# TropComplique/MultiPoseNet

Measured on AMD Instinct MI355X. Metric: images/sec keypoint fwd+bwd+Adam @512x512 bs32/GPU, higher is better.
Workload: dtype bf16; 1 GPU; MobileNet-v1+FPN+keypoint_subnet fwd+bwd+Adam, 512x512, per-GPU batch 32; global_batch=32, parallelism=dp1, hip_graph=True, rccl_ranks=1

## Files before the change

include/mpn.h:

```cpp
#ifndef MPN_H_
#define MPN_H_

#include <stddef.h>
#include <stdint.h>

#ifdef __cplusplus
extern "C" {
#endif

#define MPN_VERSION 600

enum { MPN_F32 = 0, MPN_BF16 = 1, MPN_F16 = 2  };

enum {
    MPN_OK = 0,
    MPN_ERR_BAD_SHAPE = -1,
    MPN_ERR_BAD_DTYPE = -2,
    MPN_ERR_BAD_ALIGN = -3,
    MPN_ERR_HIP = -4,
    MPN_ERR_BAD_ARG = -5,
    MPN_ERR_WORKSPACE = -6,
    MPN_ERR_BAD_DATA = -7
};

enum { MPN_ACT_NONE = 0, MPN_ACT_RELU = 1, MPN_ACT_RELU6 = 2 };

typedef void* mpn_stream_t;

int mpn_version(void);
int mpn_last_error(char* buf, size_t n);

size_t mpn_heatmap_decode_workspace_bytes(int B);
int mpn_heatmap_decode(const void* heatmaps, int dtype, int B, int h, int w, int C,
                       const double* box_hw, float threshold,
                       int32_t* out_xyv, float* out_score, int32_t* out_index,
                       void* workspace, size_t workspace_bytes, mpn_stream_t stream);

size_t mpn_conv_packed_bytes(int Cin, int Cout, int ksize, int transpose, int dtype);
int mpn_conv_pack_weights(const float* w_hwio, int Cin, int Cout, int ksize, int transpose,
                          int dtype, void* out, mpn_stream_t stream);
size_t mpn_conv_pack_desc_bytes(void);
int mpn_conv_pack_desc_fill(void* desc_host, const float* w_hwio, int Cin, int Cout, int ksize, int transpose,
                            int dtype, void* out, int block_begin);
int mpn_conv_pack_weights_batched(const void* descs_device, int ndesc, int total_blocks, int dtype,
                                  mpn_stream_t stream);
int mpn_conv_num_parts(int N, int H, int W, int ksize);
int mpn_conv_stats_rows(int N, int H, int W, int Cin, int Cout, int ksize, int dtype);
int mpn_conv_fwd(const void* x, const void* w_packed, void* y, int N, int H, int W, int Cin,
                 int Cout, int x_stride, int y_stride, int ksize, int dtype, const float* in_scale,
                 const float* in_shift, int in_act, float* stats_part, const void* up_res,
                 mpn_stream_t stream);
int mpn_conv_fwd_grouped(int njobs, const void* const* x, const void* const* w_packed, void* const* y, int N, const int* H,
                         const int* W, int Cin, int Cout, const int* x_stride, const int* y_stride, int ksize, int dtype,
                         const float* const* in_scale, const float* const* in_shift, int in_act,
                         float* const* stats_part, mpn_stream_t stream);
int mpn_conv_bwd_data_bn_supported(int K, int C, int ksize, int dtype);
int mpn_conv_bwd_data_bn(const void* dy, const void* w_packed_t, void* dx, int N, int H, int W, int K, int C, int dy_stride,
                         int dx_stride, int ksize, int dtype, const void* bn_x, int bn_x_stride, const float* bn_scale,
                         const float* bn_shift, int bn_act, float* part, mpn_stream_t stream);
int mpn_conv_bwd_data_bn_grouped(int njobs, const void* const* dy, const void* const* w_packed_t, void* const* dx, int N,
                                 const int* H, const int* W, int K, int C, const int* dy_stride, const int* dx_stride,
                                 int dtype, const void* const* bn_x, const int* bn_x_stride, const float* const* bn_scale,
                                 const float* const* bn_shift, int bn_act, float* const* part, mpn_stream_t stream);

int mpn_conv_wgrad_num_parts(int N, int H, int W, int Cin, int Cout, int ksize, int dtype);
int mpn_conv_bwd_weight(const void* x, const void* dy, float* part, int N, int H, int W, int Cin,
                        int Cout, int x_stride, int dy_stride, int ksize, int dtype, const float* in_scale,
                        const float* in_shift, int in_act, mpn_stream_t stream);

int mpn_conv1x1_bwd_fused_supported(int Cin, int Cout, int dtype);
int mpn_conv1x1_bwd_fused(const void* x, const void* dy, const float* w, void* dx, float* wpart, float* bn_part, int N, int H, int W,
                          int Cin, int Cout, int x_stride, int dy_stride, int dx_stride, int dtype, const float* in_scale,
                          const float* in_shift, int in_act, mpn_stream_t stream);
int mpn_conv1x1_bwd_fused_apply_supported(int Cin, int Cout, int dtype);
int mpn_conv1x1_bwd_fused_apply(const void* x, const void* g, const void* y_raw, const float* w, void* dx, float* wpart, float* bn_part,
                                int N, int H, int W, int Cin, int Cout, int x_stride, int g_stride, int y_stride, int dx_stride,
                                int dtype, const float* in_scale, const float* in_shift, int in_act, const float* ap_scale,
                                const float* ap_shift, const float* ap_mean, const float* ap_invstd, const float* ap_k1,
                                const float* ap_k2, int ap_act, mpn_stream_t stream);
int mpn_conv_wgrad_grouped_num_parts(int njobs, int N, const int* H, const int* W, int Cin, int Cout, int ksize, int dtype,
                                     int* nparts);
int mpn_conv_bwd_weight_grouped(int njobs, const void* const* x, const void* const* dy, float* const* part, int N,
                                const int* H, const int* W, int Cin, int Cout, const int* x_stride, const int* dy_stride,
                                int ksize, int dtype, const float* const* in_scale, const float* const* in_shift,
                                int in_act, mpn_stream_t stream);

int mpn_bn_stats_num_parts(long long M);
int mpn_bn_stats(const void* x, long long M, int C, int dtype, float* part, mpn_stream_t stream);
int mpn_bn_finalize(float* part, int nparts, int C, long long count, const float* gamma,
                    const float* beta, float* moving_mean, float* moving_var, float momentum,
                    float eps, float* scale, float* shift, float* save_mean, float* save_invstd,
                    mpn_stream_t stream);
int mpn_bn_bwd_reduce_grouped(int njobs, void* const* dA, const void* const* x, const long long* M, int C, int dtype,
                              const float* const* scale, const float* const* shift, const float* const* mean,
                              const float* const* invstd, int act, float* const* part, const int* dA_stride,
                              const int* x_stride, mpn_stream_t stream);
int mpn_bn_bwd_apply_grouped(int njobs, void* const* dA, const void* const* x, const long long* M, int C, int dtype,
                             const float* const* scale, const float* const* shift, const float* const* mean,
                             const float* const* invstd, const float* const* k1, const float* const* k2, int act,
                             const float* const* add_ch0, const int* dA_stride, const int* x_stride,
                             mpn_stream_t stream);
size_t mpn_bn_fin_desc_bytes(void);
size_t mpn_bn_bwd_fin_desc_bytes(void);
int mpn_bn_fin_desc_fill(void* desc_host, const float* part, int nparts, int C, long long count, const float* gamma,
                         const float* beta, float* moving_mean, float* moving_var, float* scale, float* shift,
                         float* save_mean, float* save_invstd, int block_begin);
int mpn_bn_bwd_fin_desc_fill(void* desc_host, const float* part, int nparts, int C, long long count, float* dgamma,
                             float* dbeta, float* k1, float* k2, int block_begin);
int mpn_bn_bwd_fin_desc_fill_raw(void* desc_host, const float* part, int nparts, int C, long long count, float* dgamma,
                                 float* dbeta, float* k1, float* k2, const float* mean, const float* invstd,
                                 int block_begin);
int mpn_bn_finalize_batched(const void* descs_device, int ndesc, int total_blocks, float momentum, float eps,
                            mpn_stream_t stream);
int mpn_bn_bwd_finalize_batched(const void* descs_device, int ndesc, int total_blocks, mpn_stream_t stream);
int mpn_bn_inference_affine(int C, const float* gamma, const float* beta, const float* moving_mean,
                            const float* moving_var, float eps, float* scale, float* shift,
                            mpn_stream_t stream);
int mpn_bn_act_apply(const void* x, void* y, long long M, int C, int dtype, const float* scale,
                     const float* shift, int act, mpn_stream_t stream);
int mpn_bn_bwd_reduce(const void* dA, const void* x, long long M, int C, int dtype,
                      const float* scale, const float* shift, const float* mean,
                      const float* invstd, int act, float* part, mpn_stream_t stream);
int mpn_bn_bwd_finalize(float* part, int nparts, int C, long long count, float* dgamma,
                        float* dbeta, float* k1, float* k2, mpn_stream_t stream);
int mpn_bn_bwd_finalize_raw(float* part, int nparts, int C, long long count, float* dgamma, float* dbeta, float* k1,
                            float* k2, const float* mean, const float* invstd, mpn_stream_t stream);
int mpn_bn_bwd_apply(void* dA, const void* x, long long M, int C, int dtype, const float* scale,
                     const float* shift, const float* mean, const float* invstd, const float* k1,
                     const float* k2, int act, const float* add_ch0, mpn_stream_t stream);

int mpn_dwconv_out_size(int size, int stride);
int mpn_dwconv_num_parts(int N, int H, int W, int C, int stride, int dtype);
int mpn_dwconv_fwd(const void* x, const float* w, void* y, int N, int H, int W, int C, int stride,
                   int dtype, const float* in_scale, const float* in_shift, int in_act, int flip,
                   float* stats_part, mpn_stream_t stream);
int mpn_dwconv_bwd_data(const void* dy, const float* w, void* dx, int N, int H, int W, int C,
                        int stride, int dtype, mpn_stream_t stream);
int mpn_dwconv_bwd_data_bn_num_parts(int N, int H, int W, int C, int stride, int dtype);
int mpn_dwconv_bwd_data_bn(const void* dy, const float* w, void* dx, int N, int H, int W, int C, int stride, int dtype,
                           const void* x_bn, const float* scale, const float* shift, const float* mean,
                           const float* invstd, int act, float* part, mpn_stream_t stream);
int mpn_dwconv_bwd_data_add_supported(int N, int H, int W, int C, int stride, int dtype);
int mpn_dwconv_bwd_data_add(const void* dy, const float* w, void* dx, int N, int H, int W, int C, int stride, int dtype,
                            const void* addend, const void* x_bn, const float* scale, const float* shift,
                            const float* mean, const float* invstd, int act, float* part, mpn_stream_t stream);
int mpn_dwconv_wgrad_num_parts(int N, int H, int W, int C, int stride, int dtype);
int mpn_dwconv_bwd_weight(const void* x, const void* dy, float* part, int N, int H, int W, int C,
                          int stride, int dtype, const float* in_scale, const float* in_shift,
                          int in_act, mpn_stream_t stream);

int mpn_dwconv_bwd_fused_supported(int N, int H, int W, int C, int stride, int dtype);
int mpn_dwconv_bwd_fused(const void* x, const void* dy, const float* w, void* dx, float* wpart, int N, int H, int W, int C,
                         int dtype, const float* in_scale, const float* in_shift, int in_act, const float* mean,
                         const float* invstd, float* bn_part, mpn_stream_t stream);
int mpn_dwconv_bwd_fused_s2(const void* x, const void* dy, const float* w, void* dx, float* wpart, int N, int H, int W, int C,
                            int dtype, const float* in_scale, const float* in_shift, int in_act, const float* mean,
                            const float* invstd, float* bn_part, const void* addend, mpn_stream_t stream);

int mpn_stem_conv_fwd(const void* images, int images_u8, const float* w, void* y, int N, int H,
                      int W, int C0, int dtype, mpn_stream_t stream);
int mpn_stem_conv_fwd_num_parts(int N, int H, int W, int C0, int dtype);
int mpn_stem_conv_fwd_stats(const void* images, int images_u8, const float* w, void* y, int N, int H, int W, int C0,
                            int dtype, float* stats_part, mpn_stream_t stream);
int mpn_stem_conv_wgrad_num_parts(int N, int H, int W);
int mpn_stem_conv_bwd_weight(const void* images, int images_u8, const void* dy, float* part, int N,
                             int H, int W, int C0, int dtype, mpn_stream_t stream);

int mpn_bilinear_up_fwd(const void* x, void* y, int N, int h, int w, int C, int upsample,
                        int y_channel_offset, int y_channels_total, int dtype,
                        const float* in_scale, const float* in_shift, int in_act,
                        mpn_stream_t stream);
int mpn_bilinear_up_bwd(const void* dy, void* dx, int N, int h, int w, int C, int upsample,
                        int y_channel_offset, int y_channels_total, int dtype, mpn_stream_t stream);
int mpn_sumpool2x2(const void* src, void* dst, int N, int h, int w, int C, int accumulate,
                   int dtype, mpn_stream_t stream);
int mpn_add_inplace(void* dst, const void* src, long long n, int dtype, mpn_stream_t stream);

int mpn_heatmap_head_fwd(const void* x, const float* w, const float* bias, long long M, int Cin,
                         int dtype, const float* in_scale, const float* in_shift, int in_act,
                         int mode, float* out, float* out_seg, mpn_stream_t stream);
int mpn_heatmap_head_bwd_num_parts(long long M);
int mpn_heatmap_head_bwd(const void* x, const float* dlogits, const float* w, long long M, int Cin,
                         int dtype, const float* in_scale, const float* in_shift, int in_act,
                         void* dA, float* part, mpn_stream_t stream);
int mpn_heatmap_head_bwd_bn_supported(int Cin, int dtype);
int mpn_heatmap_head_bwd_bn(const void* x, const float* dlogits, const float* w, long long M, int Cin, int dtype,
                            const float* in_scale, const float* in_shift, int in_act, void* dA, float* part,
                            float* bn_part, mpn_stream_t stream);

int mpn_keypoint_loss_num_parts(int B, int h, int w);
int mpn_keypoint_loss(const float* logits, const float* heatmaps, const float* loss_masks,
                      const float* segmentation_masks, const int* num_boxes, const void* p2,
                      const void* p3, const void* p4, const void* p5, int p_channels, int p_dtype,
                      float* dlogits, float* daux2, float* daux3, float* daux4, float* daux5,
                      float* part, float* losses_out, int B, int h, int w, mpn_stream_t stream);

int mpn_adam_prepare(long long* step, float* hyper, double initial_learning_rate,
                     double decay_steps, double alpha, double beta1, double beta2,
                     mpn_stream_t stream);
int mpn_adam_step(float* params, const float* grads, float* m, float* v, long long n,
                  const float* hyper, float beta1, float beta2, float eps, float clip,
                  float grad_scale, mpn_stream_t stream);
int mpn_adam_step_cast(float* params, const float* grads, float* m, float* v, long long n, const float* hyper, float beta1,
                       float beta2, float eps, float clip, float grad_scale, int ncast, const long long* cast_begin,
                       const long long* cast_count, void* const* cast_dst, int cast_dtype, mpn_stream_t stream);
int mpn_reduce_partials(const float* part, int nparts, long long n, float* out, int accumulate,
                        float scale, mpn_stream_t stream);
size_t mpn_reduce_desc_bytes(void);
int mpn_reduce_desc_fill(void* desc_host, const float* part, int nparts, long long n, float* out, float scale,
                         int block_begin);
int mpn_reduce_partials_batched(const void* descs_device, int ndesc, int total_blocks, mpn_stream_t stream);
int mpn_axpy(long long n, float a, const float* x, float* y, mpn_stream_t stream);
int mpn_axpy_batched(int count, const float* const* x, float* const* y, const long long* n, float a, mpn_stream_t stream);
int mpn_l2_loss_accumulate(long long n, const float* w, float scale, float* acc, mpn_stream_t stream);
size_t mpn_l2_loss_batched_workspace_bytes(int count, const long long* n);
int mpn_l2_loss_batched(int count, const float* const* w, const long long* n, float scale, float* acc, void* workspace,
                        size_t workspace_bytes, mpn_stream_t stream);

size_t mpn_heatmap_render_workspace_bytes(int total_persons);
int mpn_heatmap_render(const int32_t* keypoints, const float* boxes, const int32_t* first_person,
                       int B, int total_persons, int width, int height, int downsample, float* out,
                       void* workspace, size_t workspace_bytes, mpn_stream_t stream);

enum {
    MPN_AUGMENT_ROTATE = 1, MPN_AUGMENT_COLOR = 2, MPN_AUGMENT_GRAYSCALE = 4, MPN_AUGMENT_PIXEL_SCALE = 8,
    MPN_AUGMENT_FLIP = 16, MPN_AUGMENT_EVAL = 32
};
#define MPN_KEYPOINT_AUGMENT_DESC_BYTES 192
typedef struct mpn_keypoint_augment_desc {
    int64_t src_offset, mask_offset;
    int32_t src_h, src_w, mask_h, mask_w;
    int32_t crop_y, crop_x, crop_h, crop_w;
    int32_t valid_h, valid_w, valid_mh, valid_mw;
    float transform[8], mask_transform[8];
    float window[4];
    float scale_y, scale_x;
    float mask_scale_y, mask_scale_x;
    float color[3];
    uint32_t seed;
    int32_t flags;
    int32_t reserved[3];
} mpn_keypoint_augment_desc;
#ifdef __cplusplus
static_assert(sizeof(mpn_keypoint_augment_desc) == MPN_KEYPOINT_AUGMENT_DESC_BYTES, "descriptor size is fixed");
#endif
size_t mpn_keypoint_augment_desc_bytes(void);
int mpn_keypoint_augment(const uint8_t* sources, const uint8_t* masks, const void* descs, int B, int H, int W,
                         float* images, float* loss_masks, float* segmentation_masks, mpn_stream_t stream);

enum { MPN_AUGMENT_PAD = 64 };
#define MPN_DETECTOR_AUGMENT_DESC_BYTES 112
typedef struct mpn_detector_augment_desc {
    int64_t src_offset;
    int32_t src_h, src_w;
    int32_t crop_y, crop_x, crop_h, crop_w;
    int32_t valid_h, valid_w;
    int32_t pad_y, pad_x, pad_h, pad_w;
    float scale_y, scale_x;
    float pad_scale_y, pad_scale_x;
    float color[3];
    float minval, maxval;
    uint32_t seed;
    int32_t flags;
    int32_t reserved[3];
} mpn_detector_augment_desc;
#ifdef __cplusplus
static_assert(sizeof(mpn_detector_augment_desc) == MPN_DETECTOR_AUGMENT_DESC_BYTES, "descriptor size is fixed");
#endif
size_t mpn_detector_augment_desc_bytes(void);
int mpn_detector_augment(const uint8_t* sources, const void* descs, int B, int H, int W, float* images,
                         mpn_stream_t stream);

#define MPN_PRN_EXAMPLE_DESC_BYTES 16
typedef struct mpn_prn_example_desc {
    int32_t image;
    int32_t person;
    int32_t flip;
    int32_t reserved;
} mpn_prn_example_desc;
#ifdef __cplusplus
static_assert(sizeof(mpn_prn_example_desc) == MPN_PRN_EXAMPLE_DESC_BYTES, "descriptor size is fixed");
#endif
size_t mpn_prn_example_desc_bytes(void);
size_t mpn_prn_examples_workspace_bytes(int total_persons);
int mpn_prn_examples(const int32_t* keypoints, const float* boxes, int total_persons,
                     const int32_t* first_person, const int32_t* width, const int32_t* height,
                     int num_images, const void* examples, int N, int crop_h, int crop_w, int downsample,
                     float* crops, float* labels, void* workspace, size_t workspace_bytes, mpn_stream_t stream);

int mpn_gemm_nt_num_parts(int K);
int mpn_gemm_nt(const void* a, const void* b, float* part, int M, int N, int K, int dtype, mpn_stream_t stream);
int mpn_transpose_cast(const void* in, int in_dtype, void* out, int out_dtype, int R, int C, mpn_stream_t stream);
int mpn_cast(const void* in, int in_dtype, void* out, int out_dtype, long long n, mpn_stream_t stream);
int mpn_bias_relu_fwd(const void* pre, int pre_dtype, const float* bias, void* y, int out_dtype, int R, int C,
                      mpn_stream_t stream);
int mpn_bias_relu_bwd(const void* y, int y_dtype, const float* dy, void* dpre, int dpre_dtype, float* dbias, int R,
                      int C, mpn_stream_t stream);
int mpn_prn_loss(const float* x, const void* y2, int y2_dtype, const float* labels, int B, int P, int C,
                 float* logits, float* dlogits, float* loss_part, float grad_scale, mpn_stream_t stream);
int mpn_prn_residual(const float* x, const void* y2, int y2_dtype, long long n, float* logits, mpn_stream_t stream);

int mpn_heatmap_minmax(const float* heatmaps, int B, int h, int w, int C, void* minmax_keys, mpn_stream_t stream);
int mpn_prn_crop(const float* heatmaps, const void* minmax_keys, const float* boxes, const int* box_ind, int nb, int B,
                 int h, int w, int C, int crop_h, int crop_w, float threshold, float* crops, mpn_stream_t stream);
int mpn_prn_crop_slots(const float* heatmaps, const void* minmax_keys, const float* boxes, const int* num_boxes, int slot0,
                       int nb, int max_boxes, int B, int h, int w, int C, int crop_h, int crop_w, float threshold,
                       float* crops, mpn_stream_t stream);
int mpn_prn_decode(const float* logits, int nb, int crop_h, int crop_w, int C, float* scores, float* positions,
                   mpn_stream_t stream);

// ... 267 lines not shown
```

multiposenet_amd/_lib.py:

```python
import ctypes
import os

_HERE = os.path.dirname(os.path.abspath(__file__))
LIB_PATH = os.environ.get("MPN_LIB") or os.path.join(_HERE, "libmpn_hip.so")

MPN_VERSION = 600
MPN_F32, MPN_BF16, MPN_F16 = 0, 1, 2
ACT_NONE, ACT_RELU, ACT_RELU6 = 0, 1, 2

_c = ctypes
_P = _c.c_void_p
_I = _c.c_int
_F = _c.c_float
_D = _c.c_double
_Z = _c.c_size_t
_L = _c.c_longlong

SIGNATURES = {
    "mpn_version": (_I, []),
    "mpn_last_error": (_I, [_c.c_char_p, _Z]),
    "mpn_heatmap_decode_workspace_bytes": (_Z, [_I]),
    "mpn_heatmap_decode": (_I, [_P, _I, _I, _I, _I, _I, _P, _F, _P, _P, _P, _P, _Z, _P]),
    "mpn_heatmap_render_workspace_bytes": (_Z, [_I]),
    "mpn_heatmap_render": (_I, [_P, _P, _P, _I, _I, _I, _I, _I, _P, _P, _Z, _P]),
    "mpn_keypoint_augment_desc_bytes": (_Z, []),
    "mpn_keypoint_augment": (_I, [_P, _P, _P, _I, _I, _I, _P, _P, _P, _P]),
    "mpn_detector_augment_desc_bytes": (_Z, []),
    "mpn_detector_augment": (_I, [_P, _P, _I, _I, _I, _P, _P]),
    "mpn_prn_example_desc_bytes": (_Z, []),
    "mpn_prn_examples_workspace_bytes": (_Z, [_I]),
    "mpn_prn_examples": (_I, [_P, _P, _I, _P, _P, _P, _I, _P, _I, _I, _I, _I, _P, _P, _P, _Z, _P]),
    "mpn_conv_packed_bytes": (_Z, [_I, _I, _I, _I, _I]),
    "mpn_conv_pack_weights": (_I, [_P, _I, _I, _I, _I, _I, _P, _P]),
    "mpn_conv_pack_desc_bytes": (_Z, []),
    "mpn_conv_pack_desc_fill": (_I, [_P, _P, _I, _I, _I, _I, _I, _P, _I]),
    "mpn_conv_pack_weights_batched": (_I, [_P, _I, _I, _I, _P]),
    "mpn_conv_num_parts": (_I, [_I, _I, _I, _I]),
    "mpn_conv_stats_rows": (_I, [_I, _I, _I, _I, _I, _I, _I]),
    "mpn_conv_fwd": (_I, [_P, _P, _P, _I, _I, _I, _I, _I, _I, _I, _I, _I, _P, _P, _I, _P, _P, _P]),
    "mpn_conv_fwd_grouped": (_I, [_I, _P, _P, _P, _I, _P, _P, _I, _I, _P, _P, _I, _I, _P, _P, _I, _P, _P]),
    "mpn_conv_wgrad_num_parts": (_I, [_I, _I, _I, _I, _I, _I, _I]),
    "mpn_conv_bwd_weight": (_I, [_P, _P, _P, _I, _I, _I, _I, _I, _I, _I, _I, _I, _P, _P, _I, _P]),
    "mpn_conv1x1_bwd_fused_supported": (_I, [_I, _I, _I]),
    "mpn_conv1x1_bwd_fused": (_I, [_P, _P, _P, _P, _P, _P, _I, _I, _I, _I, _I, _I, _I, _I, _I, _P, _P, _I, _P]),
    "mpn_conv1x1_bwd_fused_apply_supported": (_I, [_I, _I, _I]),
    "mpn_conv1x1_bwd_fused_apply": (_I, [_P, _P, _P, _P, _P, _P, _P, _I, _I, _I, _I, _I, _I, _I, _I, _I, _I, _P, _P, _I, _P, _P, _P, _P, _P, _P, _I, _P]),
    "mpn_conv_wgrad_grouped_num_parts": (_I, [_I, _I, _P, _P, _I, _I, _I, _I, _P]),
    "mpn_conv_bwd_weight_grouped": (_I, [_I, _P, _P, _P, _I, _P, _P, _I, _I, _P, _P, _I, _I, _P, _P, _I, _P]),
    "mpn_bn_stats_num_parts": (_I, [_L]),
    "mpn_bn_stats": (_I, [_P, _L, _I, _I, _P, _P]),
    "mpn_bn_finalize": (_I, [_P, _I, _I, _L, _P, _P, _P, _P, _F, _F, _P, _P, _P, _P, _P]),
    "mpn_bn_inference_affine": (_I, [_I, _P, _P, _P, _P, _F, _P, _P, _P]),
    "mpn_bn_act_apply": (_I, [_P, _P, _L, _I, _I, _P, _P, _I, _P]),
    "mpn_bn_bwd_reduce": (_I, [_P, _P, _L, _I, _I, _P, _P, _P, _P, _I, _P, _P]),
    "mpn_bn_bwd_finalize": (_I, [_P, _I, _I, _L, _P, _P, _P, _P, _P]),
    "mpn_bn_bwd_apply": (_I, [_P, _P, _L, _I, _I, _P, _P, _P, _P, _P, _P, _I, _P, _P]),
    "mpn_dwconv_out_size": (_I, [_I, _I]),
    "mpn_dwconv_num_parts": (_I, [_I, _I, _I, _I, _I, _I]),
    "mpn_dwconv_fwd": (_I, [_P, _P, _P, _I, _I, _I, _I, _I, _I, _P, _P, _I, _I, _P, _P]),
    "mpn_dwconv_bwd_data": (_I, [_P, _P, _P, _I, _I, _I, _I, _I, _I, _P]),
    "mpn_dwconv_bwd_data_bn_num_parts": (_I, [_I, _I, _I, _I, _I, _I]),
    "mpn_dwconv_bwd_data_bn": (_I, [_P, _P, _P, _I, _I, _I, _I, _I, _I, _P, _P, _P, _P, _P, _I, _P, _P]),
    "mpn_dwconv_bwd_data_add_supported": (_I, [_I, _I, _I, _I, _I, _I]),
    "mpn_dwconv_bwd_data_add": (_I, [_P, _P, _P, _I, _I, _I, _I, _I, _I, _P, _P, _P, _P, _P, _P, _I, _P, _P]),
    "mpn_dwconv_wgrad_num_parts": (_I, [_I, _I, _I, _I, _I, _I]),
    "mpn_dwconv_bwd_weight": (_I, [_P, _P, _P, _I, _I, _I, _I, _I, _I, _P, _P, _I, _P]),
    "mpn_dwconv_bwd_fused_supported": (_I, [_I, _I, _I, _I, _I, _I]),
    "mpn_dwconv_bwd_fused": (_I, [_P, _P, _P, _P, _P, _I, _I, _I, _I, _I, _P, _P, _I, _P, _P, _P, _P]),
    "mpn_dwconv_bwd_fused_s2": (_I, [_P, _P, _P, _P, _P, _I, _I, _I, _I, _I, _P, _P, _I, _P, _P, _P, _P, _P]),
    "mpn_stem_conv_fwd": (_I, [_P, _I, _P, _P, _I, _I, _I, _I, _I, _P]),
    "mpn_stem_conv_fwd_num_parts": (_I, [_I, _I, _I, _I, _I]),
    "mpn_stem_conv_fwd_stats": (_I, [_P, _I, _P, _P, _I, _I, _I, _I, _I, _P, _P]),
    "mpn_stem_conv_wgrad_num_parts": (_I, [_I, _I, _I]),
    "mpn_stem_conv_bwd_weight": (_I, [_P, _I, _P, _P, _I, _I, _I, _I, _I, _P]),
    "mpn_bilinear_up_fwd": (_I, [_P, _P, _I, _I, _I, _I, _I, _I, _I, _I, _P, _P, _I, _P]),
    "mpn_bilinear_up_bwd": (_I, [_P, _P, _I, _I, _I, _I, _I, _I, _I, _I, _P]),
    "mpn_sumpool2x2": (_I, [_P, _P, _I, _I, _I, _I, _I, _I, _P]),
    "mpn_add_inplace": (_I, [_P, _P, _L, _I, _P]),
    "mpn_heatmap_head_fwd": (_I, [_P, _P, _P, _L, _I, _I, _P, _P, _I, _I, _P, _P, _P]),
    "mpn_heatmap_head_bwd_num_parts": (_I, [_L]),
    "mpn_heatmap_head_bwd": (_I, [_P, _P, _P, _L, _I, _I, _P, _P, _I, _P, _P, _P]),
    "mpn_heatmap_head_bwd_bn_supported": (_I, [_I, _I]),
    "mpn_heatmap_head_bwd_bn": (_I, [_P, _P, _P, _L, _I, _I, _P, _P, _I, _P, _P, _P, _P]),
    "mpn_keypoint_loss_num_parts": (_I, [_I, _I, _I]),
    "mpn_keypoint_loss": (_I, [_P] * 9 + [_I, _I] + [_P] * 7 + [_I, _I, _I, _P]),
    "mpn_adam_prepare": (_I, [_P, _P, _D, _D, _D, _D, _D, _P]),
    "mpn_adam_step": (_I, [_P, _P, _P, _P, _L, _P, _F, _F, _F, _F, _F, _P]),
    "mpn_adam_step_cast": (_I, [_P, _P, _P, _P, _L, _P, _F, _F, _F, _F, _F, _I, _P, _P, _P, _I, _P]),
    "mpn_reduce_partials": (_I, [_P, _I, _L, _P, _I, _F, _P]),
    "mpn_reduce_desc_bytes": (_Z, []),
    "mpn_reduce_desc_fill": (_I, [_P, _P, _I, _L, _P, _F, _I]),
    "mpn_reduce_partials_batched": (_I, [_P, _I, _I, _P]),
    "mpn_gemm_nt_num_parts": (_I, [_I]),
    "mpn_gemm_nt": (_I, [_P, _P, _P, _I, _I, _I, _I, _P]),
    "mpn_transpose_cast": (_I, [_P, _I, _P, _I, _I, _I, _P]),
    "mpn_cast": (_I, [_P, _I, _P, _I, _L, _P]),
    "mpn_bias_relu_fwd": (_I, [_P, _I, _P, _P, _I, _I, _I, _P]),
    "mpn_bias_relu_bwd": (_I, [_P, _I, _P, _P, _I, _P, _I, _I, _P]),
    "mpn_prn_loss": (_I, [_P, _P, _I, _P, _I, _I, _I, _P, _P, _P, _F, _P]),
    "mpn_bn_bwd_reduce_grouped": (_I, [_I, _P, _P, _P, _I, _I, _P, _P, _P, _P, _I, _P, _P, _P, _P]),
    "mpn_bn_bwd_apply_grouped": (_I, [_I, _P, _P, _P, _I, _I, _P, _P, _P, _P, _P, _P, _I, _P, _P, _P, _P]),
    "mpn_bn_fin_desc_bytes": (_Z, []),
    "mpn_bn_bwd_fin_desc_bytes": (_Z, []),
    "mpn_bn_fin_desc_fill": (_I, [_P, _P, _I, _I, _L, _P, _P, _P, _P, _P, _P, _P, _P, _I]),
    "mpn_bn_bwd_fin_desc_fill": (_I, [_P, _P, _I, _I, _L, _P, _P, _P, _P, _I]),
    "mpn_bn_finalize_batched": (_I, [_P, _I, _I, _F, _F, _P]),
    "mpn_bn_bwd_finalize_batched": (_I, [_P, _I, _I, _P]),
    "mpn_heatmap_minmax": (_I, [_P, _I, _I, _I, _I, _P, _P]),
    "mpn_prn_crop": (_I, [_P, _P, _P, _P, _I, _I, _I, _I, _I, _I, _I, _F, _P, _P]),
    "mpn_prn_decode": (_I, [_P, _I, _I, _I, _I, _P, _P, _P]),
    "mpn_conv_bwd_data_bn_supported": (_I, [_I, _I, _I, _I]),
    "mpn_conv_bwd_data_bn": (_I, [_P, _P, _P, _I, _I, _I, _I, _I, _I, _I, _I, _I, _P, _I, _P, _P, _I, _P, _P]),
    "mpn_bn_bwd_finalize_raw": (_I, [_P, _I, _I, _L, _P, _P, _P, _P, _P, _P, _P]),
    "mpn_conv_bwd_data_bn_grouped": (_I, [_I, _P, _P, _P, _I, _P, _P, _I, _I, _P, _P, _I, _P, _P, _P, _P, _I, _P, _P]),
    "mpn_bn_bwd_fin_desc_fill_raw": (_I, [_P, _P, _I, _I, _L, _P, _P, _P, _P, _P, _P, _I]),
    "mpn_prn_crop_slots": (_I, [_P, _P, _P, _P, _I, _I, _I, _I, _I, _I, _I, _I, _I, _F, _P, _P]),
    "mpn_prn_residual": (_I, [_P, _P, _I, _L, _P, _P]),
    "mpn_retina_loss_finalize": (_I, [_P, _P, _F, _F, _P, _P, _P, _P]),
    "mpn_axpy": (_I, [_L, _F, _P, _P, _P]),
    "mpn_axpy_batched": (_I, [_I, _P, _P, _P, _F, _P]),
    "mpn_patchify3x3s2": (_I, [_P, _P, _I, _I, _I, _I, _I, _P, _P, _I, _P]),
    "mpn_unpatchify3x3s2": (_I, [_P, _P, _I, _I, _I, _I, _I, _P]),
    "mpn_retina_match_workspace_bytes": (_Z, [_I, _I]),
    "mpn_retina_match": (_I, [_P, _P, _P, _I, _I, _I, _F, _F, _P, _P, _P, _P, _Z, _P]),
    "mpn_retina_loss_num_parts": (_I, [_I, _I]),
    "mpn_retina_loss": (_I, [_P, _P, _P, _P, _P, _P, _I, _P, _P, _P, _P, _P, _I, _F, _F, _F, _F, _P, _P]),
    "mpn_retina_nms_workspace_bytes": (_Z, [_I, _I]),
    "mpn_retina_nms_overflow_offset": (_Z, [_I, _I]),
    "mpn_retina_nms": (_I, [_P, _P, _P, _P, _I, _P, _P, _P, _I, _F, _F, _I, _P, _P, _P, _P, _Z, _P]),
    "mpn_l2_loss_accumulate": (_I, [_L, _P, _F, _P, _P]),
    "mpn_l2_loss_batched_workspace_bytes": (_Z, [_I, _P]),
    "mpn_l2_loss_batched": (_I, [_I, _P, _P, _F, _P, _P, _Z, _P]),
    "mpn_pose_gather_record_bytes": (_Z, [_I, _I]),
    "mpn_pose_gather_row_offset": (_Z, [_I, _I, _I]),
    "mpn_pose_gather": (_I, [_P, _P, _P, _P, _P, _P, _I, _I, _F, _I, _I, _P, _Z, _P]),
    "mpn_pose_gather_sized": (_I, [_P, _P, _P, _P, _P, _P, _I, _I, _F, _P, _P, _Z, _P]),
    "mpn_oks_gt_row_bytes": (_Z, []),
    "mpn_oks_match_out_bytes": (_Z, [_I, _I]),
    "mpn_oks_match": (_I, [_P, _I, _I, _P, _P, _I, _P, _I, _I, _I, _P, _P, _P]),
    "mpn_pose_track_state_bytes": (_Z, [_I, _I]),
    "mpn_pose_track_out_bytes": (_Z, [_I, _I]),
    "mpn_pose_track": (_I, [_P, _I, _I, _I, _I, _I, _F, _F, _I, _P, _P, _P, _P]),
    "mpn_coco_masks_image_desc_bytes": (_Z, []),
    "mpn_coco_masks_part_desc_bytes": (_Z, []),
    "mpn_coco_masks_plane_words": (_Z, [_I, _I]),
    "mpn_coco_masks_packed_bytes": (_Z, [_I, _I]),
    "mpn_coco_masks": (_I, [_P, _I, _I, _P, _I, _P, _L, _P, _L, _P, _L, _P, _Z, _P, _Z, _P, _Z, _P]),
    "mpn_image_resize_desc_bytes": (_Z, []),
    "mpn_image_resize_workspace_bytes": (_Z, [_I, _I, _I, _L]),
    "mpn_image_resize": (_I, [_P, _P, _P, _I, _I, _I, _P, _P, _Z, _P]),
    "mpn_draw_desc_bytes": (_Z, []),
    "mpn_draw_dot_stamp": (_I, [_I, _I, _I]),
    "mpn_draw_detections_workspace_bytes": (_Z, [_I, _I]),
    "mpn_draw_detections": (_I, [_P, _Z, _P, _P, _Z, _I, _I, _I, _P, _Z, _P, _Z, _P]),
    "mpn_plot_maps_desc_bytes": (_Z, []),
    "mpn_plot_maps_workspace_bytes": (_Z, [_I, _I, _I, _I, _I]),
    "mpn_plot_maps": (_I, [_P, _P, _P, _P, _P, _Z, _P, _I, _I, _I, _I, _I, _P, _P, _Z, _P]),
    "mpn_jpeg_desc_bytes": (_Z, []),
    "mpn_jpeg_info": (_I, [_P, _Z, _P]),
    "mpn_jpeg_entropy_decode": (_I, [_P, _Z, _P, _Z, _P]),
    "mpn_jpeg_decode_workspace_bytes": (_Z, [_I, _L]),
    "mpn_jpeg_decode": (_I, [_P, _Z, _P, _I, _P, _Z, _P, _Z, _P]),
    "mpn_jpeg_scans_info": (_I, [_P, _Z, _P]),
    "mpn_jpeg_scans_decode": (_I, [_P, _Z, _P, _Z, _P]),
    "mpn_jpeg_scan_desc_bytes": (_Z, []),
    "mpn_jpeg_scan_prepare": (_I, [_P, _Z, _P]),
    "mpn_jpeg_entropy_decode_device_workspace_bytes": (_Z, [_I, _L]),
    "mpn_jpeg_entropy_decode_device": (_I, [_P, _Z, _P, _I, _P, _Z, _P, _P, _P, _Z, _I, _P]),
    "mpn_jpeg_enc_desc_bytes": (_Z, []),
    "mpn_jpeg_forward": (_I, [_P, _Z, _P, _I, _P, _Z, _P]),
    "mpn_jpeg_entropy_encode_workspace_bytes": (_Z, [_L, _L]),
    "mpn_jpeg_entropy_encode": (_I, [_P, _Z, _P, _I, _P, _Z, _P, _P, _Z, _P]),
    "mpn_mirror_images": (_I, [_P, _I, _I, _I, _P, _P]),
    "mpn_tta_merge": (_I, [_P, _I, _I, _I, _I, _P, _P, _P]),
}

_lib = None


class MpnError(RuntimeError):
    pass


def lib():
    global _lib
    if _lib is None:
        if not os.path.exists(LIB_PATH):
            raise MpnError(
                f"{LIB_PATH} not found: build it with `python -m multiposenet_amd.build` "
                "(there is no CPU fallback)")
        import torch
        hip_rt = os.path.join(os.path.dirname(torch.__file__), "lib", "libamdhip64.so")
        if os.path.exists(hip_rt):
            ctypes.CDLL(hip_rt, mode=ctypes.RTLD_GLOBAL)
        l = ctypes.CDLL(LIB_PATH)
        l.mpn_version.restype = _I
        if l.mpn_version() != MPN_VERSION:
            raise MpnError(f"{LIB_PATH} is ABI revision {l.mpn_version()}, this binding needs {MPN_VERSION}: "
                           "rebuild with `python -m multiposenet_amd.build --force`")
        for name, (res, args) in SIGNATURES.items():
            fn = getattr(l, name)
            fn.restype = res
            fn.argtypes = args
        _lib = l
    return _lib


def last_error():
    buf = ctypes.create_string_buffer(512)
    lib().mpn_last_error(buf, 512)
    return buf.value.decode("utf-8", "replace")


_ERR_NAMES = {-1: "BAD_SHAPE", -2: "BAD_DTYPE", -3: "BAD_ALIGN", -4: "HIP", -5: "BAD_ARG", -6: "WORKSPACE", -7: "BAD_DATA"}


def check(rc):
    if rc != 0:
        msg = f"MPN_ERR_{_ERR_NAMES.get(rc, rc)}: {last_error()}"
        if rc in (-1, -2, -3, -5, -7):
            raise ValueError(msg)
        raise MpnError(msg)
# ... 92 lines not shown
```

multiposenet_amd/csrc/dwconv.hip:

```cpp
#include <type_traits>
#include "dwconv_walk.h"

namespace {

template <int STRIDE> struct DwTile;
template <> struct DwTile<1> { static constexpr int TH = 8, TW = 16, HH = 10, HW = 18; };
template <> struct DwTile<2> { static constexpr int TH = 4, TW = 8, HH = 9, HW = 17; };

struct DwBnReduce {
    const void* x;
    const float* scale;
    const float* shift;
    const float* mean;
    const float* invstd;
    int act;
};

struct DwParams {
    const void* x;
    const float* w;
    void* y;
    const void* dy;
    float* part;
    const float* in_scale;
    const float* in_shift;
    int in_act;
    int flip;
    int N, H, W, C, OH, OW;
    int pad_t, pad_l;
    int tiles_x, tiles_y;
    int nvg;
    int cblocks;
    DwBnReduce bnr;
    const void* addend;
    int stride;
    float* wpart;
    int swr;
};

__device__ __forceinline__ void load4(const float* p, float (&f)[4]) {
    const float4 q = *reinterpret_cast<const float4*>(p);
    f[0] = q.x; f[1] = q.y; f[2] = q.z; f[3] = q.w;
}
__device__ __forceinline__ void load4(const bf16_t* p, float (&f)[4]) {
    const uint2 q = *reinterpret_cast<const uint2*>(p);
    f[0] = __uint_as_float(q.x << 16); f[1] = __uint_as_float(q.x & 0xffff0000u);
    f[2] = __uint_as_float(q.y << 16); f[3] = __uint_as_float(q.y & 0xffff0000u);
}

template <int NV>
__device__ __forceinline__ void reduce_same_vg(float (&v)[NV], int nvg, float* smem ) {
#pragma unroll
    for (int k = 0; k < NV; ++k)
        for (int o = nvg; o < 64; o <<= 1) v[k] += __shfl_xor(v[k], o, 64);
    const int lane = threadIdx.x & 63, wave = threadIdx.x >> 6;
    __syncthreads();
    if (lane < nvg)
#pragma unroll
        for (int k = 0; k < NV; ++k) smem[(wave * 16 + lane) * NV + k] = v[k];
    __syncthreads();
    if ((int)threadIdx.x < nvg)
#pragma unroll
        for (int k = 0; k < NV; ++k)
            v[k] = smem[(0 * 16 + lane) * NV + k] + smem[(1 * 16 + lane) * NV + k] + smem[(2 * 16 + lane) * NV + k] +
                   smem[(3 * 16 + lane) * NV + k];
}

template <typename T> struct HaloAffine {
    float sc[Vec16<T>::N], sh[Vec16<T>::N];
    bool on;
};

template <typename T>
__device__ __forceinline__ HaloAffine<T> load_halo_affine(const DwParams& p, int c0, int cb_vecs) {
    constexpr int VE = Vec16<T>::N;
    HaloAffine<T> a;
    const int vg = threadIdx.x % p.nvg;
    a.on = p.in_scale != nullptr;
#pragma unroll
    for (int j = 0; j < VE; ++j) {
        const bool ok = a.on && vg < cb_vecs;
        a.sc[j] = ok ? p.in_scale[c0 + vg * VE + j] : 1.f;
        a.sh[j] = ok ? p.in_shift[c0 + vg * VE + j] : 0.f;
    }
    return a;
}

template <typename T, int STRIDE> struct HaloRegs {
    using TL = DwTile<STRIDE>;
    static constexpr int MAXV = (TL::HH * TL::HW * 8 + kThreads - 1) / kThreads;
    Vec16<T> v[MAXV];
    unsigned okmask;

    __device__ __forceinline__ void load(const DwParams& p, int img, int oy0, int ox0, int c0, int cb_vecs) {
        constexpr int VE = Vec16<T>::N;
        const T* __restrict__ x = reinterpret_cast<const T*>(p.x);
        const int iy0 = oy0 * STRIDE - p.pad_t, ix0 = ox0 * STRIDE - p.pad_l;
        int tid_ = threadIdx.x;
        asm volatile("" : "+v"(tid_));
        const int vg = tid_ % p.nvg;
        const int hp0 = tid_ / p.nvg, hstep = kThreads / p.nvg;
        okmask = 0u;
#pragma unroll
        for (int k = 0; k < MAXV; ++k) {
            const int hp = hp0 + k * hstep;
            const int hy = hp / TL::HW, hx = hp - hy * TL::HW;
            const int iy = iy0 + hy, ix = ix0 + hx;
            const bool ok = hp < TL::HH * TL::HW && vg < cb_vecs && iy >= 0 && iy < p.H && ix >= 0 && ix < p.W;
            v[k].load(x + (ok ? (((long long)img * p.H + iy) * p.W + ix) * p.C + c0 + vg * VE : 0));
            okmask |= (ok ? 1u : 0u) << k;
        }
    }

    __device__ __forceinline__ void commit(const DwParams& p, const HaloAffine<T>& aff, float* tile) {
        constexpr int VE = Vec16<T>::N;
        int tid_ = threadIdx.x;
        asm volatile("" : "+v"(tid_));
        const int vg = tid_ % p.nvg;
        const int hp0 = tid_ / p.nvg, hstep = kThreads / p.nvg;
        const float lo = (p.in_act != MPN_ACT_NONE) ? 0.f : -INFINITY;
        const float hi = (p.in_act == MPN_ACT_RELU6) ? 6.f : INFINITY;
#pragma unroll
        for (int k = 0; k < MAXV; ++k) {
            const int hp = hp0 + k * hstep;
            if (hp < TL::HH * TL::HW) {
                float f[VE];
                v[k].unpack(f);
                const bool ok = (okmask >> k) & 1u;
                if (aff.on) {
#pragma unroll
                    for (int j = 0; j < VE; ++j) f[j] = __builtin_amdgcn_fmed3f(f[j] * aff.sc[j] + aff.sh[j], lo, hi);
                }
                if (!ok) {
#pragma unroll
                    for (int j = 0; j < VE; ++j) f[j] = 0.f;
                }
                float* dst = tile + (hp * p.nvg + vg) * VE;
#pragma unroll
                for (int j = 0; j < VE; j += 4)
                    *reinterpret_cast<float4*>(dst + j) = make_float4(f[j], f[j + 1], f[j + 2], f[j + 3]);
            }
        }
    }
};

__device__ __forceinline__ void dw_tile_origin(const DwParams& p, int t, int th, int tw, int& img, int& oy0, int& ox0) {
    const int tx = t % p.tiles_x;
    const int t2 = t / p.tiles_x;
    const int ty = t2 % p.tiles_y;
    img = t2 / p.tiles_y;
    oy0 = ty * th;
    ox0 = tx * tw;
}


__host__ __device__ inline int sw_rows(int OH) { return OH >= 64 ? 32 : 16; }

template <typename T>
__global__ __launch_bounds__(kThreads) void dwconv_fwd_s2_kernel(const DwParams p, int ncg, int cols, int xblocks, int yblocks) {
    __shared__ float red[kThreads * 8];
    const SwLane l = sw_lane<1, false>(p.C, p.OW, ncg, cols, xblocks, yblocks, p.cblocks);
    f32x2_t w01[9], w23[9];
    load_weights(p.w, p.C, l.cc, p.flip != 0, w01, w23);
    InAffine aff;
    aff.load<true>(p.in_scale, p.in_shift, p.in_act, l.cc);
    const int swr = p.swr > 0 ? p.swr : sw_rows(p.OH);
    const int oy_begin = l.yb * swr, oy_end = min(oy_begin + swr, p.OH);
    const T* ximg = reinterpret_cast<const T*>(p.x) + (long long)l.img * p.H * p.W * p.C + l.cc;
    WinCols<T, 3> win;
    win.init(l.ox * 2 - p.pad_l, l.ok, p.H, p.W, p.C);
    auto row_act = [&](const Raw4<T> (&r)[3], int iy, f32x2_t (&a)[3][2]) { win.template act<true, true, -1>(r, iy, aff, a); };
    f32x2_t s01 = {0.f, 0.f}, s23 = {0.f, 0.f}, q01 = {0.f, 0.f}, q23 = {0.f, 0.f};
    f32x2_t r0[3][2], r1[3][2], r2[3][2];
    T* yp = reinterpret_cast<T*>(p.y) + (((long long)l.img * p.OH + oy_begin) * p.OW + l.ox) * p.C + l.cc;
    const long long ystep = (long long)p.OW * p.C;
    auto emit = [&](const f32x2_t (&a)[3][2], const f32x2_t (&bb)[3][2], const f32x2_t (&cr)[3][2]) {
        f32x2_t a01 = {0.f, 0.f}, a23 = {0.f, 0.f};
#pragma unroll
        for (int k = 0; k < 3; ++k) {
            a01 += a[k][0] * w01[k];      a23 += a[k][1] * w23[k];
            a01 += bb[k][0] * w01[3 + k]; a23 += bb[k][1] * w23[3 + k];
            a01 += cr[k][0] * w01[6 + k]; a23 += cr[k][1] * w23[6 + k];
        }
        if (l.ok) {
            add_stats(a01, a23, s01, s23, q01, q23);
            store4x2(yp, a01, a23);
        }
        yp += ystep;
    };
    Raw4<T> ra[3], rb[3];
// ... 91 lines not shown
        bnr_load(yb, oy_begin + 1);
        bnr_load(yc, oy_begin + 2);
        row_act(ra, iy, r0);
        win.load(ra, ximg, iy + 3);
        row_act(rb, iy + 1, r1);
        win.load(rb, ximg, iy + 4);
        iy += 2;
        for (int oy = oy_begin; oy < oy_end; oy += 3, iy += 3) {
            row_act(rc, iy, r2);
            win.load(rc, ximg, iy + 3);
            emit(r0, r1, r2, ya);
            bnr_load(ya, oy + 3);
            if (oy + 1 < oy_end) {
                row_act(ra, iy + 1, r0);
                win.load(ra, ximg, iy + 4);
                emit(r1, r2, r0, yb);
                bnr_load(yb, oy + 4);
            }
            if (oy + 2 < oy_end) {
                row_act(rb, iy + 2, r1);
                win.load(rb, ximg, iy + 5);
                emit(r2, r0, r1, yc);
                bnr_load(yc, oy + 5);
            }
        }
    };
    if (interior) walk(std::false_type{}); else walk(std::true_type{});
    if (p.part != nullptr) write_sums_row(red, l, ncg, cols, p.C, p.part, s01, s23, q01, q23);
}

template <typename T>
__global__ __launch_bounds__(kThreads) void dwconv_wgrad_s2_kernel(const DwParams p, int ncg, int cols, int xblocks, int yblocks,
                                                                  int rows) {
    __shared__ __attribute__((aligned(16))) float red[9 * kThreads * 4];
    const SwLane l = sw_lane<1, true>(p.C, p.OW, ncg, cols, xblocks, yblocks, p.cblocks);
    InAffine aff;
    aff.load<true>(p.in_scale, p.in_shift, p.in_act, l.cc);
    const int oy_begin = l.yb * rows, oy_end = min(oy_begin + rows, p.OH);
    const T* ximg = reinterpret_cast<const T*>(p.x) + (long long)l.img * p.H * p.W * p.C + l.cc;
    const T* dyimg = reinterpret_cast<const T*>(p.dy) + ((long long)l.img * p.OH * p.OW + l.ox) * p.C + l.cc;
    WinCols<T, 3> win;
    win.init(l.ox * 2 - p.pad_l, l.ok, p.H, p.W, p.C);
    auto row_act = [&](const Raw4<T> (&r)[3], int iy, f32x2_t (&a)[3][2]) { win.template act<true, true, -1>(r, iy, aff, a); };
    auto dy_load = [&](Raw4<T>& r, int oy) { raw_load(r, dyimg + (long long)min(oy, p.OH - 1) * p.OW * p.C); };
    f32x2_t a01[9] = {}, a23[9] = {};
    auto accum = [&](const f32x2_t (&ra_)[3][2], const f32x2_t (&rb_)[3][2], const f32x2_t (&rc_)[3][2], const Raw4<T>& d) {
        f32x2_t g01, g23;
        raw_unpack2(d, g01, g23);
#pragma unroll
        for (int k = 0; k < 3; ++k) {
            a01[k] += ra_[k][0] * g01;     a23[k] += ra_[k][1] * g23;
            a01[3 + k] += rb_[k][0] * g01; a23[3 + k] += rb_[k][1] * g23;
            a01[6 + k] += rc_[k][0] * g01; a23[6 + k] += rc_[k][1] * g23;
        }
    };
    f32x2_t r0[3][2], r1[3][2], r2[3][2];
    Raw4<T> ra[3], rb[3], da, db;
    int iy = oy_begin * 2 - p.pad_t;
    win.load(ra, ximg, iy);
    dy_load(da, oy_begin);
    dy_load(db, oy_begin + 1);
    row_act(ra, iy, r0);
    win.load(ra, ximg, iy + 1);
    win.load(rb, ximg, iy + 2);
    for (int oy = oy_begin; oy < oy_end; oy += 2, iy += 4) {
        row_act(ra, iy + 1, r1);
        row_act(rb, iy + 2, r2);
        win.load(ra, ximg, iy + 3);
        win.load(rb, ximg, iy + 4);
        accum(r0, r1, r2, da);
        dy_load(da, oy + 2);
        if (oy + 1 < oy_end) {
            row_act(ra, iy + 3, r1);
            row_act(rb, iy + 4, r0);
            win.load(ra, ximg, iy + 5);
            win.load(rb, ximg, iy + 6);
            accum(r2, r1, r0, db);
            dy_load(db, oy + 3);
        }
    }
    write_taps_row(red, l, ncg, cols, p.C, p.part, a01, a23);
}

template <typename T>
__global__ __launch_bounds__(kThreads) void dwconv_wgrad_sw2_kernel(const DwParams p, int ncg, int cols, int xblocks, int yblocks,
                                                                   int rows) {
    __shared__ __attribute__((aligned(16))) float red[9 * kThreads * 4];
    const SwLane l = sw_lane<2, true>(p.C, p.OW, ncg, cols, xblocks, yblocks, p.cblocks);
    const bool ok1 = l.ok && l.ox + 1 < p.OW;
    InAffine aff;
    aff.load<true>(p.in_scale, p.in_shift, p.in_act, l.cc);
    const int oy_begin = l.yb * rows, oy_end = min(oy_begin + rows, p.OH);
    const T* ximg = reinterpret_cast<const T*>(p.x) + (long long)l.img * p.H * p.W * p.C + l.cc;
    const T* dyimg = reinterpret_cast<const T*>(p.dy) + ((long long)l.img * p.OH * p.OW + l.ox) * p.C + l.cc;
    const int dyoff1 = ok1 ? p.C : 0;
    WinCols<T, 4> win;
    win.init(l.ox - p.pad_l, l.ok, p.H, p.W, p.C);
    auto row_act = [&](const Raw4<T> (&r)[4], int iy, f32x2_t (&a)[4][2]) { win.template act<true, true, 1>(r, iy, aff, a); };
    auto dy_load = [&](Raw4<T> (&r)[2], int oy) {
        const T* q = dyimg + (long long)min(oy, p.OH - 1) * p.OW * p.C;
        raw_load(r[0], q);
        raw_load(r[1], q + dyoff1);
    };
    f32x2_t a01[9] = {}, a23[9] = {};
    auto accum = [&](const f32x2_t (&ra_)[4][2], const f32x2_t (&rb_)[4][2], const f32x2_t (&rc_)[4][2], const Raw4<T> (&d)[2]) {
        float h[4];
        f32x2_t g01, g23;
        raw_unpack2(d[0], g01, g23);
        raw_unpack(d[1], h);
        const float m1 = ok1 ? 1.f : 0.f;
        const f32x2_t h01 = {h[0] * m1, h[1] * m1}, h23 = {h[2] * m1, h[3] * m1};
#pragma unroll
        for (int k = 0; k < 3; ++k) {
            a01[k] += ra_[k][0] * g01 + ra_[k + 1][0] * h01;     a23[k] += ra_[k][1] * g23 + ra_[k + 1][1] * h23;
            a01[3 + k] += rb_[k][0] * g01 + rb_[k + 1][0] * h01; a23[3 + k] += rb_[k][1] * g23 + rb_[k + 1][1] * h23;
            a01[6 + k] += rc_[k][0] * g01 + rc_[k + 1][0] * h01; a23[6 + k] += rc_[k][1] * g23 + rc_[k + 1][1] * h23;
        }
    };
    f32x2_t r0[4][2], r1[4][2], r2[4][2];
    Raw4<T> ra[4], rb[4], rc[4], da[2], db[2], dc[2];
    int iy = oy_begin - p.pad_t;
    win.load(ra, ximg, iy);
    win.load(rb, ximg, iy + 1);
    win.load(rc, ximg, iy + 2);
    dy_load(da, oy_begin);
    dy_load(db, oy_begin + 1);
    dy_load(dc, oy_begin + 2);
    row_act(ra, iy, r0);
    win.load(ra, ximg, iy + 3);
    row_act(rb, iy + 1, r1);
    win.load(rb, ximg, iy + 4);
    iy += 2;
    for (int oy = oy_begin; oy < oy_end; oy += 3, iy += 3) {
        row_act(rc, iy, r2);
        win.load(rc, ximg, iy + 3);
        accum(r0, r1, r2, da);
        dy_load(da, oy + 3);
        if (oy + 1 < oy_end) {
            row_act(ra, iy + 1, r0);
            win.load(ra, ximg, iy + 4);
            accum(r1, r2, r0, db);
            dy_load(db, oy + 4);
        }
        if (oy + 2 < oy_end) {
            row_act(rb, iy + 2, r1);
            win.load(rb, ximg, iy + 5);
            accum(r2, r0, r1, dc);
            dy_load(dc, oy + 5);
        }
    }
    write_taps_row(red, l, ncg, cols, p.C, p.part, a01, a23);
}

template <typename T, bool BNR>
__global__ __launch_bounds__(kThreads) void dwconv_bwd_sw2_kernel(const DwParams p, int ncg, int cols, int xblocks, int yblocks, int rows) {
    __shared__ __attribute__((aligned(16))) float red[9 * kThreads * 4];
    const SwLane l = sw_lane<2, true>(p.C, p.W, ncg, cols, xblocks, yblocks, p.cblocks);
    const bool ok1 = l.ok && l.ox + 1 < p.W;
    f32x2_t w01[9], w23[9];
#pragma unroll
    for (int t = 0; t < 9; ++t) {
        const float4 q = *reinterpret_cast<const float4*>(p.w + (8 - t) * p.C + l.cc);
        w01[t] = (f32x2_t){q.x, q.y};
        w23[t] = (f32x2_t){q.z, q.w};
    }
    InAffine aff;
    aff.load<false>(p.in_scale, p.in_shift, p.in_act, l.cc);
    f32x2_t s01 = {0.f, 0.f}, s23 = {0.f, 0.f}, q01 = {0.f, 0.f}, q23 = {0.f, 0.f};
    BnReduce<T> bn;
    if constexpr (BNR) bn.load(p.in_scale, p.in_shift, p.bnr.mean, p.bnr.invstd, p.in_act, l.cc);
    const int oy_begin = l.yb * rows, oy_end = min(oy_begin + rows, p.H);
    const long long img_off = (long long)l.img * p.H * p.W * p.C + l.cc;
    const T* ximg = reinterpret_cast<const T*>(p.x) + img_off;
    const T* dimg = reinterpret_cast<const T*>(p.dy) + img_off;
    WinCols<T, 4> win;
    win.init(l.ox - 1, l.ok, p.H, p.W, p.C);
    bool xok[4];
#pragma unroll
    for (int k = 0; k < 4; ++k) xok[k] = l.ok && l.ox - 1 + k >= 0 && l.ox - 1 + k < p.W;
    auto dy_row = [&](const Raw4<T> (&r)[4], int iy, f32x2_t (&a)[4][2]) {
        const bool rowok = iy >= 0 && iy < p.H;
#pragma unroll
        for (int k = 0; k < 4; ++k) {
            float f[4];
            raw_unpack(r[k], f);
            zero_unless(rowok && xok[k], f);
            store_pairs(a[k], f);
        }
    };
    auto in_row = [&](const Raw4<T> (&r)[4], f32x2_t (&a)[4][2]) {
#pragma unroll
        for (int k = 0; k < 4; ++k) {
            float f[4];
            raw_unpack(r[k], f);
            aff.apply(f);
            if (k != 1) zero_unless(xok[k], f);
            store_pairs(a[k], f);
        }
    };
    f32x2_t a01[9] = {}, a23[9] = {};
    T* yp = reinterpret_cast<T*>(p.y) + img_off + ((long long)oy_begin * p.W + l.ox) * p.C;
    auto step = [&](const f32x2_t (&d0)[4][2], const f32x2_t (&d1)[4][2], const f32x2_t (&d2)[4][2], const f32x2_t (&xin)[4][2],
                    const Raw4<T> (&xr)[4]) {
        f32x2_t e01 = {0.f, 0.f}, e23 = {0.f, 0.f}, g01 = {0.f, 0.f}, g23 = {0.f, 0.f};
#pragma unroll
        for (int k = 0; k < 3; ++k) {
            e01 += d0[k][0] * w01[k];          e23 += d0[k][1] * w23[k];
            e01 += d1[k][0] * w01[3 + k];      e23 += d1[k][1] * w23[3 + k];
            e01 += d2[k][0] * w01[6 + k];      e23 += d2[k][1] * w23[6 + k];
            g01 += d0[k + 1][0] * w01[k];      g23 += d0[k + 1][1] * w23[k];
            g01 += d1[k + 1][0] * w01[3 + k];  g23 += d1[k + 1][1] * w23[3 + k];
            g01 += d2[k + 1][0] * w01[6 + k];  g23 += d2[k + 1][1] * w23[6 + k];
        }
        if (l.ok) {
            if constexpr (BNR) bn.add(e01, e23, xr[1], s01, s23, q01, q23);
            store4x2(yp, e01, e23);
        }
        if (ok1) {
            if constexpr (BNR) bn.add(g01, g23, xr[2], s01, s23, q01, q23);
            store4x2(yp + p.C, g01, g23);
        }
        yp += win.rstep;
#pragma unroll
        for (int k = 0; k < 3; ++k) {
            a01[k] += xin[k][0] * d2[1][0] + xin[k + 1][0] * d2[2][0];     a23[k] += xin[k][1] * d2[1][1] + xin[k + 1][1] * d2[2][1];
            a01[3 + k] += xin[k][0] * d1[1][0] + xin[k + 1][0] * d1[2][0]; a23[3 + k] += xin[k][1] * d1[1][1] + xin[k + 1][1] * d1[2][1];
            a01[6 + k] += xin[k][0] * d0[1][0] + xin[k + 1][0] * d0[2][0]; a23[6 + k] += xin[k][1] * d0[1][1] + xin[k + 1][1] * d0[2][1];
        }
    };
    f32x2_t r0[4][2], r1[4][2], r2[4][2], xin[4][2];
    Raw4<T> da[4], db[4], dc[4], xa[4], xb[4], xc[4];
    win.load(da, dimg, oy_begin - 1);
    win.load(db, dimg, oy_begin);
    win.load(dc, dimg, oy_begin + 1);
    win.load(xa, ximg, oy_begin);
    win.load(xb, ximg, oy_begin + 1);
    win.load(xc, ximg, oy_begin + 2);
    dy_row(da, oy_begin - 1, r0);
    win.load(da, dimg, oy_begin + 2);
    dy_row(db, oy_begin, r1);
    win.load(db, dimg, oy_begin + 3);
    for (int r = oy_begin; r < oy_end; r += 3) {
        dy_row(dc, r + 1, r2);
        win.load(dc, dimg, r + 4);
        in_row(xa, xin);
        step(r0, r1, r2, xin, xa);
        win.load(xa, ximg, r + 3);
        if (r + 1 < oy_end) {
            dy_row(da, r + 2, r0);
            win.load(da, dimg, r + 5);
            in_row(xb, xin);
            step(r1, r2, r0, xin, xb);
            win.load(xb, ximg, r + 4);
        }
        if (r + 2 < oy_end) {
            dy_row(db, r + 3, r1);
            win.load(db, dimg, r + 6);
            in_row(xc, xin);
            step(r2, r0, r1, xin, xc);
            win.load(xc, ximg, r + 5);
        }
    }
    write_taps_row(red, l, ncg, cols, p.C, p.wpart, a01, a23);
    if constexpr (BNR) {
        __syncthreads();
        write_sums_row(red, l, ncg, cols, p.C, p.part, s01, s23, q01, q23);
    }
}

__host__ __device__ inline int dg_rows(int OH) { return OH >= 64 ? 32 : (OH >= 32 ? 16 : 8); }
template <typename T, bool BNR, bool ADD>
__global__ __launch_bounds__(kThreads) void dwconv_dgrad_s2_sw_kernel(const T* __restrict__ dy, const float* __restrict__ w,
                                                                      T* __restrict__ dx, int H, int W, int C, int OH, int OW,
                                                                      int ncg, int cols, int xblocks, int yblocks, int cblocks,
                                                                      const DwParams p) {
    __shared__ float red[BNR ? kThreads * 8 : 1];
    const SwLane l = sw_lane<1, false>(C, OW, ncg, cols, xblocks, yblocks, cblocks);
    f32x2_t w01[9], w23[9];
#pragma unroll
    for (int t = 0; t < 9; ++t) {
        const float4 q = *reinterpret_cast<const float4*>(w + t * C + l.cc);
        w01[t] = (f32x2_t){q.x, q.y};
        w23[t] = (f32x2_t){q.z, q.w};
    }
    const int dgr = dg_rows(OH);
    const int a_begin = l.yb * dgr, a_end = min(a_begin + dgr, OH);
    const bool left_ok = l.ox > 0;
    const T* dyimg = dy + ((long long)l.img * OH * OW) * C + l.cc;
    const int off_c = l.ox * C, off_l = (left_ok ? l.ox - 1 : 0) * C;
    auto dy_load = [&](Raw4<T> (&r)[2], int a) {
        const T* rowp = dyimg + (long long)min(max(a, 0), OH - 1) * OW * C;
        raw_load(r[0], rowp + off_l);
        raw_load(r[1], rowp + off_c);
    };
    auto dy_cvt = [&](const Raw4<T> (&r)[2], int a, f32x2_t (&v)[2][2]) {
        if (a < 0) {
            v[0][0] = v[0][1] = v[1][0] = v[1][1] = (f32x2_t){0.f, 0.f};
            return;
        }
        float f[4];
        raw_unpack(r[0], f);
#pragma unroll
        for (int j = 0; j < 4; ++j) f[j] = left_ok ? f[j] : 0.f;
        v[0][0] = (f32x2_t){f[0], f[1]}; v[0][1] = (f32x2_t){f[2], f[3]};
        raw_unpack(r[1], f);
        v[1][0] = (f32x2_t){f[0], f[1]}; v[1][1] = (f32x2_t){f[2], f[3]};
    };
    const long long xrow = (long long)W * C;
    const long long quad0 = (((long long)l.img * H + 2 * a_begin) * W + 2 * l.ox) * C + l.cc;
    T* xp = dx + quad0;
    f32x2_t s01 = {0.f, 0.f}, s23 = {0.f, 0.f}, q01 = {0.f, 0.f}, q23 = {0.f, 0.f};
    BnReduce<T> bn;
    const T* bxp = nullptr;
    if constexpr (BNR) {
        bn.load(p.bnr.scale, p.bnr.shift, p.bnr.mean, p.bnr.invstd, p.bnr.act, l.cc);
        bxp = reinterpret_cast<const T*>(p.bnr.x) + quad0;
    }
    const T* adp = nullptr;
    if constexpr (ADD) adp = reinterpret_cast<const T*>(p.addend) + quad0;
    Raw4<T> yq[4], aq[4];
    auto next_quads = [&](int a) {
        const long long o = (long long)(2 * (min(a, OH - 1) - a_begin)) * xrow;
        if constexpr (BNR) quad_load(yq, bxp + o, xrow, C);
        if constexpr (ADD) quad_load(aq, adp + o, xrow, C);
    };
    int a_cur = a_begin;
    auto emit = [&](const f32x2_t (&pv)[2][2], const f32x2_t (&cv)[2][2]) {
        f32x2_t e01 = cv[1][0] * w01[0] + pv[1][0] * w01[6] + cv[0][0] * w01[2] + pv[0][0] * w01[8];
        f32x2_t e23 = cv[1][1] * w23[0] + pv[1][1] * w23[6] + cv[0][1] * w23[2] + pv[0][1] * w23[8];
        f32x2_t f01 = cv[1][0] * w01[1] + pv[1][0] * w01[7];
        f32x2_t f23 = cv[1][1] * w23[1] + pv[1][1] * w23[7];
        f32x2_t g01 = cv[1][0] * w01[3] + cv[0][0] * w01[5];
        f32x2_t g23 = cv[1][1] * w23[3] + cv[0][1] * w23[5];
        f32x2_t h01 = cv[1][0] * w01[4];
        f32x2_t h23 = cv[1][1] * w23[4];
        if constexpr (ADD) {
            add_raw4(aq[0], e01, e23);
            add_raw4(aq[1], f01, f23);
            add_raw4(aq[2], g01, g23);
            add_raw4(aq[3], h01, h23);
        }
        if (l.ok) {
            store4x2(xp, e01, e23);
            store4x2(xp + C, f01, f23);
            store4x2(xp + xrow, g01, g23);
            store4x2(xp + xrow + C, h01, h23);
            if constexpr (BNR) {
                bn.add(e01, e23, yq[0], s01, s23, q01, q23);
                bn.add(f01, f23, yq[1], s01, s23, q01, q23);
                bn.add(g01, g23, yq[2], s01, s23, q01, q23);
                bn.add(h01, h23, yq[3], s01, s23, q01, q23);
            }
        }
        xp += 2 * xrow;
        next_quads(++a_cur);
    };
    next_quads(a_begin);
    Raw4<T> ra[2], rb[2], rc[2];
    f32x2_t v0[2][2], v1[2][2];
    dy_load(ra, a_begin - 1);
    dy_load(rb, a_begin);
    dy_load(rc, a_begin + 1);
    dy_cvt(ra, a_begin - 1, v0);
    dy_load(ra, a_begin + 2);
    for (int a = a_begin; a < a_end; a += 6) {
        dy_cvt(rb, a, v1);     dy_load(rb, a + 3); emit(v0, v1);
        if (a + 1 < a_end) { dy_cvt(rc, a + 1, v0); dy_load(rc, a + 4); emit(v1, v0); }
        if (a + 2 < a_end) { dy_cvt(ra, a + 2, v1); dy_load(ra, a + 5); emit(v0, v1); }
        if (a + 3 < a_end) { dy_cvt(rb, a + 3, v0); dy_load(rb, a + 6); emit(v1, v0); }
        if (a + 4 < a_end) { dy_cvt(rc, a + 4, v1); dy_load(rc, a + 7); emit(v0, v1); }
        if (a + 5 < a_end) { dy_cvt(ra, a + 5, v0); dy_load(ra, a + 8); emit(v1, v0); }
    }
    if constexpr (BNR) write_sums_row(red, l, ncg, cols, C, p.part, s01, s23, q01, q23);
}

template <typename T, bool BNR, bool ADD>
__global__ __launch_bounds__(kThreads) void dwconv_bwd_s2_kernel(const DwParams p, int ncg, int cols, int xblocks, int yblocks, int rows) {
    __shared__ __attribute__((aligned(16))) float red[9 * kThreads * 4];
    const int H = p.H, W = p.W, C = p.C, OH = p.OH, OW = p.OW;
    const SwLane l = sw_lane<1, true>(C, OW, ncg, cols, xblocks, yblocks, p.cblocks);
    f32x2_t w01[9], w23[9];
#pragma unroll
    for (int t = 0; t < 9; ++t) {
        const float4 q = *reinterpret_cast<const float4*>(p.w + t * C + l.cc);
        w01[t] = (f32x2_t){q.x, q.y};
        w23[t] = (f32x2_t){q.z, q.w};
    }
    InAffine aff;
    aff.load<false>(p.in_scale, p.in_shift, p.in_act, l.cc);
    f32x2_t s01 = {0.f, 0.f}, s23 = {0.f, 0.f}, q01 = {0.f, 0.f}, q23 = {0.f, 0.f};
    BnReduce<T> bn;
    if constexpr (BNR) bn.load(p.in_scale, p.in_shift, p.bnr.mean, p.bnr.invstd, p.in_act, l.cc);
    const int a_begin = l.yb * rows, a_end = min(a_begin + rows, OH);
    const bool right_ok = l.ok && 2 * l.ox + 2 < W;
    const bool left_ok = l.ox > 0;
    const T* dyimg = reinterpret_cast<const T*>(p.dy) + ((long long)l.img * OH * OW) * C + l.cc;
    const int off_c = l.ox * C, off_l = (left_ok ? l.ox - 1 : 0) * C;
    auto dy_load = [&](Raw4<T> (&r)[2], int a) {
        const T* rowp = dyimg + (long long)min(max(a, 0), OH - 1) * OW * C;
        raw_load(r[0], rowp + off_l);
        raw_load(r[1], rowp + off_c);
    };
    auto dy_cvt = [&](const Raw4<T> (&r)[2], int a, f32x2_t (&v)[2][2]) {
        if (a < 0) {
            v[0][0] = v[0][1] = v[1][0] = v[1][1] = (f32x2_t){0.f, 0.f};
            return;
        }
        float f[4];
        raw_unpack(r[0], f);
#pragma unroll
        for (int j = 0; j < 4; ++j) f[j] = left_ok ? f[j] : 0.f;
        v[0][0] = (f32x2_t){f[0], f[1]}; v[0][1] = (f32x2_t){f[2], f[3]};
        raw_unpack(r[1], f);
        v[1][0] = (f32x2_t){f[0], f[1]}; v[1][1] = (f32x2_t){f[2], f[3]};
    };
    const T* ximg = reinterpret_cast<const T*>(p.x) + (long long)l.img * H * W * C + l.cc;
    const int xo0 = 2 * l.ox * C, xo1 = xo0 + C, xo2 = right_ok ? xo0 + 2 * C : xo0;
    const long long xrow = (long long)W * C;
    auto x_load = [&](Raw4<T> (&r)[3], int iy) {
        const T* rowp = ximg + (long long)min(iy, H - 1) * xrow;
        raw_load(r[0], rowp + xo0);
        raw_load(r[1], rowp + xo1);
        raw_load(r[2], rowp + xo2);
    };
    auto x_act = [&](const Raw4<T> (&r)[3], int iy, f32x2_t (&a)[3][2]) {
        const bool rowok = iy < H;
#pragma unroll
        for (int k = 0; k < 3; ++k) {
            float f[4];
            raw_unpack(r[k], f);
            aff.apply(f);
            zero_unless(rowok && (k < 2 || right_ok), f);
            store_pairs(a[k], f);
        }
    };
    const long long quad0 = (((long long)l.img * H + 2 * a_begin) * W + 2 * l.ox) * C + l.cc;
    T* xp = reinterpret_cast<T*>(p.y) + quad0;
    const T* adp = nullptr;
    if constexpr (ADD) adp = reinterpret_cast<const T*>(p.addend) + quad0;
    Raw4<T> aq[4];
    auto add_load = [&](int a) {
        if constexpr (ADD) quad_load(aq, adp + (long long)(2 * (min(a, OH - 1) - a_begin)) * xrow, xrow, C);
    };
    f32x2_t a01[9] = {}, a23[9] = {};
    int a_cur = a_begin;
    auto emit = [&](const f32x2_t (&pv)[2][2], const f32x2_t (&cv)[2][2], const Raw4<T> (&e0)[2], const Raw4<T> (&e1)[2]) {
        f32x2_t e01 = cv[1][0] * w01[0] + pv[1][0] * w01[6] + cv[0][0] * w01[2] + pv[0][0] * w01[8];
        f32x2_t e23 = cv[1][1] * w23[0] + pv[1][1] * w23[6] + cv[0][1] * w23[2] + pv[0][1] * w23[8];
        f32x2_t f01 = cv[1][0] * w01[1] + pv[1][0] * w01[7];
        f32x2_t f23 = cv[1][1] * w23[1] + pv[1][1] * w23[7];
        f32x2_t g01 = cv[1][0] * w01[3] + cv[0][0] * w01[5];
        f32x2_t g23 = cv[1][1] * w23[3] + cv[0][1] * w23[5];
        f32x2_t h01 = cv[1][0] * w01[4];
        f32x2_t h23 = cv[1][1] * w23[4];
        if constexpr (ADD) {
            add_raw4(aq[0], e01, e23);
            add_raw4(aq[1], f01, f23);
            add_raw4(aq[2], g01, g23);
            add_raw4(aq[3], h01, h23);
        }
        if (l.ok) {
            store4x2(xp, e01, e23);
            store4x2(xp + C, f01, f23);
            store4x2(xp + xrow, g01, g23);
            store4x2(xp + xrow + C, h01, h23);
            if constexpr (BNR) {
                bn.add(e01, e23, e0[0], s01, s23, q01, q23);
                bn.add(f01, f23, e0[1], s01, s23, q01, q23);
                bn.add(g01, g23, e1[0], s01, s23, q01, q23);
                bn.add(h01, h23, e1[1], s01, s23, q01, q23);
            }
        }
        xp += 2 * xrow;
        add_load(++a_cur);
    };
    auto wacc = [&](const f32x2_t (&r0)[3][2], const f32x2_t (&r1)[3][2], const f32x2_t (&r2)[3][2], const f32x2_t (&cv)[2][2]) {
#pragma unroll
        for (int k = 0; k < 3; ++k) {
            a01[k] += r0[k][0] * cv[1][0];     a23[k] += r0[k][1] * cv[1][1];
            a01[3 + k] += r1[k][0] * cv[1][0]; a23[3 + k] += r1[k][1] * cv[1][1];
            a01[6 + k] += r2[k][0] * cv[1][0]; a23[6 + k] += r2[k][1] * cv[1][1];
        }
    };
    add_load(a_begin);
    Raw4<T> ra[2], rb[2], rc[2];
    Raw4<T> xa[3], xb[3];
    Raw4<T> ke[2], ko[2], k1[2];
    f32x2_t v0[2][2], v1[2][2];
    f32x2_t E0[3][2], E1[3][2], E2[3][2];
    dy_load(ra, a_begin - 1);
    dy_load(rb, a_begin);
    dy_load(rc, a_begin + 1);
    x_load(xa, 2 * a_begin);
    dy_cvt(ra, a_begin - 1, v0);
    dy_load(ra, a_begin + 2);
    x_act(xa, 2 * a_begin, E0);
    ke[0] = xa[0]; ke[1] = xa[1];
    x_load(xa, 2 * a_begin + 1);
    x_load(xb, 2 * a_begin + 2);
    auto step = [&](int a, Raw4<T> (&rd)[2], const f32x2_t (&pv)[2][2], f32x2_t (&cv)[2][2], const f32x2_t (&Ein)[3][2], const Raw4<T> (&kin)[2],
                    f32x2_t (&Eout)[3][2], Raw4<T> (&kout)[2]) __attribute__((always_inline)) {
        dy_cvt(rd, a, cv);
        dy_load(rd, a + 3);
        x_act(xa, 2 * a + 1, E1);
        k1[0] = xa[0]; k1[1] = xa[1];
        x_act(xb, 2 * a + 2, Eout);
        kout[0] = xb[0]; kout[1] = xb[1];
        x_load(xa, 2 * a + 3);
        x_load(xb, 2 * a + 4);
        emit(pv, cv, kin, k1);
        wacc(Ein, E1, Eout, cv);
    };
    for (int a = a_begin; a < a_end; a += 6) {
        step(a, rb, v0, v1, E0, ke, E2, ko);
        if (a + 1 < a_end) step(a + 1, rc, v1, v0, E2, ko, E0, ke);
        if (a + 2 < a_end) step(a + 2, ra, v0, v1, E0, ke, E2, ko);
        if (a + 3 < a_end) step(a + 3, rb, v1, v0, E2, ko, E0, ke);
        if (a + 4 < a_end) step(a + 4, rc, v0, v1, E0, ke, E2, ko);
        if (a + 5 < a_end) step(a + 5, ra, v1, v0, E2, ko, E0, ke);
    }
    write_taps_row(red, l, ncg, cols, C, p.wpart, a01, a23);
    if constexpr (BNR) {
        __syncthreads();
        write_sums_row(red, l, ncg, cols, C, p.part, s01, s23, q01, q23);
    }
}

template <typename T>
__global__ __launch_bounds__(kThreads) void dwconv_dgrad_s2_kernel(const T* __restrict__ dy, const float* __restrict__ w,
                                                                   T* __restrict__ dx, int N, int H, int W, int C, int OH,
                                                                   int OW, int pad_t, int pad_l, long long total_vec) {
    constexpr int VE = Vec16<T>::N;
    const int cvec = C / VE;
    for (long long i = (long long)blockIdx.x * kThreads + threadIdx.x; i < total_vec;
         i += (long long)gridDim.x * kThreads) {
        const int vg = (int)(i % cvec);
        long long r = i / cvec;
        const int ix = (int)(r % W); r /= W;
        const int iy = (int)(r % H);
        const int n = (int)(r / H);
        float acc[VE];
#pragma unroll
        for (int j = 0; j < VE; ++j) acc[j] = 0.f;
#pragma unroll
        for (int ky = 0; ky < 3; ++ky) {
            const int ty = iy + pad_t - ky;
            if (ty < 0 || (ty & 1) || (ty >> 1) >= OH) continue;
#pragma unroll
            for (int kx = 0; kx < 3; ++kx) {
                const int tx = ix + pad_l - kx;
                if (tx < 0 || (tx & 1) || (tx >> 1) >= OW) continue;
                Vec16<T> v;
                v.load(dy + (((long long)n * OH + (ty >> 1)) * OW + (tx >> 1)) * C + vg * VE);
                float f[VE];
                v.unpack(f);
#pragma unroll
                for (int j = 0; j < VE; ++j) acc[j] += f[j] * w[(ky * 3 + kx) * C + vg * VE + j];
            }
        }
        Vec16<T> ov;
        ov.pack(acc);
        ov.store(dx + i * VE);
    }
}

template <typename T, int STRIDE>
__global__ __launch_bounds__(kThreads, 2) void dwconv_wgrad_kernel(const DwParams p, int nsplit) {
    using TL = DwTile<STRIDE>;
    constexpr int VE = Vec16<T>::N;
    extern __shared__ __attribute__((aligned(16))) float smem_f[];
    float* tile = smem_f;
    float* red = smem_f + TL::HH * TL::HW * p.nvg * VE;

    const int cb = blockIdx.x % p.cblocks;
    const int split = blockIdx.x / p.cblocks;
    const int c0 = cb * p.nvg * VE;
    const int cb_vecs = min(p.nvg, (p.C - c0) / VE);
    const int cstride = p.nvg * VE;
    const int ncg = cstride / 4;
    const int cg = threadIdx.x % ncg;
    const int pt = threadIdx.x / ncg;
    const int npt = kThreads / ncg;
    const bool cg_ok = cg * 4 < cb_vecs * VE;
    const T* __restrict__ dy = reinterpret_cast<const T*>(p.dy);

    f32x2_t acc2[18];
#pragma unroll
    for (int j = 0; j < 18; ++j) acc2[j] = (f32x2_t){0.f, 0.f};

    const HaloAffine<T> aff = load_halo_affine<T>(p, c0, cb_vecs);
    const int ntiles = p.N * p.tiles_y * p.tiles_x;
    HaloRegs<T, STRIDE> hr;
    int img, oy0, ox0;
    constexpr int NOP = TL::TH * TL::TW / (kThreads / 16);
    if (split < ntiles) {
        dw_tile_origin(p, split, TL::TH, TL::TW, img, oy0, ox0);
        hr.load(p, img, oy0, ox0, c0, cb_vecs);
        hr.commit(p, aff, tile);
    }
    for (int t = split; t < ntiles; t += nsplit) {
        dw_tile_origin(p, t, TL::TH, TL::TW, img, oy0, ox0);
        float g_all[NOP][4];
        unsigned gmask = 0u;
#pragma unroll
        for (int k = 0; k < NOP; ++k) {
            const int op = pt + k * npt;
            const int oyl = op / TL::TW, oxl = op - oyl * TL::TW;
            const int oy = oy0 + oyl, ox = ox0 + oxl;
            const bool ok = op < TL::TH * TL::TW && cg_ok && oy < p.OH && ox < p.OW;
            load4(dy + (ok ? (((long long)img * p.OH + oy) * p.OW + ox) * p.C + c0 + cg * 4 : 0), g_all[k]);
            gmask |= (ok ? 1u : 0u) << k;
        }
        const bool more = t + nsplit < ntiles;
        if (more) {
            int img2, oy2, ox2;
            dw_tile_origin(p, t + nsplit, TL::TH, TL::TW, img2, oy2, ox2);
            hr.load(p, img2, oy2, ox2, c0, cb_vecs);
        }
        __syncthreads();
#pragma unroll
        for (int k = 0; k < NOP; ++k) {
            const int op = pt + k * npt;
            const int oyl = op / TL::TW, oxl = op - oyl * TL::TW;
            if (!((gmask >> k) & 1u)) continue;
            const float (&g)[4] = g_all[k];
            float4 q[9];
            const float* base = tile + ((oyl * STRIDE) * TL::HW + oxl * STRIDE) * cstride + cg * 4;
#pragma unroll
            for (int t = 0; t < 9; ++t) q[t] = *reinterpret_cast<const float4*>(base + ((t / 3) * TL::HW + (t % 3)) * cstride);
            __builtin_amdgcn_sched_barrier(0);
#pragma unroll
            for (int t = 0; t < 9; ++t) {
                acc2[t * 2 + 0] += (f32x2_t){q[t].x, q[t].y} * (f32x2_t){g[0], g[1]};
                acc2[t * 2 + 1] += (f32x2_t){q[t].z, q[t].w} * (f32x2_t){g[2], g[3]};
            }
            __builtin_amdgcn_sched_barrier(0);
        }
        __syncthreads();
        if (more) hr.commit(p, aff, tile);
    }
    float acc[36];
#pragma unroll
    for (int j = 0; j < 18; ++j) { acc[2 * j] = acc2[j].x; acc[2 * j + 1] = acc2[j].y; }
    reduce_same_vg<36>(acc, ncg, red);
    if ((int)threadIdx.x < ncg && cg_ok) {
// ... 173 lines not shown
        return dw_launch_fwd(p, dw_sw_geom(p), dtype, "dwconv_bwd_data", st);
    }
    const DwDgS2Geom g = dw_dg_s2_geom(p);
    if (g.ok) {
        unsigned grid;
        if (int rc = dw_grid((long long)N * g.cblocks * g.yblocks * g.xblocks, "dwconv_bwd_data", &grid)) return rc;
        MPN_DISPATCH_DTYPE(dtype, dw_with_bnr_add(bnr != nullptr, addend != nullptr, [&](auto B, auto A) {
            dwconv_dgrad_s2_sw_kernel<T, decltype(B)::value, decltype(A)::value><<<grid, kThreads, 0, st>>>(
                (const T*)dy, w, (T*)dx, H, W, C, p.OH, p.OW, g.ncg, g.cols, g.xblocks, g.yblocks, g.cblocks, p);
        }));
        MPN_LAUNCH_CHECK();
        return MPN_OK;
    }
    MPN_REQUIRE(bnr == nullptr, MPN_ERR_BAD_SHAPE, "dwconv_bwd_data_bn: shape not supported (mpn_dwconv_bwd_data_bn_num_parts == 0)");
    const int ve = dtype == MPN_F32 ? 4 : 8;
    const long long total_vec = (long long)N * H * W * (C / ve);
    long long blocks = (total_vec + kThreads - 1) / kThreads;
    if (blocks > 8192) blocks = 8192;
    MPN_DISPATCH_DTYPE(dtype, (dwconv_dgrad_s2_kernel<T><<<(int)blocks, kThreads, 0, st>>>(
                                  (const T*)dy, w, (T*)dx, N, H, W, C, p.OH, p.OW, p.pad_t, p.pad_l, total_vec)));
    MPN_LAUNCH_CHECK();
    return MPN_OK;
}

extern "C" int mpn_dwconv_bwd_data(const void* dy, const float* w, void* dx, int N, int H, int W, int C, int stride,
                                   int dtype, mpn_stream_t stream) {
    return dw_bwd_data_impl(dy, w, dx, N, H, W, C, stride, dtype, nullptr, nullptr, stream);
}

extern "C" int mpn_dwconv_bwd_data_bn_num_parts(int N, int H, int W, int C, int stride, int dtype) {
    DwParams p = {};
    if (fill_params(p, N, H, W, C, stride, dtype)) return 0;
    if (C % 4 != 0) return 0;
    if (stride == 1) {
        p.bnr.x = &p;
        const DwSwGeom g = dw_sw_geom(p);
        if (kThreads % g.ncg != 0) return 0;
        return p.N * g.yblocks * g.xblocks;
    }
    const DwDgS2Geom g = dw_dg_s2_geom(p);
    return g.ok ? N * g.yblocks * g.xblocks : 0;
}

extern "C" int mpn_dwconv_bwd_data_bn(const void* dy, const float* w, void* dx, int N, int H, int W, int C, int stride,
                                      int dtype, const void* x_bn, const float* scale, const float* shift, const float* mean,
                                      const float* invstd, int act, float* part, mpn_stream_t stream) {
    MPN_REQUIRE(x_bn && scale && shift && mean && invstd && part, MPN_ERR_BAD_ARG, "dwconv_bwd_data_bn: null pointer");
    MPN_REQUIRE(mpn_dwconv_bwd_data_bn_num_parts(N, H, W, C, stride, dtype) > 0, MPN_ERR_BAD_SHAPE,
                "dwconv_bwd_data_bn: shape not supported (mpn_dwconv_bwd_data_bn_num_parts == 0)");
    const DwBnReduce b = {x_bn, scale, shift, mean, invstd, act};
    return dw_bwd_data_impl(dy, w, dx, N, H, W, C, stride, dtype, &b, part, stream);
}

extern "C" int mpn_dwconv_bwd_data_add_supported(int N, int H, int W, int C, int stride, int dtype) {
    DwParams p = {};
    if (fill_params(p, N, H, W, C, stride, dtype)) return 0;
    return (stride == 2 && C % 4 == 0 && dw_dg_s2_geom(p).ok) ? 1 : 0;
}

extern "C" int mpn_dwconv_bwd_data_add(const void* dy, const float* w, void* dx, int N, int H, int W, int C, int stride,
                                       int dtype, const void* addend, const void* x_bn, const float* scale,
                                       const float* shift, const float* mean, const float* invstd, int act, float* part,
                                       mpn_stream_t stream) {
    MPN_REQUIRE(addend, MPN_ERR_BAD_ARG, "dwconv_bwd_data_add: null addend");
    MPN_REQUIRE(mpn_dwconv_bwd_data_add_supported(N, H, W, C, stride, dtype), MPN_ERR_BAD_SHAPE,
                "dwconv_bwd_data_add: shape not supported (mpn_dwconv_bwd_data_add_supported == 0)");
    if (x_bn == nullptr) return dw_bwd_data_impl(dy, w, dx, N, H, W, C, stride, dtype, nullptr, nullptr, stream, addend);
    MPN_REQUIRE(scale && shift && mean && invstd && part, MPN_ERR_BAD_ARG, "dwconv_bwd_data_add: null batch-norm pointer");
    const DwBnReduce b = {x_bn, scale, shift, mean, invstd, act};
    return dw_bwd_data_impl(dy, w, dx, N, H, W, C, stride, dtype, &b, part, stream, addend);
}

struct DwWgSwGeom { int ncg, cols, xblocks, yblocks, cblocks, rows, units; };
static DwWgSwGeom dw_wg_sw_geom(const DwParams& p) {
    DwWgSwGeom g;
    const int cg_total = p.C / 4;
    g.ncg = cg_total < 32 ? cg_total : 32;
    g.cols = kThreads / g.ncg;
    g.cblocks = (cg_total + g.ncg - 1) / g.ncg;
    g.rows = p.stride == 1 ? (p.OH >= 128 ? 64 : (p.OH >= 64 ? 32 : 16)) : (p.OH >= 64 ? 32 : (p.OH >= 32 ? 16 : 8));
    g.xblocks = (p.OW + g.cols * dw_cols_per_lane(p.stride) - 1) / (g.cols * dw_cols_per_lane(p.stride));
    g.yblocks = (p.OH + g.rows - 1) / g.rows;
    g.units = p.N * g.yblocks * g.xblocks;
    return g;
}
static bool dw_wg_use_sw(const DwParams& p) {
    const int cg_total = p.C / 4;
    const int ncg = cg_total < 32 ? cg_total : 32;
    return (ncg & (ncg - 1)) == 0 && kThreads % ncg == 0;
}

extern "C" int mpn_dwconv_wgrad_num_parts(int N, int H, int W, int C, int stride, int dtype) {
    DwParams p = {};
    if (fill_params(p, N, H, W, C, stride, dtype)) return 0;
    if (dw_wg_use_sw(p)) return dw_wg_sw_geom(p).units;
    const int ntiles = N * p.tiles_y * p.tiles_x;
    int nsplit = 2048 / p.cblocks;
    if (nsplit < 1) nsplit = 1;
    if (nsplit > ntiles) nsplit = ntiles;
    return nsplit;
}

extern "C" int mpn_dwconv_bwd_weight(const void* x, const void* dy, float* part, int N, int H, int W, int C,
                                     int stride, int dtype, const float* in_scale, const float* in_shift, int in_act,
                                     mpn_stream_t stream) {
    DwParams p = {};
    if (int rc = fill_params(p, N, H, W, C, stride, dtype)) return rc;
    MPN_REQUIRE(x && dy && part, MPN_ERR_BAD_ARG, "dwconv_bwd_weight: null pointer");
    p.x = x; p.dy = dy; p.part = part;
    p.in_scale = in_scale; p.in_shift = in_shift; p.in_act = in_act;
    const int ve = dtype == MPN_F32 ? 4 : 8;
    const int nsplit = mpn_dwconv_wgrad_num_parts(N, H, W, C, stride, dtype);
    hipStream_t st = (hipStream_t)stream;
    if (dw_wg_use_sw(p)) {
        const DwWgSwGeom g = dw_wg_sw_geom(p);
        p.cblocks = g.cblocks;
        unsigned grid;
        if (int rc = dw_grid((long long)g.units * g.cblocks, "dwconv_bwd_weight", &grid)) return rc;
        MPN_DISPATCH_DTYPE(dtype, {
            if (stride == 1) dwconv_wgrad_sw2_kernel<T><<<grid, kThreads, 0, st>>>(p, g.ncg, g.cols, g.xblocks, g.yblocks, g.rows);
            else dwconv_wgrad_s2_kernel<T><<<grid, kThreads, 0, st>>>(p, g.ncg, g.cols, g.xblocks, g.yblocks, g.rows);
        });
        MPN_LAUNCH_CHECK();
        return MPN_OK;
    }
    const int grid = nsplit * p.cblocks;
    if (stride == 1) {
        const size_t sm = dw_smem<1>(ve, 36, p.nvg);
        MPN_DISPATCH_DTYPE(dtype, {
            if (int rc = set_smem(dwconv_wgrad_kernel<T, 1>, sm)) return rc;
            dwconv_wgrad_kernel<T, 1><<<grid, kThreads, sm, st>>>(p, nsplit);
        });
    } else {
        const size_t sm = dw_smem<2>(ve, 36, p.nvg);
        MPN_DISPATCH_DTYPE(dtype, {
            if (int rc = set_smem(dwconv_wgrad_kernel<T, 2>, sm)) return rc;
            dwconv_wgrad_kernel<T, 2><<<grid, kThreads, sm, st>>>(p, nsplit);
        });
    }
    MPN_LAUNCH_CHECK();
    return MPN_OK;
}

extern "C" int mpn_dwconv_bwd_fused_supported(int N, int H, int W, int C, int stride, int dtype) {
    DwParams p = {};
    if ((stride != 1 && stride != 2) || fill_params(p, N, H, W, C, stride, dtype)) return 0;
    if (C % 4 != 0 || !dw_wg_use_sw(p)) return 0;
    if (stride == 1) return 1;
    const DwDgS2Geom d = dw_dg_s2_geom(p);
    const DwWgSwGeom g = dw_wg_sw_geom(p);
    return (d.ok && d.ncg == g.ncg && d.cols == g.cols && d.xblocks == g.xblocks && d.yblocks == g.yblocks && dg_rows(p.OH) == g.rows) ? 1 : 0;
}

extern "C" int mpn_dwconv_bwd_fused(const void* x, const void* dy, const float* w, void* dx, float* wpart, int N, int H, int W, int C,
                                    int dtype, const float* in_scale, const float* in_shift, int in_act, const float* mean,
                                    const float* invstd, float* bn_part, mpn_stream_t stream) {
    MPN_REQUIRE(mpn_dwconv_bwd_fused_supported(N, H, W, C, 1, dtype), MPN_ERR_BAD_SHAPE,
                "dwconv_bwd_fused: shape not supported (mpn_dwconv_bwd_fused_supported == 0)");
    MPN_REQUIRE(x && dy && w && dx && wpart && in_scale && in_shift, MPN_ERR_BAD_ARG, "dwconv_bwd_fused: null pointer");
    MPN_REQUIRE(bn_part == nullptr || (mean && invstd), MPN_ERR_BAD_ARG, "dwconv_bwd_fused: the reduction needs mean and invstd");
    MPN_REQUIRE(dx != dy && dx != x, MPN_ERR_BAD_ARG, "dwconv_bwd_fused: dx must not alias an input");
    DwParams p = {};
    if (int rc = fill_params(p, N, H, W, C, 1, dtype)) return rc;
    p.x = x; p.dy = dy; p.w = w; p.y = dx; p.wpart = wpart; p.part = bn_part;
    p.in_scale = in_scale; p.in_shift = in_shift; p.in_act = in_act; p.bnr.mean = mean; p.bnr.invstd = invstd;
    const DwWgSwGeom g = dw_wg_sw_geom(p);
    p.cblocks = g.cblocks;
    unsigned grid;
    if (int rc = dw_grid((long long)g.units * g.cblocks, "dwconv_bwd_fused", &grid)) return rc;
    hipStream_t st = (hipStream_t)stream;
    MPN_DISPATCH_DTYPE(dtype, {
        if (bn_part) dwconv_bwd_sw2_kernel<T, true><<<grid, kThreads, 0, st>>>(p, g.ncg, g.cols, g.xblocks, g.yblocks, g.rows);
        else dwconv_bwd_sw2_kernel<T, false><<<grid, kThreads, 0, st>>>(p, g.ncg, g.cols, g.xblocks, g.yblocks, g.rows);
    });
    MPN_LAUNCH_CHECK();
    return MPN_OK;
}

extern "C" int mpn_dwconv_bwd_fused_s2(const void* x, const void* dy, const float* w, void* dx, float* wpart, int N, int H, int W, int C,
                                       int dtype, const float* in_scale, const float* in_shift, int in_act, const float* mean,
                                       const float* invstd, float* bn_part, const void* addend, mpn_stream_t stream) {
    MPN_REQUIRE(mpn_dwconv_bwd_fused_supported(N, H, W, C, 2, dtype), MPN_ERR_BAD_SHAPE,
                "dwconv_bwd_fused_s2: shape not supported (mpn_dwconv_bwd_fused_supported == 0)");
    MPN_REQUIRE(x && dy && w && dx && wpart && in_scale && in_shift, MPN_ERR_BAD_ARG, "dwconv_bwd_fused_s2: null pointer");
    MPN_REQUIRE(bn_part == nullptr || (mean && invstd), MPN_ERR_BAD_ARG, "dwconv_bwd_fused_s2: the reduction needs mean and invstd");
    MPN_REQUIRE(dx != dy && dx != x && dx != addend, MPN_ERR_BAD_ARG, "dwconv_bwd_fused_s2: dx must not alias an input");
    DwParams p = {};
    if (int rc = fill_params(p, N, H, W, C, 2, dtype)) return rc;
    p.x = x; p.dy = dy; p.w = w; p.y = dx; p.wpart = wpart; p.part = bn_part; p.addend = addend;
    p.in_scale = in_scale; p.in_shift = in_shift; p.in_act = in_act; p.bnr.mean = mean; p.bnr.invstd = invstd;
    const DwWgSwGeom g = dw_wg_sw_geom(p);
    p.cblocks = g.cblocks;
    unsigned grid;
    if (int rc = dw_grid((long long)g.units * g.cblocks, "dwconv_bwd_fused_s2", &grid)) return rc;
    hipStream_t st = (hipStream_t)stream;
    MPN_DISPATCH_DTYPE(dtype, dw_with_bnr_add(bn_part != nullptr, addend != nullptr, [&](auto B, auto A) {
        dwconv_bwd_s2_kernel<T, decltype(B)::value, decltype(A)::value><<<grid, kThreads, 0, st>>>(p, g.ncg, g.cols, g.xblocks, g.yblocks, g.rows);
    }));
    MPN_LAUNCH_CHECK();
    return MPN_OK;
}
```

multiposenet_amd/csrc/dwconv_walk.h:

```cpp
#pragma once
#include "common.h"

namespace {

constexpr int kThreads = 256;
typedef float f32x2_t __attribute__((ext_vector_type(2)));
typedef __bf16 bf16x2_t __attribute__((ext_vector_type(2)));

template <typename T> struct Raw4;
template <> struct Raw4<float> { float4 v; };
template <> struct Raw4<bf16_t> { uint2 v; };
__device__ __forceinline__ void raw_load(Raw4<float>& r, const float* p) { r.v = *reinterpret_cast<const float4*>(p); }
__device__ __forceinline__ void raw_load(Raw4<bf16_t>& r, const bf16_t* p) { r.v = *reinterpret_cast<const uint2*>(p); }
__device__ __forceinline__ void raw_unpack(const Raw4<float>& r, float (&f)[4]) { f[0] = r.v.x; f[1] = r.v.y; f[2] = r.v.z; f[3] = r.v.w; }
__device__ __forceinline__ void raw_unpack(const Raw4<bf16_t>& r, float (&f)[4]) {
    f[0] = __uint_as_float(r.v.x << 16); f[1] = __uint_as_float(r.v.x & 0xffff0000u);
    f[2] = __uint_as_float(r.v.y << 16); f[3] = __uint_as_float(r.v.y & 0xffff0000u);
}
template <typename T> __device__ __forceinline__ void raw_unpack2(const Raw4<T>& r, f32x2_t& v01, f32x2_t& v23) {
    float f[4];
    raw_unpack(r, f);
    v01 = (f32x2_t){f[0], f[1]};
    v23 = (f32x2_t){f[2], f[3]};
}
// ... 4 lines not shown
    const bf16x2_t lo = __builtin_convertvector(a, bf16x2_t), hi = __builtin_convertvector(b, bf16x2_t);
    uint2 q;
    q.x = __builtin_bit_cast(unsigned, lo);
    q.y = __builtin_bit_cast(unsigned, hi);
    *reinterpret_cast<uint2*>(p) = q;
}
template <typename T> __device__ __forceinline__ f32x2_t round_storage(f32x2_t a);
template <> __device__ __forceinline__ f32x2_t round_storage<float>(f32x2_t a) { return a; }
template <> __device__ __forceinline__ f32x2_t round_storage<bf16_t>(f32x2_t a) {
    return __builtin_convertvector(__builtin_convertvector(a, bf16x2_t), f32x2_t);
}

__device__ __forceinline__ int xcd_work_id() {
    const int wid = blockIdx.x, nwg = gridDim.x, q = nwg >> 3, r = nwg & 7, xcd = wid & 7;
    return (xcd < r ? xcd * (q + 1) : r * (q + 1) + (xcd - r) * q) + (wid >> 3);
}

struct SwLane {
    int img, yb, cgb, unit;
    int ox;
    int cc;
    bool ok;
};
template <int XT, bool CB_INNER>
__device__ __forceinline__ SwLane sw_lane(int C, int OW, int ncg, int cols, int xblocks, int yblocks, int cblocks) {
    SwLane l;
    int b = xcd_work_id(), xb;
    if (CB_INNER) {
        l.cgb = b % cblocks; b /= cblocks;
        l.unit = b;
        xb = b % xblocks; b /= xblocks;
        l.yb = b % yblocks;
        l.img = b / yblocks;
    } else {
        xb = b % xblocks; b /= xblocks;
        l.yb = b % yblocks; b /= yblocks;
        l.cgb = b % cblocks;
        l.img = b / cblocks;
        l.unit = (l.img * yblocks + l.yb) * xblocks + xb;
    }
    const int cgl = threadIdx.x % ncg, col = threadIdx.x / ncg;
    const int c = (l.cgb * ncg + cgl) * 4, ox = (xb * cols + col) * XT;
    l.ok = c < C && ox < OW && col < cols;
    l.cc = l.ok ? c : 0;
    l.ox = l.ok ? ox : 0;
    return l;
}

struct InAffine {
    f32x2_t sc01, sc23, sh01, sh23;
    float lo, hi;
    template <bool NULLABLE>
    __device__ __forceinline__ void load(const float* scale, const float* shift, int act, int cc) {
        const bool on = !NULLABLE || scale != nullptr;
        float4 s4 = make_float4(1.f, 1.f, 1.f, 1.f), h4 = make_float4(0.f, 0.f, 0.f, 0.f);
        if (on) { s4 = *reinterpret_cast<const float4*>(scale + cc); h4 = *reinterpret_cast<const float4*>(shift + cc); }
        sc01 = (f32x2_t){s4.x, s4.y}; sc23 = (f32x2_t){s4.z, s4.w};
        sh01 = (f32x2_t){h4.x, h4.y}; sh23 = (f32x2_t){h4.z, h4.w};
        lo = (on && act != MPN_ACT_NONE) ? 0.f : -INFINITY;
        hi = (on && act == MPN_ACT_RELU6) ? 6.f : INFINITY;
    }
    __device__ __forceinline__ void apply(float (&f)[4]) const {
        const f32x2_t v01 = (f32x2_t){f[0], f[1]} * sc01 + sh01, v23 = (f32x2_t){f[2], f[3]} * sc23 + sh23;
        f[0] = __builtin_amdgcn_fmed3f(v01.x, lo, hi); f[1] = __builtin_amdgcn_fmed3f(v01.y, lo, hi);
        f[2] = __builtin_amdgcn_fmed3f(v23.x, lo, hi); f[3] = __builtin_amdgcn_fmed3f(v23.y, lo, hi);
    }
};

__device__ __forceinline__ void load_weights(const float* w, int C, int cc, bool flip, f32x2_t (&w01)[9], f32x2_t (&w23)[9]) {
#pragma unroll
    for (int t = 0; t < 9; ++t) {
        const float4 q = *reinterpret_cast<const float4*>(w + (flip ? 8 - t : t) * C + cc);
        w01[t] = (f32x2_t){q.x, q.y};
        w23[t] = (f32x2_t){q.z, q.w};
    }
}

__device__ __forceinline__ void zero_unless(bool ok, float (&f)[4]) {
#pragma unroll
    for (int j = 0; j < 4; ++j) f[j] = ok ? f[j] : 0.f;
}
__device__ __forceinline__ void store_pairs(f32x2_t (&a)[2], const float (&f)[4]) {
    a[0] = (f32x2_t){f[0], f[1]};
    a[1] = (f32x2_t){f[2], f[3]};
}

template <typename T, int NC> struct WinCols {
    bool ok[NC];
    int off[NC];
    int H;
    long long rstep;
    __device__ __forceinline__ void init(int ix0, bool lane_ok, int H_, int W, int C) {
        H = H_;
        rstep = (long long)W * C;
#pragma unroll
        for (int k = 0; k < NC; ++k) {
            const int ix = ix0 + k;
            ok[k] = lane_ok && ix >= 0 && ix < W;
            off[k] = (ok[k] ? ix : 0) * C;
        }
    }
    __device__ __forceinline__ void load(Raw4<T> (&r)[NC], const T* img, int iy) const {
        const T* rowp = img + (long long)min(max(iy, 0), H - 1) * rstep;
#pragma unroll
        for (int k = 0; k < NC; ++k) raw_load(r[k], rowp + off[k]);
    }
    template <bool AFF, bool EDGE, int INSIDE>
    __device__ __forceinline__ void act(const Raw4<T> (&r)[NC], int iy, const InAffine& aff, f32x2_t (&a)[NC][2]) const {
        if (iy < 0 || iy >= H) {
#pragma unroll
            for (int k = 0; k < NC; ++k) { a[k][0] = (f32x2_t){0.f, 0.f}; a[k][1] = (f32x2_t){0.f, 0.f}; }
            return;
        }
#pragma unroll
        for (int k = 0; k < NC; ++k) {
            float f[4];
            raw_unpack(r[k], f);
            if constexpr (AFF) aff.apply(f);
            if (EDGE && k != INSIDE) zero_unless(ok[k], f);
            store_pairs(a[k], f);
        }
    }
};

__device__ __forceinline__ void add_stats(f32x2_t y01, f32x2_t y23, f32x2_t& s01, f32x2_t& s23, f32x2_t& q01, f32x2_t& q23) {
    s01 += y01; s23 += y23;
    q01 += y01 * y01; q23 += y23 * y23;
}
template <typename T> struct BnReduce {
    f32x2_t sc01, sc23, sh01, sh23, is01, is23, nm01, nm23;
    float lo, hi;
    __device__ __forceinline__ void load(const float* scale, const float* shift, const float* mean, const float* invstd, int act, int cc) {
        const float4 s4 = *reinterpret_cast<const float4*>(scale + cc), h4 = *reinterpret_cast<const float4*>(shift + cc);
        const float4 m4 = *reinterpret_cast<const float4*>(mean + cc), i4 = *reinterpret_cast<const float4*>(invstd + cc);
        sc01 = (f32x2_t){s4.x, s4.y}; sc23 = (f32x2_t){s4.z, s4.w};
        sh01 = (f32x2_t){h4.x, h4.y}; sh23 = (f32x2_t){h4.z, h4.w};
        is01 = (f32x2_t){i4.x, i4.y}; is23 = (f32x2_t){i4.z, i4.w};
        nm01 = (f32x2_t){-m4.x * i4.x, -m4.y * i4.y}; nm23 = (f32x2_t){-m4.z * i4.z, -m4.w * i4.w};
        lo = (act != MPN_ACT_NONE) ? 0.f : -INFINITY;
        hi = (act == MPN_ACT_RELU6) ? 6.f : INFINITY;
    }
    __device__ __forceinline__ void add(f32x2_t d01, f32x2_t d23, const Raw4<T>& xr, f32x2_t& s01, f32x2_t& s23, f32x2_t& q01, f32x2_t& q23) const {
        f32x2_t x01, x23;
        raw_unpack2(xr, x01, x23);
        const f32x2_t p01 = x01 * sc01 + sh01, p23 = x23 * sc23 + sh23;
        d01 = round_storage<T>(d01); d23 = round_storage<T>(d23);
        f32x2_t g01, g23;
        g01.x = (p01.x > lo && p01.x < hi) ? d01.x : 0.f; g01.y = (p01.y > lo && p01.y < hi) ? d01.y : 0.f;
        g23.x = (p23.x > lo && p23.x < hi) ? d23.x : 0.f; g23.y = (p23.y > lo && p23.y < hi) ? d23.y : 0.f;
        s01 += g01; s23 += g23;
        q01 += g01 * (x01 * is01 + nm01); q23 += g23 * (x23 * is23 + nm23);
    }
};
__device__ __forceinline__ void write_sums_row(float* red, const SwLane& l, int ncg, int cols, int C, float* part, f32x2_t s01, f32x2_t s23,
                                               f32x2_t q01, f32x2_t q23) {
    float st[8] = {s01.x, s01.y, s23.x, s23.y, q01.x, q01.y, q23.x, q23.y};
#pragma unroll
    for (int j = 0; j < 8; ++j) red[threadIdx.x * 8 + j] = l.ok ? st[j] : 0.f;
    __syncthreads();
    if ((int)threadIdx.x < ncg && (l.cgb * ncg + (int)threadIdx.x) * 4 < C) {
        float acc8[8] = {0.f, 0.f, 0.f, 0.f, 0.f, 0.f, 0.f, 0.f};
        for (int cidx = 0; cidx < cols; ++cidx)
#pragma unroll
            for (int j = 0; j < 8; ++j) acc8[j] += red[(cidx * ncg + threadIdx.x) * 8 + j];
        float* dst = part + (long long)l.unit * 2 * C + (l.cgb * ncg + threadIdx.x) * 4;
#pragma unroll
        for (int j = 0; j < 4; ++j) { dst[j] = acc8[j]; dst[C + j] = acc8[4 + j]; }
    }
}
__device__ __forceinline__ void write_taps_row(float* red, const SwLane& l, int ncg, int cols, int C, float* part, const f32x2_t (&a01)[9],
                                               const f32x2_t (&a23)[9]) {
#pragma unroll
    for (int t = 0; t < 9; ++t) {
        float4 v = make_float4(a01[t].x, a01[t].y, a23[t].x, a23[t].y);
        if (!l.ok) v = make_float4(0.f, 0.f, 0.f, 0.f);
        *reinterpret_cast<float4*>(&red[(t * kThreads + threadIdx.x) * 4]) = v;
    }
    __syncthreads();
    const int nch = ncg * 4;
    float* dst = part + (long long)l.unit * 9 * C + l.cgb * nch;
    for (int o = threadIdx.x; o < 9 * nch; o += kThreads) {
        const int t = o / nch, cj = o - t * nch;
        if (l.cgb * nch + cj < C) {
            float sum = 0.f;
            for (int cidx = 0; cidx < cols; ++cidx) sum += red[(t * kThreads + cidx * ncg) * 4 + cj];
            dst[t * C + cj] = sum;
        }
    }
}

template <typename T> __device__ __forceinline__ void quad_load(Raw4<T> (&r)[4], const T* q, long long xrow, int C) {
    raw_load(r[0], q); raw_load(r[1], q + C); raw_load(r[2], q + xrow); raw_load(r[3], q + xrow + C);
}
template <typename T> __device__ __forceinline__ void add_raw4(const Raw4<T>& r, f32x2_t& o01, f32x2_t& o23) {
    float f[4];
    raw_unpack(r, f);
    o01 += (f32x2_t){f[0], f[1]};
    o23 += (f32x2_t){f[2], f[3]};
}

}
```

multiposenet_amd/net.py:

```python
import math
import os
from collections import OrderedDict

import numpy as np
import torch

from . import _lib, ops
from ._lib import ACT_NONE, ACT_RELU, ACT_RELU6
from .model_state import ModelState, _Arena, is_trainable, resolve_device

NUM_KEYPOINTS = 17
DOWNSAMPLE = 4
DIVISOR = 128
DEPTH = 128
STRIDES_AND_FILTERS = [(1, 64), (2, 128), (1, 128), (2, 256), (1, 256), (2, 512), (1, 512), (1, 512),
                       (1, 512), (1, 512), (1, 512), (2, 1024), (1, 1024)]
FEATURE_BLOCKS = {3: "c2", 5: "c3", 11: "c4", 13: "c5"}


def depth(x, depth_multiplier):
    return max(int(x * depth_multiplier), 8)


def variable_shapes(depth_multiplier=1.0):
    s = OrderedDict()

    def bn(prefix, c):
        for n in ("gamma", "beta", "moving_mean", "moving_variance"):
            s[f"{prefix}/{n}"] = (c,)

    c = depth(32, depth_multiplier)
    s["MobilenetV1/Conv2d_0/weights"] = (3, 3, 3, c)
    bn("MobilenetV1/Conv2d_0/BatchNorm", c)
    for i, (_, f) in enumerate(STRIDES_AND_FILTERS, 1):
        s[f"MobilenetV1/Conv2d_{i}_depthwise/depthwise_weights"] = (3, 3, c, 1)
        bn(f"MobilenetV1/Conv2d_{i}_depthwise/BatchNorm", c)
        f = depth(f, depth_multiplier)
        s[f"MobilenetV1/Conv2d_{i}_pointwise/weights"] = (1, 1, c, f)
        bn(f"MobilenetV1/Conv2d_{i}_pointwise/BatchNorm", f)
        c = f
    feat = {2: depth(128, depth_multiplier), 3: depth(256, depth_multiplier),
            4: depth(512, depth_multiplier), 5: depth(1024, depth_multiplier)}
    s["keypoint_fpn/lateral5/kernel"] = (1, 1, feat[5], DEPTH)
    s["keypoint_fpn/p5/kernel"] = (3, 3, DEPTH, DEPTH)
    for i in (4, 3, 2):
        s[f"keypoint_fpn/lateral{i}/kernel"] = (1, 1, feat[i], DEPTH)
        s[f"keypoint_fpn/p{i}/kernel"] = (3, 3, DEPTH, DEPTH)
    for l in (2, 3, 4, 5):
        bn(f"p{l}_batch_norm", DEPTH)
    for l in (2, 3, 4, 5):
        s[f"phi_subnet_{l}/conv1/kernel"] = (3, 3, DEPTH, DEPTH)
        bn(f"phi_subnet_{l}/bn1", DEPTH)
        s[f"phi_subnet_{l}/conv2/kernel"] = (3, 3, DEPTH, DEPTH)
        bn(f"phi_subnet_{l}/bn2", DEPTH)
    s["final_conv3x3/kernel"] = (3, 3, 4 * DEPTH, 64)
    bn("final_bn", 64)
    s["heatmaps/kernel"] = (1, 1, 64, NUM_KEYPOINTS + 1)
    s["heatmaps/bias"] = (NUM_KEYPOINTS + 1,)
    return s


def internal_shapes(depth_multiplier=1.0):
    ref = variable_shapes(depth_multiplier)
    c0 = depth(32, depth_multiplier)
    c0p = (c0 + 15) // 16 * 16
    if c0p == c0:
        return ref, {}
    shapes, pads = OrderedDict(), {}
    for name, shape in ref.items():
        axis = None
        if name.startswith("MobilenetV1/Conv2d_0/") or name.startswith("MobilenetV1/Conv2d_1_depthwise/BatchNorm/"):
            axis = len(shape) - 1
        elif name in ("MobilenetV1/Conv2d_1_depthwise/depthwise_weights", "MobilenetV1/Conv2d_1_pointwise/weights"):
            axis = 2
        if axis is not None:
            assert shape[axis] == c0
            pads[name] = (axis, c0)
            shape = tuple(c0p if i == axis else d for i, d in enumerate(shape))
        shapes[name] = shape
    return shapes, pads


def initial_values(seed=0, depth_multiplier=1.0):
    rs = np.random.RandomState(seed)
    out = OrderedDict()
    for name, shape in variable_shapes(depth_multiplier).items():
        if name.endswith("/gamma") or name.endswith("moving_variance"):
            v = np.ones(shape)
        elif name.endswith("/beta") or name.endswith("moving_mean"):
            v = np.zeros(shape)
        elif name == "heatmaps/bias":
            v = np.array([-math.log(99.0)] * NUM_KEYPOINTS + [0.0])
        elif name == "heatmaps/kernel":
            v = rs.randn(*shape) * 1e-4
        else:
            fan_in = shape[0] * shape[1] * (shape[2] if not name.endswith("depthwise_weights") else 1)
            v = rs.randn(*shape) * math.sqrt(1.0 / fan_in) * 1.2
        out[name] = v.astype(np.float32)
    return out


DP_DEEP_FROM_BLOCK = 7


def backbone_deep_begin_of(arena, first_block=DP_DEEP_FROM_BLOCK):
    return arena.offsets[f"MobilenetV1/Conv2d_{first_block}_depthwise/depthwise_weights"][0]


def backbone_grad_end_of(arena):
    end = 0
    for k, (o, n, _) in arena.offsets.items():
        if k.startswith("MobilenetV1/"):
            end = max(end, o + (n + 3) // 4 * 4)
    return end


@ops._lib.device_guarded("_init", "load_state_dict", "repack_weights", "prepare_inference", "forward", "predict",
                         "backbone_forward", "subnet_forward", "compute_losses", "backward", "add_weight_decay_gradients",
                         "add_weight_decay_loss", "optimizer_step")
class KeypointNet(ModelState):
    def __init__(self, values=None, depth_multiplier=1.0, dtype=torch.bfloat16, device="cuda:0", seed=0):
        if dtype not in (torch.float32, torch.bfloat16):
            raise ValueError("dtype must be torch.float32 or torch.bfloat16")
        self.dtype, self.device, self.dm = dtype, resolve_device(device), depth_multiplier
        self._init(values, depth_multiplier, dtype, seed)

    def _init(self, values, depth_multiplier, dtype, seed):
        shapes, pads = internal_shapes(depth_multiplier)
        for n, s in shapes.items():
            if n.endswith("gamma") and (s[0] % 16 != 0):
                raise ValueError(f"depth_multiplier={depth_multiplier}: {n} has {s[0]} channels; every layer behind the stem "
                                 f"must be a multiple of 16 channels wide (depth multipliers that are multiples of 0.25)")
        self._init_state(shapes, pads=pads)
        self.load_state_dict(values if values is not None else initial_values(seed, depth_multiplier))
        self._build_layers()
        self._bufs = {}

    def _build_layers(self):
        self.stem_w = self.vars["MobilenetV1/Conv2d_0/weights"]
        self.stem_dw = self.grads["MobilenetV1/Conv2d_0/weights"]
        self.stem_bn = self._bn("MobilenetV1/Conv2d_0/BatchNorm", ACT_RELU6)
        self.blocks = []
        for i, (stride, _) in enumerate(STRIDES_AND_FILTERS, 1):
            d, p = f"MobilenetV1/Conv2d_{i}_depthwise", f"MobilenetV1/Conv2d_{i}_pointwise"
            self.blocks.append(dict(
                i=i, stride=stride,
                dw_w=self.vars[d + "/depthwise_weights"], dw_dw=self.grads[d + "/depthwise_weights"],
                dw_bn=self._bn(d + "/BatchNorm", ACT_RELU6),
                pw=self._conv(p + "/weights"), pw_bn=self._bn(p + "/BatchNorm", ACT_RELU6)))
        self.lateral = {l: self._conv(f"keypoint_fpn/lateral{l}/kernel") for l in (5, 4, 3, 2)}
        self.pconv = {l: self._conv(f"keypoint_fpn/p{l}/kernel") for l in (5, 4, 3, 2)}
        self.p_bn = {l: self._bn(f"p{l}_batch_norm", ACT_RELU) for l in (2, 3, 4, 5)}
        self.phi = {}
        for l in (2, 3, 4, 5):
            s = f"phi_subnet_{l}"
            self.phi[l] = dict(conv1=self._conv(s + "/conv1/kernel"), bn1=self._bn(s + "/bn1", ACT_RELU),
                               conv2=self._conv(s + "/conv2/kernel"), bn2=self._bn(s + "/bn2", ACT_RELU))
        self.final_conv = self._conv("final_conv3x3/kernel")
        self.final_bn = self._bn("final_bn", ACT_RELU)
        self.concat_scale = torch.ones(4 * DEPTH, dtype=torch.float32, device=self.device)
        self.concat_shift = torch.zeros(4 * DEPTH, dtype=torch.float32, device=self.device)
        self.phi[2]["bn2"].scale = self.concat_scale[:DEPTH]
        self.phi[2]["bn2"].shift = self.concat_shift[:DEPTH]
        self.concat_affine = ops.Affine(self.concat_scale, self.concat_shift, ACT_RELU)
        self.heat_w, self.heat_b = self.vars["heatmaps/kernel"], self.vars["heatmaps/bias"]
        ok, nk, _ = self._train_arena.offsets["heatmaps/kernel"]
        ob, nb, _ = self._train_arena.offsets["heatmaps/bias"]
        assert ob == ok + nk, "heatmaps/kernel and heatmaps/bias must be adjacent in the arena"
        self._head_grad = self.grad[ok:ob + nb]
        self.fuse_dw_bn = True
        self.fuse_conv_bn = True
        self._l2 = None
        self._wd = None
        self.cache_inference_affine = False
        self._infer_clean = False
        self.fuse_stem_stats = True
        self._build_pack_table()
        self.all_bn = [self.stem_bn] + [b[k] for b in self.blocks for k in ("dw_bn", "pw_bn")] + \
            [self.p_bn[l] for l in (2, 3, 4, 5)] + [self.phi[l][k] for l in (2, 3, 4, 5) for k in ("bn1", "bn2")] + [self.final_bn]

    def _build_pack_table(self):
        import ctypes
        lib = ops._lib.lib()
        nb = lib.mpn_conv_pack_desc_bytes()
        jobs = [(c, t) for c in self.convs for t in (0, 1)]
        host = (ctypes.c_ubyte * (nb * len(jobs)))()
        begin = 0
        dc = ops._lib.dtype_code(self.dtype)
        for j, (c, t) in enumerate(jobs):
            out = c.packed.bwd if t else c.packed.fwd
            blocks = lib.mpn_conv_pack_desc_fill(ctypes.byref(host, j * nb), ops.ptr(c.w), c.cin, c.cout, c.ksize, t, dc,
                                                 ops.ptr(out), begin)
            assert blocks > 0
            begin += blocks
        self._pack_table = torch.frombuffer(bytearray(host), dtype=torch.uint8).to(self.device)
        self._pack_jobs, self._pack_blocks = len(jobs), begin

    def repack_weights(self):
        if ops.LAUNCH_JOBS_ALONE:
            for c in self.convs:
                c.packed.repack()
            return
        ops.call("mpn_conv_pack_weights_batched", ops.ptr(self._pack_table), self._pack_jobs, self._pack_blocks,
                 ops._lib.dtype_code(self.dtype), ops.stream_ptr())

    def _buffers(self, N, H, W, head=True):
        key = (N, H, W) if head else (N, H, W, "backbone")
        b = self._bufs.get(key)
        if b is not None:
            return b
        if H % DIVISOR or W % DIVISOR:
            raise ValueError(f"image height and width must be multiples of {DIVISOR} (got {H}x{W})")
        dt, dev = self.dtype, self.device

        def act(h, w, c):
            return torch.empty((N, h, w, c), dtype=dt, device=dev)

        b = {"shape": (N, H, W)}
        h, w = H // 2, W // 2
        c = self.stem_w.shape[3]
        b["stem"] = act(h, w, c)
        b["dw"], b["pw"], b["hw"] = [], [], [(h, w)]
        for blk in self.blocks:
            if blk["stride"] == 2:
                h, w = h // 2, w // 2
            b["dw"].append(act(h, w, c))
            c = blk["pw"].cout
            b["pw"].append(act(h, w, c))
            b["hw"].append((h, w))
        if not head:
            nbn0 = ops._lib.lib().mpn_bn_stats_num_parts
            b["stat_part"] = torch.empty(nbn0(N * (H // 2) * (W // 2)) * 2 * b["stem"].shape[3], dtype=torch.float32, device=dev)
            self._bufs[key] = b
            return b
        lv = {l: (H >> l, W >> l) for l in (2, 3, 4, 5)}
        b["lv"] = lv
        b["x"] = {l: act(*lv[l], DEPTH) for l in lv}
        b["p"] = {l: act(*lv[l], DEPTH) for l in lv}
        b["y1"] = {l: act(*lv[l], DEPTH) for l in lv}
        b["concat"] = act(*lv[2], 4 * DEPTH)
        b["y2"] = {l: act(*lv[l], DEPTH) for l in lv if l != 2}
        b["y2"][2] = b["concat"][..., :DEPTH]
        b["final"] = act(*lv[2], 64)
        b["logits"] = torch.empty((N, lv[2][0], lv[2][1], NUM_KEYPOINTS + 1), dtype=torch.float32, device=dev)
        nbn = ops._lib.lib().mpn_bn_stats_num_parts

        def rows(t):
            return t.numel() // t.shape[3]

        stat_floats = nbn(rows(b["stem"])) * 2 * b["stem"].shape[3]
        for i, blk in enumerate(self.blocks):
            hh, ww = b["hw"][i]
            cdw, cpw = b["dw"][i].shape[3], blk["pw"].cout
            stat_floats = max(stat_floats, ops.dwconv_num_parts(N, hh, ww, cdw, blk["stride"], dt) * 2 * cdw,
                              nbn(rows(b["dw"][i])) * 2 * cdw,
                              ops.conv_num_parts(N, *b["hw"][i + 1], 1) * 2 * cpw, nbn(rows(b["pw"][i])) * 2 * cpw,
                              ops.dwconv_bwd_data_bn_num_parts(N, hh, ww, cdw, blk["stride"], dt) * 2 * cdw,
                              ops.dwconv_wgrad_num_parts(N, hh, ww, cdw, blk["stride"], dt) * 2 * cdw,
                              ops.conv_wgrad_num_parts(N, *b["hw"][i + 1], cdw, cpw, 1, dt) * 2 * cdw)
        for l in lv:
            stat_floats = max(stat_floats, ops.conv_num_parts(N, *lv[l], 3) * 2 * DEPTH, nbn(N * lv[l][0] * lv[l][1]) * 2 * DEPTH)
        b["stat_part"] = torch.empty(stat_floats, dtype=torch.float32, device=dev)
        b["stat_lv"] = {l: torch.empty(max(ops.conv_num_parts(N, *lv[l], 3), nbn(N * lv[l][0] * lv[l][1])) * 2 * DEPTH,
                                       dtype=torch.float32, device=dev) for l in lv}
        b["fin"] = None
        b["loss_part"] = torch.empty(ops._lib.lib().mpn_keypoint_loss_num_parts(N, *lv[2]) * 8, dtype=torch.float32, device=dev)
        b["losses"] = torch.zeros(8, dtype=torch.float32, device=dev)
        self._bufs[key] = b
        return b

    def _grad_buffers(self, b):
        if "g" in b:
            return b["g"]
        N, H, W = b["shape"]
        dt, dev = self.dtype, self.device
        g = {}
        g["dlogits"] = torch.empty_like(b["logits"])
        g["daux"] = {l: torch.empty((N, *b["lv"][l]), dtype=torch.float32, device=dev) for l in b["lv"]}
        g["final"] = torch.empty_like(b["final"])
        g["concat"] = torch.empty_like(b["concat"])
        for k in ("y1", "p", "x"):
            g[k] = {l: torch.empty_like(b[k][l]) for l in b["lv"]}
        g["y2"] = {l: torch.empty_like(b["y2"][l]) for l in b["lv"] if l != 2}
        g["y2"][2] = g["concat"][..., :DEPTH]
        g["c"] = {}
        for i, name in FEATURE_BLOCKS.items():
            g["c"][name] = torch.empty_like(b["pw"][i - 1])
        g["pw"] = [torch.empty_like(t) for t in b["pw"]]
        g["dw"] = [torch.empty_like(t) for t in b["dw"]]
        g["stem"] = torch.empty_like(b["stem"])
        lib, dc = ops._lib.lib(), ops._lib.dtype_code(dt)
        sites = []
        grouped_np = {}
        for group in self._wgrad_groups():
            hws = [self._conv_hw(b, c) for c in group]
            for c, np_ in zip(group, ops.conv_wgrad_grouped_num_parts(N, hws, group[0].cin, group[0].cout, group[0].ksize, dt)):
                grouped_np[id(c.dw)] = np_
        for c in self.convs:
            hw = self._conv_hw(b, c)
            np_ = grouped_np.get(id(c.dw))
            if np_ is None:
                np_ = ops.conv_wgrad_num_parts(N, hw[0], hw[1], c.cin, c.cout, c.ksize, dt)
            sites.append((id(c.dw), np_, c.w.numel(), c.dw))
        for i, blk in enumerate(self.blocks):
            hh, ww = b["hw"][i]
            cc = b["dw"][i].shape[3]
            sites.append((id(blk["dw_dw"]), lib.mpn_dwconv_wgrad_num_parts(N, hh, ww, cc, blk["stride"], dc), 9 * cc, blk["dw_dw"]))
        sites.append((id(self.stem_dw), lib.mpn_stem_conv_wgrad_num_parts(N, H, W), self.stem_w.numel(), self.stem_dw))
        sites.append((id(self._head_grad), lib.mpn_heatmap_head_bwd_num_parts(N * b["lv"][2][0] * b["lv"][2][1]),
                      self._head_grad.numel(), self._head_grad))
        total = sum(((np_ * n + 3) // 4) * 4 for _, np_, n, _ in sites)
        slab = torch.empty(total, dtype=torch.float32, device=dev)
        deep_keys = {id(blk[k]) if k == "dw_dw" else id(blk[k].dw) for blk in self.blocks if blk["i"] >= DP_DEEP_FROM_BLOCK
                     for k in ("pw", "dw_dw")}
        shallow_keys = {id(blk[k]) if k == "dw_dw" else id(blk[k].dw) for blk in self.blocks if blk["i"] < DP_DEEP_FROM_BLOCK
                        for k in ("pw", "dw_dw")} | {id(self.stem_dw)}
        g["slab"], jobs, off = {}, ([], [], []), 0
        for key, np_, n, out in sites:
            view = slab[off:off + np_ * n]
            g["slab"][key] = view
            jobs[1 if key in deep_keys else (2 if key in shallow_keys else 0)].append((view, np_, n, out.view(-1)))
            off += ((np_ * n + 3) // 4) * 4
        g["reducer"] = tuple(ops.SlabReducer(j, dev) for j in jobs)
# ... 87 lines not shown
                             [self.p_bn[l].affine for l in LV], [b["y1"][l] for l in LV], spl)
        if sep:
            fin["bn1"].run()
        ops.conv_fwd_grouped([b["y1"][l] for l in LV], [self.phi[l]["conv2"].packed.fwd for l in LV], DEPTH, 3,
                             [self.phi[l]["bn1"].affine for l in LV], [b["y2"][l] for l in LV], spl)
        if sep:
            fin["bn2"].run()
        for l in (3, 4, 5):
            ops.bilinear_up_fwd(b["y2"][l], 2 ** (l - 2), b["concat"], (l - 2) * DEPTH, self.phi[l]["bn2"].affine)
        return self._subnet_final(b, N, sp, sep, inference_outputs)

    def _subnet_final(self, b, N, sp, sep, inference_outputs):
        h, w = b["lv"][2]
        ops.conv_fwd(b["concat"], self.final_conv.packed.fwd, 64, 3, self.concat_affine, out=b["final"], stats_part=sp)
        if sep:
            ops.bn_finalize(self.final_bn, sp, ops.conv_stats_rows(N, h, w, b["concat"].shape[3], 64, 3, self.dtype), N * h * w)
        if inference_outputs:
            return ops.heatmap_head_fwd(b["final"], self.heat_w, self.heat_b, self.final_bn.affine, inference=True)
        return ops.heatmap_head_fwd(b["final"], self.heat_w, self.heat_b, self.final_bn.affine, out=b["logits"])

    def _finalize_tables(self, b):
        N = b["shape"][0]
        nbn = ops._lib.lib().mpn_bn_stats_num_parts
        fwd = {k: [] for k in ("p", "bn1", "bn2")}
        bwd = {k: [] for k in ("p", "bn1", "bn2")}
        for l in (2, 3, 4, 5):
            h, w = b["lv"][l]
            cnt = N * h * w
            for k, bn in (("p", self.p_bn[l]), ("bn1", self.phi[l]["bn1"]), ("bn2", self.phi[l]["bn2"])):
                rows3 = ops.conv_stats_rows(N, h, w, DEPTH, DEPTH, 3, self.dtype)
                fwd[k].append((bn, b["stat_lv"][l], rows3, cnt))
                if k != "bn2" and self._fused_conv_bn():
                    bwd[k].append((bn, b["stat_lv"][l], rows3, cnt, True))
                else:
                    bwd[k].append((bn, b["stat_lv"][l], nbn(cnt), cnt))
        out = {k: ops.BnFinalizeBatch(v, self.device) for k, v in fwd.items()}
        out.update({"d" + k: ops.BnBwdFinalizeBatch(v, self.device) for k, v in bwd.items()})
        return out

    def _fused_conv_bn(self):
        return self.fuse_conv_bn and ops.conv_bwd_data_bn_supported(DEPTH, DEPTH, 3, self.dtype)

    def forward(self, images, is_training):
        N, H, W, _ = images.shape
        b = self._buffers(N, H, W)
        feats = self.backbone_forward(images, is_training, b)
        logits = self.subnet_forward(feats, is_training, b)
        self._last = (b, feats, images)
        return logits, {f"p{l}": b["p"][l] for l in (2, 3, 4, 5)}

    def predict(self, images):
        N, H, W, _ = images.shape
        b = self._buffers(N, H, W)
        feats = self.backbone_forward(images, False, b)
        return self.subnet_forward(feats, False, b, inference_outputs=True)

    def compute_losses(self, labels, with_grad=True):
        b = self._last[0]
        g = self._grad_buffers(b) if with_grad else None
        ps = [b["p"][l] for l in (2, 3, 4, 5)]
        return ops.keypoint_loss(b["logits"], labels, ps, g["dlogits"] if g else None,
                                 [g["daux"][l] for l in (2, 3, 4, 5)] if g else None, b["loss_part"], b["losses"])

    @property
    def backbone_deep_begin(self):
        return backbone_deep_begin_of(self._train_arena)

    @property
    def backbone_grad_end(self):
        return backbone_grad_end_of(self._train_arena)

    def backward(self, part=None):
        b, feats, images = self._last
        g = self._grad_buffers(b)
        sp, slab = b["stat_part"], g["slab"]
        if part in (None, 0):
            self._backward_head(b, g, feats, sp, slab)
            g["reducer"][0].run()
        for ph in (1, 2):
            if part in (None, ph):
                self._backward_backbone(b, g, images, sp, slab, ph)
                g["reducer"][ph].run()

    def _backward_head(self, b, g, feats, sp, slab):
        if self._fused_conv_bn() and ops.heatmap_head_bwd_bn_supported(b["final"].shape[3], self.dtype):
            rows = ops.heatmap_head_bwd(b["final"], g["dlogits"], self.heat_w, self.final_bn.affine, g["final"], self._head_grad,
                                        slab[id(self._head_grad)], reduce=False, bn_part=sp)
            ops.bn_backward(self.final_bn, g["final"], b["final"], sp, reduced_parts=rows, raw=True)
        else:
            ops.heatmap_head_bwd(b["final"], g["dlogits"], self.heat_w, self.final_bn.affine, g["final"], self._head_grad,
                                 slab[id(self._head_grad)], reduce=False)
            ops.bn_backward(self.final_bn, g["final"], b["final"], sp)
        ops.conv_bwd_weight(b["concat"], g["final"], 3, self.concat_affine, self.final_conv.dw, slab[id(self.final_conv.dw)], reduce=False)
        ops.conv_fwd(g["final"], self.final_conv.packed.bwd, 4 * DEPTH, 3, None, out=g["concat"])
        if b["fin"] is None:
            b["fin"] = self._finalize_tables(b)
        fin, spl = b["fin"], b["stat_lv"]
        LV = (2, 3, 4, 5)
        sps = [spl[l] for l in LV]
        bn2s, bn1s, pbns = [self.phi[l]["bn2"] for l in LV], [self.phi[l]["bn1"] for l in LV], [self.p_bn[l] for l in LV]
        gy2, gy1, gp = [g["y2"][l] for l in LV], [g["y1"][l] for l in LV], [g["p"][l] for l in LV]
        by2, by1, bp = [b["y2"][l] for l in LV], [b["y1"][l] for l in LV], [b["p"][l] for l in LV]
        for l in (3, 4, 5):
            ops.bilinear_up_bwd(g["concat"], 2 ** (l - 2), (l - 2) * DEPTH, DEPTH, out=g["y2"][l])
        ops.bn_bwd_reduce_grouped(bn2s, gy2, by2, sps)
        fin["dbn2"].run()
        none4 = [None] * 4
        fused = self._fused_conv_bn()
        ops.bn_bwd_apply_grouped(bn2s, gy2, by2)
        ops.conv_bwd_weight_grouped(by1, gy2, 3, [self.phi[l]["bn1"].affine for l in LV], [slab[id(self.phi[l]["conv2"].dw)] for l in LV])
        if fused:
            ops.conv_bwd_data_bn_grouped(gy2, [self.phi[l]["conv2"].packed.bwd for l in LV], DEPTH, bn1s, by1, gy1, sps)
        else:
            ops.conv_fwd_grouped([g["y2"][l] for l in LV], [self.phi[l]["conv2"].packed.bwd for l in LV], DEPTH, 3, none4,
                                 [g["y1"][l] for l in LV], none4)
            ops.bn_bwd_reduce_grouped(bn1s, gy1, by1, sps)
        fin["dbn1"].run()
        ops.bn_bwd_apply_grouped(bn1s, gy1, by1)
        ops.conv_bwd_weight_grouped(bp, gy1, 3, [self.p_bn[l].affine for l in LV], [slab[id(self.phi[l]["conv1"].dw)] for l in LV])
        if fused:
            ops.conv_bwd_data_bn_grouped(gy1, [self.phi[l]["conv1"].packed.bwd for l in LV], DEPTH, pbns, bp, gp, sps)
        else:
            ops.conv_fwd_grouped([g["y1"][l] for l in LV], [self.phi[l]["conv1"].packed.bwd for l in LV], DEPTH, 3, none4,
                                 [g["p"][l] for l in LV], none4)
            ops.bn_bwd_reduce_grouped(pbns, gp, bp, sps)
        fin["dp"].run()
        ops.bn_bwd_apply_grouped(pbns, gp, bp, [g["daux"][l] for l in LV])
        ops.conv_bwd_weight_grouped([b["x"][l] for l in LV], gp, 3, none4, [slab[id(self.pconv[l].dw)] for l in LV])
        ops.conv_fwd_grouped(gp, [self.pconv[l].packed.bwd for l in LV], DEPTH, 3, none4, [g["x"][l] for l in LV], none4)
        g["c5_reduced"] = 0
        for l in (2, 3, 4, 5):
            if l > 2:
                ops.sumpool2x2(g["x"][l - 1], g["x"][l], accumulate=True)
            raw, aff = feats[f"c{l}"]
            ops.conv_bwd_weight(raw, g["x"][l], 1, aff, self.lateral[l].dw, slab[id(self.lateral[l].dw)], reduce=False)
            if l == 5 and self.fuse_conv_bn and ops.conv_bwd_data_bn_supported(DEPTH, raw.shape[3], 1, self.dtype):
                g["c5_reduced"] = ops.conv_bwd_data_bn(g["x"][l], self.lateral[l].packed.bwd, raw.shape[3], 1, self.blocks[-1]["pw_bn"], raw,
                                                       g["c"][f"c{l}"], sp)
            else:
                ops.conv_fwd(g["x"][l], self.lateral[l].packed.bwd, raw.shape[3], 1, None, out=g["c"][f"c{l}"])

    def _backward_backbone(self, b, g, images, sp, slab, phase):
        first, last = DP_DEEP_FROM_BLOCK - 1, len(self.blocks) - 1
        if phase == 1:
            dA, reduced, lateral_added = g["c"]["c5"], g.get("c5_reduced", 0), False
            rng = range(last, first - 1, -1)
        else:
            dA, reduced, lateral_added = g["bb_chain"]
            rng = range(first - 1, -1, -1)
        for i in rng:
            feature = FEATURE_BLOCKS.get(self.blocks[i]["i"])
            if feature in ("c2", "c3", "c4") and not lateral_added:
                ops.add_inplace(dA, g["c"][feature])
            dY = self._backward_pointwise(b, g, sp, slab, i, dA, reduced, raw=i == last)
            dA, reduced, lateral_added = self._backward_depthwise(b, g, sp, slab, i, dY)
        if phase == 1:
            g["bb_chain"] = (dA, reduced, lateral_added)
            return
        ops.bn_backward(self.stem_bn, g["stem"], b["stem"], sp, reduced_parts=reduced)
        ops.stem_conv_bwd_weight(images, g["stem"], self.stem_dw, slab[id(self.stem_dw)], reduce=False)

    def _backward_pointwise(self, b, g, sp, slab, i, dA, reduced, raw):
        blk = self.blocks[i]
        pw, x, dY = blk["pw"], b["dw"][i], g["dw"][i]
        fused = self.fuse_conv_bn and ops.conv1x1_bwd_fused_supported(pw.cin, pw.cout, self.dtype) and pw.cin <= 64
        apply = fused and ops.conv1x1_bwd_fused_apply_supported(pw.cin, pw.cout, self.dtype)
        ops.bn_backward(blk["pw_bn"], dA, b["pw"][i], sp, reduced_parts=reduced, raw=raw, apply=not apply)
        rows = 0
        with _lib.tagged("pointwise"):
            if fused:
                rows = ops.conv1x1_bwd_fused(x, dA, pw.w, blk["dw_bn"], dY, slab[id(pw.dw)], sp,
                                             apply_bn=blk["pw_bn"] if apply else None, y_raw=b["pw"][i] if apply else None)
            else:
                ops.conv_bwd_weight(x, dA, 1, blk["dw_bn"].affine, pw.dw, slab[id(pw.dw)], reduce=False)
                if self.fuse_conv_bn and ops.conv_bwd_data_bn_supported(pw.cout, pw.cin, 1, self.dtype):
                    rows = ops.conv_bwd_data_bn(dA, pw.packed.bwd, pw.cin, 1, blk["dw_bn"], x, dY, sp)
                else:
                    ops.conv_fwd(dA, pw.packed.bwd, pw.cin, 1, None, out=dY)
        ops.bn_backward(blk["dw_bn"], dY, x, sp, reduced_parts=rows, raw=True)
        return dY

    def _backward_depthwise(self, b, g, sp, slab, i, dY):
        blk = self.blocks[i]
        x, bn, dA = (b["pw"][i - 1], self.blocks[i - 1]["pw_bn"], g["pw"][i - 1]) if i > 0 else (b["stem"], self.stem_bn, g["stem"])
        N, hw, C, s = dA.shape[0], b["hw"][i], dA.shape[3], blk["stride"]
        lateral = g["c"][FEATURE_BLOCKS[self.blocks[i - 1]["i"]]] if i > 0 and self.blocks[i - 1]["i"] in FEATURE_BLOCKS else None
        if self.fuse_dw_bn and (s == 2 or lateral is None) and ops.dwconv_bwd_fused_supported(N, *hw, C, s, self.dtype):
            _, reduced = ops.dwconv_bwd_fused(x, dY, blk["dw_w"], bn, None, out=dA, wpart=slab[id(blk["dw_dw"])], bn_part=sp,
                                              reduce=False, stride=s, addend=lateral)
            return dA, reduced, lateral is not None
        ops.dwconv_bwd_weight(x, dY, s, bn.affine, blk["dw_dw"], slab[id(blk["dw_dw"])], reduce=False)
        late = lateral is not None and not ops.dwconv_bwd_data_add_supported(N, *hw, C, s, self.dtype)
        addend = None if late else lateral
        if self.fuse_dw_bn and not late and ops.dwconv_bwd_data_bn_num_parts(N, *hw, C, s, self.dtype) > 0:
            _, reduced = ops.dwconv_bwd_data(dY, blk["dw_w"], hw, s, out=dA, bn=bn, x_bn=x, part=sp, addend=addend)
            return dA, reduced, addend is not None
        ops.dwconv_bwd_data(dY, blk["dw_w"], hw, s, out=dA, addend=addend)
        return dA, 0, addend is not None

    def add_weight_decay_gradients(self, weight_decay):
        if self._wd is None:
            ks = [k for k in self.vars if ("weights" in k or "kernel" in k) and "depthwise_weights" not in k]
            self._wd = ops.AxpyBatch([self.vars[k] for k in ks], [self.grads[k] for k in ks])
        self._wd.run(weight_decay)

    def add_weight_decay_loss(self, weight_decay):
        total = self._last[0]["losses"][6:7]
        if self._l2 is None:
            self._l2 = ops.L2LossBatch([w for k, w in self.vars.items()
                                        if ("weights" in k or "kernel" in k) and "depthwise_weights" not in k])
        self._l2.run(weight_decay, total)

    def optimizer_step(self, initial_learning_rate, num_steps, grad_scale=1.0):
        ops.adam_prepare(self.global_step, self.hyper, initial_learning_rate, num_steps)
        ops.adam_step(self.theta, self.grad, self.adam_m, self.adam_v, self.hyper, grad_scale=grad_scale)
        self.mark_variables_changed()
        self.repack_weights()
```

multiposenet_amd/ops.py:

```python
import ctypes
from collections import namedtuple

import torch

from . import _lib
from ._lib import ACT_NONE, ACT_RELU, ACT_RELU6, call, ptr, stream_ptr

BN_MOMENTUM = 0.95
BN_EPSILON = 1e-3

LAUNCH_JOBS_ALONE = False

Affine = namedtuple("Affine", ["scale", "shift", "act"])


def _f32(n, dev):
    return torch.empty(n, dtype=torch.float32, device=dev)


def _check_nhwc(x, name="x"):
    if x.dim() != 4 or not x.is_contiguous():
        raise ValueError(f"{name} must be a contiguous NHWC tensor, got shape {tuple(x.shape)}")
    if x.dtype not in (torch.float32, torch.bfloat16):
        raise ValueError(f"{name}: unsupported dtype {x.dtype}")
# ... 338 lines not shown
    n = len(bns)
    PA, LA, IA = ctypes.c_void_p * n, ctypes.c_longlong * n, ctypes.c_int * n
    C = xs[0].shape[-1]
    Ms = [x.numel() // x.shape[-1] for x in xs]
    sd, sx = [_row_stride(t, C) for t in dAs], [_row_stride(t, C) for t in xs]
    strides = (None, None) if all(s == C for s in sd + sx) else (IA(*sd), IA(*sx))
    return n, PA, PA(*[ptr(t) for t in dAs]), PA(*[ptr(t) for t in xs]), LA(*Ms), C, _lib.dtype_code(xs[0].dtype), strides


def bn_bwd_reduce_grouped(bns, dAs, xs, parts):
    if LAUNCH_JOBS_ALONE and len(bns) > 1:
        for j in range(len(bns)):
            bn_bwd_reduce_grouped([bns[j]], [dAs[j]], [xs[j]], [parts[j]])
        return
    n, PA, pd, px, Ms, C, dc, (sd, sx) = _bn_group_args(bns, dAs, xs)
    call("mpn_bn_bwd_reduce_grouped", n, pd, px, Ms, C, dc, PA(*[ptr(b.scale) for b in bns]), PA(*[ptr(b.shift) for b in bns]),
         PA(*[ptr(b.mean) for b in bns]), PA(*[ptr(b.invstd) for b in bns]), int(bns[0].act), PA(*[ptr(p) for p in parts]),
         sd, sx, stream_ptr())


def bn_bwd_apply_grouped(bns, dAs, xs, add_ch0s=None):
    if LAUNCH_JOBS_ALONE and len(bns) > 1:
        for j in range(len(bns)):
            bn_bwd_apply_grouped([bns[j]], [dAs[j]], [xs[j]], None if add_ch0s is None else [add_ch0s[j]])
        return
    n, PA, pd, px, Ms, C, dc, (sd, sx) = _bn_group_args(bns, dAs, xs)
    add = add_ch0s if add_ch0s is not None else [None] * n
    call("mpn_bn_bwd_apply_grouped", n, pd, px, Ms, C, dc, PA(*[ptr(b.scale) for b in bns]), PA(*[ptr(b.shift) for b in bns]),
         PA(*[ptr(b.mean) for b in bns]), PA(*[ptr(b.invstd) for b in bns]), PA(*[ptr(b.k1) for b in bns]),
         PA(*[ptr(b.k2) for b in bns]), int(bns[0].act), PA(*[ptr(t) for t in add]), sd, sx, stream_ptr())


def bn_inference_affine(bn):
    call("mpn_bn_inference_affine", bn.C, ptr(bn.gamma), ptr(bn.beta), ptr(bn.moving_mean), ptr(bn.moving_var),
         BN_EPSILON, ptr(bn.scale), ptr(bn.shift), stream_ptr())


def bn_act_apply(x, affine, out=None):
    M, C = x.numel() // x.shape[-1], x.shape[-1]
    if out is None:
        out = torch.empty_like(x)
    call("mpn_bn_act_apply", ptr(x), ptr(out), M, C, _lib.dtype_code(x.dtype), ptr(affine.scale), ptr(affine.shift),
         int(affine.act), stream_ptr())
    return out


def bn_backward(bn, dA, x, part, add_ch0=None, reduced_parts=0, raw=False, apply=True):
    M, C = x.numel() // x.shape[-1], x.shape[-1]
    dc = _lib.dtype_code(x.dtype)
    nparts = _lib.lib().mpn_bn_stats_num_parts(M)
    if reduced_parts and raw:
        call("mpn_bn_bwd_finalize_raw", ptr(part), int(reduced_parts), C, M, ptr(bn.dgamma), ptr(bn.dbeta), ptr(bn.k1), ptr(bn.k2),
             ptr(bn.mean), ptr(bn.invstd), stream_ptr())
    elif reduced_parts:
        call("mpn_bn_bwd_finalize", ptr(part), int(reduced_parts), C, M, ptr(bn.dgamma), ptr(bn.dbeta), ptr(bn.k1), ptr(bn.k2), stream_ptr())
    else:
        call("mpn_bn_bwd_reduce", ptr(dA), ptr(x), M, C, dc, ptr(bn.scale), ptr(bn.shift), ptr(bn.mean), ptr(bn.invstd),
             int(bn.act), ptr(part), stream_ptr())
        call("mpn_bn_bwd_finalize", ptr(part), nparts, C, M, ptr(bn.dgamma), ptr(bn.dbeta), ptr(bn.k1), ptr(bn.k2), stream_ptr())
    if apply:
        call("mpn_bn_bwd_apply", ptr(dA), ptr(x), M, C, dc, ptr(bn.scale), ptr(bn.shift), ptr(bn.mean), ptr(bn.invstd),
             ptr(bn.k1), ptr(bn.k2), int(bn.act), ptr(add_ch0), stream_ptr())
    return dA


def dwconv_out_hw(H, W, stride):
    l = _lib.lib()
    return l.mpn_dwconv_out_size(H, stride), l.mpn_dwconv_out_size(W, stride)


def dwconv_num_parts(N, H, W, C, stride, dtype):
    return _lib.lib().mpn_dwconv_num_parts(N, H, W, C, stride, _lib.dtype_code(dtype))


def dwconv_fwd(x, w, stride, affine=None, out=None, stats_part=None):
    _check_nhwc(x)
    N, H, W, C = x.shape
    OH, OW = dwconv_out_hw(H, W, stride)
    if out is None:
        out = torch.empty((N, OH, OW, C), dtype=x.dtype, device=x.device)
    sc, sh, act = _aff(affine)
    call("mpn_dwconv_fwd", ptr(x), ptr(w), ptr(out), N, H, W, C, stride, _lib.dtype_code(x.dtype), sc, sh, act, 0,
         ptr(stats_part), stream_ptr())
    return out


def dwconv_bwd_data_bn_num_parts(N, H, W, C, stride, dtype):
    return _lib.lib().mpn_dwconv_bwd_data_bn_num_parts(N, H, W, C, stride, _lib.dtype_code(dtype))


def dwconv_bwd_data_add_supported(N, H, W, C, stride, dtype):
    return _lib.lib().mpn_dwconv_bwd_data_add_supported(N, H, W, C, stride, _lib.dtype_code(dtype)) == 1


def dwconv_bwd_data(dy, w, in_hw, stride, out=None, bn=None, x_bn=None, part=None, addend=None):
    N, OH, OW, C = dy.shape
    H, W = in_hw
    if out is None:
        out = torch.empty((N, H, W, C), dtype=dy.dtype, device=dy.device)
    dc = _lib.dtype_code(dy.dtype)
    if addend is not None:
        if addend.shape != out.shape or addend.dtype != out.dtype or not addend.is_contiguous():
            raise ValueError("dwconv_bwd_data: addend must have the result's shape and dtype")
        rows = 0
        if bn is not None:
            rows = dwconv_bwd_data_bn_num_parts(N, H, W, C, stride, dy.dtype)
            if rows <= 0:
                raise ValueError("dwconv_bwd_data: fused batch-norm reduction not available for this shape")
            if part is None:
                part = _f32(rows * 2 * C, dy.device)
            if part.numel() < rows * 2 * C:
                raise ValueError("dwconv_bwd_data: partial slab too small")
        call("mpn_dwconv_bwd_data_add", ptr(dy), ptr(w), ptr(out), N, H, W, C, stride, dc, ptr(addend),
             ptr(x_bn) if bn is not None else None, *((ptr(bn.scale), ptr(bn.shift), ptr(bn.mean), ptr(bn.invstd), int(bn.act),
                                                      ptr(part)) if bn is not None else (None, None, None, None, 0, None)),
             stream_ptr())
        return (out, rows) if bn is not None else out
    if bn is not None:
        rows = dwconv_bwd_data_bn_num_parts(N, H, W, C, stride, dy.dtype)
        if rows <= 0:
            raise ValueError("dwconv_bwd_data: fused batch-norm reduction not available for this shape")
        if part is None:
            part = _f32(rows * 2 * C, dy.device)
        if part.numel() < rows * 2 * C:
            raise ValueError("dwconv_bwd_data: partial slab too small")
        call("mpn_dwconv_bwd_data_bn", ptr(dy), ptr(w), ptr(out), N, H, W, C, stride, dc, ptr(x_bn), ptr(bn.scale), ptr(bn.shift),
             ptr(bn.mean), ptr(bn.invstd), int(bn.act), ptr(part), stream_ptr())
        return out, rows
    call("mpn_dwconv_bwd_data", ptr(dy), ptr(w), ptr(out), N, H, W, C, stride, dc, stream_ptr())
    return out


def dwconv_wgrad_num_parts(N, H, W, C, stride, dtype):
    return _lib.lib().mpn_dwconv_wgrad_num_parts(N, H, W, C, stride, _lib.dtype_code(dtype))


def dwconv_bwd_weight(x, dy, stride, affine, dw_out, part=None, reduce=True):
    N, H, W, C = x.shape
    dc = _lib.dtype_code(x.dtype)
    nparts = _lib.lib().mpn_dwconv_wgrad_num_parts(N, H, W, C, stride, dc)
    if part is None:
        part = _f32(nparts * 9 * C, x.device)
    sc, sh, act = _aff(affine)
    call("mpn_dwconv_bwd_weight", ptr(x), ptr(dy), ptr(part), N, H, W, C, stride, dc, sc, sh, act, stream_ptr())
    if reduce:
        call("mpn_reduce_partials", ptr(part), nparts, 9 * C, ptr(dw_out), 0, 1.0, stream_ptr())
    return dw_out


def dwconv_bwd_fused_supported(N, H, W, C, stride, dtype):
    return _lib.lib().mpn_dwconv_bwd_fused_supported(N, H, W, C, stride, _lib.dtype_code(dtype)) == 1


def dwconv_bwd_fused(x, dy, w, bn, dw_out, out=None, wpart=None, bn_part=None, reduce=True, reduce_bn=True, stride=1, addend=None):
    N, H, W, C = x.shape
    dc = _lib.dtype_code(x.dtype)
    if not dwconv_bwd_fused_supported(N, H, W, C, stride, x.dtype):
        raise ValueError("dwconv_bwd_fused: shape not supported")
    if addend is not None and (stride != 2 or addend.shape != x.shape or addend.dtype != x.dtype or not addend.is_contiguous()):
        raise ValueError("dwconv_bwd_fused: addend needs stride 2 and the result's shape and dtype")
    if out is None:
        out = torch.empty_like(x)
    rows = _lib.lib().mpn_dwconv_wgrad_num_parts(N, H, W, C, stride, dc)
    if wpart is None:
        wpart = _f32(rows * 9 * C, x.device)
    if reduce_bn and bn_part is None:
        bn_part = _f32(rows * 2 * C, x.device)
    if wpart.numel() < rows * 9 * C or (reduce_bn and bn_part.numel() < rows * 2 * C):
        raise ValueError("dwconv_bwd_fused: partial slab too small")
    if stride == 2:
        call("mpn_dwconv_bwd_fused_s2", ptr(x), ptr(dy), ptr(w), ptr(out), ptr(wpart), N, H, W, C, dc, ptr(bn.scale), ptr(bn.shift),
             int(bn.act), ptr(bn.mean), ptr(bn.invstd), ptr(bn_part) if reduce_bn else None, ptr(addend), stream_ptr())
    else:
        call("mpn_dwconv_bwd_fused", ptr(x), ptr(dy), ptr(w), ptr(out), ptr(wpart), N, H, W, C, dc, ptr(bn.scale), ptr(bn.shift),
             int(bn.act), ptr(bn.mean), ptr(bn.invstd), ptr(bn_part) if reduce_bn else None, stream_ptr())
    if reduce:
        call("mpn_reduce_partials", ptr(wpart), rows, 9 * C, ptr(dw_out), 0, 1.0, stream_ptr())
    return out, (rows if reduce_bn else 0)


def stem_conv_fwd_num_parts(N, H, W, c0, dtype):
    return _lib.lib().mpn_stem_conv_fwd_num_parts(N, H, W, c0, _lib.dtype_code(dtype))


def stem_conv_fwd(images, w, c0, dtype, out=None, stats_part=None):
    if images.dim() != 4 or images.shape[3] != 3 or not images.is_contiguous():
        raise ValueError("images must be contiguous [N,H,W,3]")
    u8 = images.dtype == torch.uint8
    if not u8 and images.dtype != torch.float32:
        raise ValueError("images must be float32 in [0,1] or uint8")
    N, H, W, _ = images.shape
    if out is None:
        out = torch.empty((N, (H + 1) // 2, (W + 1) // 2, c0), dtype=dtype, device=images.device)
    if stats_part is not None:
        rows = stem_conv_fwd_num_parts(N, H, W, c0, dtype)
        if rows <= 0 or stats_part.numel() < rows * 2 * c0:
            raise ValueError("stem_conv_fwd: fused statistics not available for this shape, or slab too small")
        call("mpn_stem_conv_fwd_stats", ptr(images), int(u8), ptr(w), ptr(out), N, H, W, c0, _lib.dtype_code(dtype),
             ptr(stats_part), stream_ptr())
        return out
    call("mpn_stem_conv_fwd", ptr(images), int(u8), ptr(w), ptr(out), N, H, W, c0, _lib.dtype_code(dtype), stream_ptr())
    return out


def stem_conv_bwd_weight(images, dy, dw_out, part=None, reduce=True):
    N, H, W, _ = images.shape
    c0 = dy.shape[3]
    nparts = _lib.lib().mpn_stem_conv_wgrad_num_parts(N, H, W)
    if part is None:
        part = _f32(nparts * 27 * c0, dy.device)
    call("mpn_stem_conv_bwd_weight", ptr(images), int(images.dtype == torch.uint8), ptr(dy), ptr(part), N, H, W, c0,
         _lib.dtype_code(dy.dtype), stream_ptr())
    if reduce:
        call("mpn_reduce_partials", ptr(part), nparts, 27 * c0, ptr(dw_out), 0, 1.0, stream_ptr())
    return dw_out


def bilinear_up_fwd(x, upsample, out, channel_offset, affine=None):
    N, h, w, C = x.shape
    sc, sh, act = _aff(affine)
    call("mpn_bilinear_up_fwd", ptr(x), ptr(out), N, h, w, C, upsample, channel_offset, out.shape[3],
         _lib.dtype_code(x.dtype), sc, sh, act, stream_ptr())
    return out


def bilinear_up_bwd(dy, upsample, channel_offset, C, out=None):
    N, OH, OW, ctot = dy.shape
    h, w = OH // upsample, OW // upsample
    if out is None:
        out = torch.empty((N, h, w, C), dtype=dy.dtype, device=dy.device)
    call("mpn_bilinear_up_bwd", ptr(dy), ptr(out), N, h, w, C, upsample, channel_offset, ctot, _lib.dtype_code(dy.dtype),
         stream_ptr())
    return out


def sumpool2x2(src, dst=None, accumulate=False):
    N, H2, W2, C = src.shape
    if dst is None:
        dst = torch.empty((N, H2 // 2, W2 // 2, C), dtype=src.dtype, device=src.device)
    call("mpn_sumpool2x2", ptr(src), ptr(dst), N, H2 // 2, W2 // 2, C, int(accumulate), _lib.dtype_code(src.dtype), stream_ptr())
    return dst


def add_inplace(dst, src):
    if dst.shape != src.shape or dst.dtype != src.dtype:
        raise ValueError("add_inplace: shape/dtype mismatch")
    call("mpn_add_inplace", ptr(dst), ptr(src), dst.numel(), _lib.dtype_code(dst.dtype), stream_ptr())
    return dst


def heatmap_head_fwd(x, w, bias, affine, inference=False, out=None, out_seg=None):
    N, H, W, cin = x.shape
    M = N * H * W
    sc, sh, act = _aff(affine)
    if inference:
        if out is None:
            out = torch.empty((N, H, W, 17), dtype=torch.float32, device=x.device)
        if out_seg is None:
            out_seg = torch.empty((N, H, W), dtype=torch.float32, device=x.device)
    elif out is None:
        out = torch.empty((N, H, W, 18), dtype=torch.float32, device=x.device)
    call("mpn_heatmap_head_fwd", ptr(x), ptr(w), ptr(bias), M, cin, _lib.dtype_code(x.dtype), sc, sh, act,
         int(inference), ptr(out), ptr(out_seg), stream_ptr())
    return (out, out_seg) if inference else out


def heatmap_head_bwd_bn_supported(cin, dtype):
    return bool(_lib.lib().mpn_heatmap_head_bwd_bn_supported(int(cin), _lib.dtype_code(dtype)))


def heatmap_head_bwd(x, dlogits, w, affine, dA, dw_db_out, part=None, reduce=True, bn_part=None):
    N, H, W, cin = x.shape
    M = N * H * W
    nparts = _lib.lib().mpn_heatmap_head_bwd_num_parts(M)
    nout = cin * 18 + 18
    if part is None:
        part = _f32(nparts * nout, x.device)
    sc, sh, act = _aff(affine)
    if bn_part is not None:
        if bn_part.numel() < nparts * 2 * cin:
            raise ValueError("heatmap_head_bwd: bn_part too small")
        call("mpn_heatmap_head_bwd_bn", ptr(x), ptr(dlogits), ptr(w), M, cin, _lib.dtype_code(x.dtype), sc, sh, act, ptr(dA),
             ptr(part), ptr(bn_part), stream_ptr())
    else:
        call("mpn_heatmap_head_bwd", ptr(x), ptr(dlogits), ptr(w), M, cin, _lib.dtype_code(x.dtype), sc, sh, act, ptr(dA),
             ptr(part), stream_ptr())
    if reduce:
        call("mpn_reduce_partials", ptr(part), nparts, nout, ptr(dw_db_out), 0, 1.0, stream_ptr())
    return nparts if bn_part is not None else dA


LOSS_NAMES = ["focal_loss", "regression_loss", "segmentation_loss_at_level_2", "segmentation_loss_at_level_3",
              "segmentation_loss_at_level_4", "segmentation_loss_at_level_5", "total_loss", "per_pixel_reg_loss"]


def keypoint_loss(logits, labels, ps, dlogits=None, daux=None, part=None, losses_out=None):
    B, h, w, _ = logits.shape
    dev = logits.device
    nparts = _lib.lib().mpn_keypoint_loss_num_parts(B, h, w)
    if part is None:
        part = _f32(nparts * 8, dev)
    if losses_out is None:
        losses_out = _f32(8, dev)
    da = daux if daux is not None else [None] * 4
    call("mpn_keypoint_loss", ptr(logits), ptr(labels["heatmaps"]), ptr(labels["loss_masks"]),
         ptr(labels["segmentation_masks"]), ptr(labels["num_boxes"]), ptr(ps[0]), ptr(ps[1]), ptr(ps[2]), ptr(ps[3]),
         ps[0].shape[3], _lib.dtype_code(ps[0].dtype), ptr(dlogits), ptr(da[0]), ptr(da[1]), ptr(da[2]), ptr(da[3]),
         ptr(part), ptr(losses_out), B, h, w, stream_ptr())
    return losses_out


def adam_prepare(step, hyper, initial_learning_rate, num_steps, alpha=1e-4, beta1=0.9, beta2=0.999):
    call("mpn_adam_prepare", ptr(step), ptr(hyper), float(initial_learning_rate), float(num_steps), float(alpha),
         float(beta1), float(beta2), stream_ptr())


def adam_step(params, grads, m, v, hyper, grad_scale=1.0, beta1=0.9, beta2=0.999, eps=1e-8, clip=200.0):
    call("mpn_adam_step", ptr(params), ptr(grads), ptr(m), ptr(v), params.numel(), ptr(hyper), beta1, beta2, eps, clip,
         float(grad_scale), stream_ptr())


def gemm_nt_num_parts(k):
    return _lib.lib().mpn_gemm_nt_num_parts(int(k))
# ... 97 lines not shown
```

Baseline: 4257 images/s.

## Fold depthwise BN backward apply into the fused depthwise backward walk

Adds apply variants of the fused stride-1 and stride-2 depthwise backward kernels. Instead of a separate pass that writes the BN-backward result dY, the kernels read the raw gradient plus the pre-BN activation y_raw and compute the BN backward affine on load. This removes one full read-modify-write pass over each block's depthwise output gradient. In exchange each kernel issues extra y loads, needs more registers, and uses an unfused arithmetic path for some channels to match the rounding of the old code exactly.

```diff
diff --git a/include/mpn.h b/include/mpn.h
--- a/include/mpn.h
+++ b/include/mpn.h
@@ -156,6 +156,17 @@
 int mpn_dwconv_bwd_fused_s2(const void* x, const void* dy, const float* w, void* dx, float* wpart, int N, int H, int W, int C,
                             int dtype, const float* in_scale, const float* in_shift, int in_act, const float* mean,
                             const float* invstd, float* bn_part, const void* addend, mpn_stream_t stream);
+int mpn_dwconv_bwd_fused_apply_supported(int N, int H, int W, int C, int stride, int dtype);
+int mpn_dwconv_bwd_fused_apply(const void* x, const void* g, const void* y_raw, const float* w, void* dx, float* wpart, int N, int H,
+                               int W, int C, int dtype, const float* in_scale, const float* in_shift, int in_act, const float* mean,
+                               const float* invstd, float* bn_part, const float* ap_scale, const float* ap_shift,
+                               const float* ap_mean, const float* ap_invstd, const float* ap_k1, const float* ap_k2, int ap_act,
+                               mpn_stream_t stream);
+int mpn_dwconv_bwd_fused_s2_apply(const void* x, const void* g, const void* y_raw, const float* w, void* dx, float* wpart, int N, int H,
+                                  int W, int C, int dtype, const float* in_scale, const float* in_shift, int in_act,
+                                  const float* mean, const float* invstd, float* bn_part, const void* addend, const float* ap_scale,
+                                  const float* ap_shift, const float* ap_mean, const float* ap_invstd, const float* ap_k1,
+                                  const float* ap_k2, int ap_act, mpn_stream_t stream);
 
 int mpn_stem_conv_fwd(const void* images, int images_u8, const float* w, void* y, int N, int H,
                       int W, int C0, int dtype, mpn_stream_t stream);
diff --git a/multiposenet_amd/_lib.py b/multiposenet_amd/_lib.py
--- a/multiposenet_amd/_lib.py
+++ b/multiposenet_amd/_lib.py
@@ -68,6 +68,9 @@
     "mpn_dwconv_bwd_fused_supported": (_I, [_I, _I, _I, _I, _I, _I]),
     "mpn_dwconv_bwd_fused": (_I, [_P, _P, _P, _P, _P, _I, _I, _I, _I, _I, _P, _P, _I, _P, _P, _P, _P]),
     "mpn_dwconv_bwd_fused_s2": (_I, [_P, _P, _P, _P, _P, _I, _I, _I, _I, _I, _P, _P, _I, _P, _P, _P, _P, _P]),
+    "mpn_dwconv_bwd_fused_apply_supported": (_I, [_I, _I, _I, _I, _I, _I]),
+    "mpn_dwconv_bwd_fused_apply": (_I, [_P, _P, _P, _P, _P, _P, _I, _I, _I, _I, _I, _P, _P, _I, _P, _P, _P, _P, _P, _P, _P, _P, _P, _I, _P]),
+    "mpn_dwconv_bwd_fused_s2_apply": (_I, [_P, _P, _P, _P, _P, _P, _I, _I, _I, _I, _I, _P, _P, _I, _P, _P, _P, _P, _P, _P, _P, _P, _P, _P, _I, _P]),
     "mpn_stem_conv_fwd": (_I, [_P, _I, _P, _P, _I, _I, _I, _I, _I, _P]),
     "mpn_stem_conv_fwd_num_parts": (_I, [_I, _I, _I, _I, _I]),
     "mpn_stem_conv_fwd_stats": (_I, [_P, _I, _P, _P, _I, _I, _I, _I, _I, _P, _P]),
diff --git a/multiposenet_amd/csrc/dwconv.hip b/multiposenet_amd/csrc/dwconv.hip
--- a/multiposenet_amd/csrc/dwconv.hip
+++ b/multiposenet_amd/csrc/dwconv.hip
@@ -36,6 +36,12 @@
     int stride;
     float* wpart;
     int swr;
+    const void* ap_y;
+    const float* ap_scale;
+    const float* ap_mean;
+    const float* ap_invstd;
+    const float* ap_k1;
+    const float* ap_k2;
 };
 
 __device__ __forceinline__ void load4(const float* p, float (&f)[4]) {
@@ -433,7 +439,7 @@
     write_taps_row(red, l, ncg, cols, p.C, p.part, a01, a23);
 }
 
-template <typename T, bool BNR>
+template <typename T, bool BNR, bool APPLY = false>
 __global__ __launch_bounds__(kThreads) void dwconv_bwd_sw2_kernel(const DwParams p, int ncg, int cols, int xblocks, int yblocks, int rows) {
     __shared__ __attribute__((aligned(16))) float red[9 * kThreads * 4];
     const SwLane l = sw_lane<2, true>(p.C, p.W, ncg, cols, xblocks, yblocks, p.cblocks);
@@ -454,20 +460,31 @@
     const long long img_off = (long long)l.img * p.H * p.W * p.C + l.cc;
     const T* ximg = reinterpret_cast<const T*>(p.x) + img_off;
     const T* dimg = reinterpret_cast<const T*>(p.dy) + img_off;
+    DyApply<T> ap;
+    const T* yimg = nullptr;
+    if constexpr (APPLY) {
+        ap.load(p.ap_scale, p.ap_mean, p.ap_invstd, p.ap_k1, p.ap_k2, l.cc);
+        yimg = reinterpret_cast<const T*>(p.ap_y) + img_off;
+    }
+    constexpr int NY = APPLY ? 4 : 1;
     WinCols<T, 4> win;
     win.init(l.ox - 1, l.ok, p.H, p.W, p.C);
     bool xok[4];
 #pragma unroll
     for (int k = 0; k < 4; ++k) xok[k] = l.ok && l.ox - 1 + k >= 0 && l.ox - 1 + k < p.W;
+    Raw4<T> yr[NY];
     auto dy_row = [&](const Raw4<T> (&r)[4], int iy, f32x2_t (&a)[4][2]) {
         const bool rowok = iy >= 0 && iy < p.H;
+        const unsigned erow = (unsigned)img_off + (unsigned)min(max(iy, 0), p.H - 1) * (unsigned)win.rstep;
 #pragma unroll
         for (int k = 0; k < 4; ++k) {
             float f[4];
             raw_unpack(r[k], f);
+            if constexpr (APPLY) ap.apply(f, yr[k], erow + (unsigned)win.off[k]);
             zero_unless(rowok && xok[k], f);
             store_pairs(a[k], f);
         }
+        if constexpr (APPLY) win.load(yr, yimg, iy + 1);
     };
     auto in_row = [&](const Raw4<T> (&r)[4], f32x2_t (&a)[4][2]) {
 #pragma unroll
@@ -514,6 +531,7 @@
     win.load(da, dimg, oy_begin - 1);
     win.load(db, dimg, oy_begin);
     win.load(dc, dimg, oy_begin + 1);
+    if constexpr (APPLY) win.load(yr, yimg, oy_begin - 1);
     win.load(xa, ximg, oy_begin);
     win.load(xb, ximg, oy_begin + 1);
     win.load(xc, ximg, oy_begin + 2);
@@ -655,7 +673,7 @@
     if constexpr (BNR) write_sums_row(red, l, ncg, cols, C, p.part, s01, s23, q01, q23);
 }
 
-template <typename T, bool BNR, bool ADD>
+template <typename T, bool BNR, bool ADD, bool APPLY = false>
 __global__ __launch_bounds__(kThreads) void dwconv_bwd_s2_kernel(const DwParams p, int ncg, int cols, int xblocks, int yblocks, int rows) {
     __shared__ __attribute__((aligned(16))) float red[9 * kThreads * 4];
     const int H = p.H, W = p.W, C = p.C, OH = p.OH, OW = p.OW;
@@ -676,24 +694,41 @@
     const bool right_ok = l.ok && 2 * l.ox + 2 < W;
     const bool left_ok = l.ox > 0;
     const T* dyimg = reinterpret_cast<const T*>(p.dy) + ((long long)l.img * OH * OW) * C + l.cc;
+    DyApply<T> ap;
+    if constexpr (APPLY) ap.load(p.ap_scale, p.ap_mean, p.ap_invstd, p.ap_k1, p.ap_k2, l.cc);
+    const long long ydist = APPLY ? reinterpret_cast<const char*>(p.ap_y) - reinterpret_cast<const char*>(p.dy) : 0;
+    constexpr int NY = APPLY ? 2 : 1;
     const int off_c = l.ox * C, off_l = (left_ok ? l.ox - 1 : 0) * C;
     auto dy_load = [&](Raw4<T> (&r)[2], int a) {
         const T* rowp = dyimg + (long long)min(max(a, 0), OH - 1) * OW * C;
         raw_load(r[0], rowp + off_l);
         raw_load(r[1], rowp + off_c);
     };
+    Raw4<T> y[NY];
+    auto y_load = [&](int a) {
+        if constexpr (APPLY) {
+            const T* rowp = dyimg + (long long)min(max(a, 0), OH - 1) * OW * C;
+            raw_load(y[0], reinterpret_cast<const T*>(reinterpret_cast<const char*>(rowp + off_l) + ydist));
+            raw_load(y[1], reinterpret_cast<const T*>(reinterpret_cast<const char*>(rowp + off_c) + ydist));
+        }
+    };
     auto dy_cvt = [&](const Raw4<T> (&r)[2], int a, f32x2_t (&v)[2][2]) {
         if (a < 0) {
             v[0][0] = v[0][1] = v[1][0] = v[1][1] = (f32x2_t){0.f, 0.f};
+            y_load(a + 1);
             return;
         }
+        const unsigned erow = (unsigned)(l.img * OH * OW * C + l.cc) + (unsigned)min(a, OH - 1) * (unsigned)(OW * C);
         float f[4];
         raw_unpack(r[0], f);
+        if constexpr (APPLY) ap.apply(f, y[0], erow + (unsigned)off_l);
 #pragma unroll
         for (int j = 0; j < 4; ++j) f[j] = left_ok ? f[j] : 0.f;
         v[0][0] = (f32x2_t){f[0], f[1]}; v[0][1] = (f32x2_t){f[2], f[3]};
         raw_unpack(r[1], f);
+        if constexpr (APPLY) ap.apply(f, y[1], erow + (unsigned)off_c);
         v[1][0] = (f32x2_t){f[0], f[1]}; v[1][1] = (f32x2_t){f[2], f[3]};
+        y_load(a + 1);
     };
     const T* ximg = reinterpret_cast<const T*>(p.x) + (long long)l.img * H * W * C + l.cc;
     const int xo0 = 2 * l.ox * C, xo1 = xo0 + C, xo2 = right_ok ? xo0 + 2 * C : xo0;
@@ -772,6 +807,7 @@
     dy_load(ra, a_begin - 1);
     dy_load(rb, a_begin);
     dy_load(rc, a_begin + 1);
+    y_load(a_begin - 1);
     x_load(xa, 2 * a_begin);
     dy_cvt(ra, a_begin - 1, v0);
     dy_load(ra, a_begin + 2);
@@ -1251,51 +1287,115 @@
     return (d.ok && d.ncg == g.ncg && d.cols == g.cols && d.xblocks == g.xblocks && d.yblocks == g.yblocks && dg_rows(p.OH) == g.rows) ? 1 : 0;
 }
 
-extern "C" int mpn_dwconv_bwd_fused(const void* x, const void* dy, const float* w, void* dx, float* wpart, int N, int H, int W, int C,
-                                    int dtype, const float* in_scale, const float* in_shift, int in_act, const float* mean,
-                                    const float* invstd, float* bn_part, mpn_stream_t stream) {
-    MPN_REQUIRE(mpn_dwconv_bwd_fused_supported(N, H, W, C, 1, dtype), MPN_ERR_BAD_SHAPE,
-                "dwconv_bwd_fused: shape not supported (mpn_dwconv_bwd_fused_supported == 0)");
-    MPN_REQUIRE(x && dy && w && dx && wpart && in_scale && in_shift, MPN_ERR_BAD_ARG, "dwconv_bwd_fused: null pointer");
-    MPN_REQUIRE(bn_part == nullptr || (mean && invstd), MPN_ERR_BAD_ARG, "dwconv_bwd_fused: the reduction needs mean and invstd");
-    MPN_REQUIRE(dx != dy && dx != x, MPN_ERR_BAD_ARG, "dwconv_bwd_fused: dx must not alias an input");
+struct DwApplyArgs {
+    const void* y;
+    const float *scale, *shift, *mean, *invstd, *k1, *k2;
+    int act;
+};
+static void dw_set_apply(DwParams& p, const DwApplyArgs& a) {
+    p.ap_y = a.y; p.ap_scale = a.scale; p.ap_mean = a.mean; p.ap_invstd = a.invstd; p.ap_k1 = a.k1; p.ap_k2 = a.k2;
+}
+template <typename T> constexpr bool kDwApply = !std::is_same<T, float>::value;
+
+static int dw_bwd_fused_s1(const char* who, const void* x, const void* dy, const float* w, void* dx, float* wpart, int N, int H, int W, int C,
+                           int dtype, const float* in_scale, const float* in_shift, int in_act, const float* mean, const float* invstd,
+                           float* bn_part, const DwApplyArgs* ap, mpn_stream_t stream) {
+    MPN_REQUIRE(ap ? mpn_dwconv_bwd_fused_apply_supported(N, H, W, C, 1, dtype) : mpn_dwconv_bwd_fused_supported(N, H, W, C, 1, dtype),
+                MPN_ERR_BAD_SHAPE, "%s: shape or type not supported (mpn_dwconv_bwd_fused%s_supported == 0)", who, ap ? "_apply" : "");
+    MPN_REQUIRE(x && dy && w && dx && wpart && in_scale && in_shift, MPN_ERR_BAD_ARG, "%s: null pointer", who);
+    MPN_REQUIRE(bn_part == nullptr || (mean && invstd), MPN_ERR_BAD_ARG, "%s: the reduction needs mean and invstd", who);
+    MPN_REQUIRE(dx != dy && dx != x, MPN_ERR_BAD_ARG, "%s: dx must not alias an input", who);
+    MPN_REQUIRE(!ap || (ap->y && ap->scale && ap->shift && ap->mean && ap->invstd && ap->k1 && ap->k2), MPN_ERR_BAD_ARG,
+                "%s: null pointer (y_raw or its batch-norm)", who);
+    MPN_REQUIRE(!ap || dx != ap->y, MPN_ERR_BAD_ARG, "%s: dx must not alias an input", who);
     DwParams p = {};
     if (int rc = fill_params(p, N, H, W, C, 1, dtype)) return rc;
     p.x = x; p.dy = dy; p.w = w; p.y = dx; p.wpart = wpart; p.part = bn_part;
     p.in_scale = in_scale; p.in_shift = in_shift; p.in_act = in_act; p.bnr.mean = mean; p.bnr.invstd = invstd;
+    if (ap) dw_set_apply(p, *ap);
     const DwWgSwGeom g = dw_wg_sw_geom(p);
     p.cblocks = g.cblocks;
     unsigned grid;
-    if (int rc = dw_grid((long long)g.units * g.cblocks, "dwconv_bwd_fused", &grid)) return rc;
+    if (int rc = dw_grid((long long)g.units * g.cblocks, who, &grid)) return rc;
     hipStream_t st = (hipStream_t)stream;
     MPN_DISPATCH_DTYPE(dtype, {
-        if (bn_part) dwconv_bwd_sw2_kernel<T, true><<<grid, kThreads, 0, st>>>(p, g.ncg, g.cols, g.xblocks, g.yblocks, g.rows);
+        if (ap) {
+            if constexpr (kDwApply<T>) {
+                if (bn_part) dwconv_bwd_sw2_kernel<T, true, true><<<grid, kThreads, 0, st>>>(p, g.ncg, g.cols, g.xblocks, g.yblocks, g.rows);
+                else dwconv_bwd_sw2_kernel<T, false, true><<<grid, kThreads, 0, st>>>(p, g.ncg, g.cols, g.xblocks, g.yblocks, g.rows);
+            }
+        } else if (bn_part) dwconv_bwd_sw2_kernel<T, true><<<grid, kThreads, 0, st>>>(p, g.ncg, g.cols, g.xblocks, g.yblocks, g.rows);
         else dwconv_bwd_sw2_kernel<T, false><<<grid, kThreads, 0, st>>>(p, g.ncg, g.cols, g.xblocks, g.yblocks, g.rows);
     });
     MPN_LAUNCH_CHECK();
     return MPN_OK;
 }
 
-extern "C" int mpn_dwconv_bwd_fused_s2(const void* x, const void* dy, const float* w, void* dx, float* wpart, int N, int H, int W, int C,
-                                       int dtype, const float* in_scale, const float* in_shift, int in_act, const float* mean,
-                                       const float* invstd, float* bn_part, const void* addend, mpn_stream_t stream) {
-    MPN_REQUIRE(mpn_dwconv_bwd_fused_supported(N, H, W, C, 2, dtype), MPN_ERR_BAD_SHAPE,
-                "dwconv_bwd_fused_s2: shape not supported (mpn_dwconv_bwd_fused_supported == 0)");
-    MPN_REQUIRE(x && dy && w && dx && wpart && in_scale && in_shift, MPN_ERR_BAD_ARG, "dwconv_bwd_fused_s2: null pointer");
-    MPN_REQUIRE(bn_part == nullptr || (mean && invstd), MPN_ERR_BAD_ARG, "dwconv_bwd_fused_s2: the reduction needs mean and invstd");
-    MPN_REQUIRE(dx != dy && dx != x && dx != addend, MPN_ERR_BAD_ARG, "dwconv_bwd_fused_s2: dx must not alias an input");
+static int dw_bwd_fused_s2(const char* who, const void* x, const void* dy, const float* w, void* dx, float* wpart, int N, int H, int W, int C,
+                           int dtype, const float* in_scale, const float* in_shift, int in_act, const float* mean, const float* invstd,
+                           float* bn_part, const void* addend, const DwApplyArgs* ap, mpn_stream_t stream) {
+    MPN_REQUIRE(ap ? mpn_dwconv_bwd_fused_apply_supported(N, H, W, C, 2, dtype) : mpn_dwconv_bwd_fused_supported(N, H, W, C, 2, dtype),
+                MPN_ERR_BAD_SHAPE, "%s: shape or type not supported (mpn_dwconv_bwd_fused%s_supported == 0)", who, ap ? "_apply" : "");
+    MPN_REQUIRE(x && dy && w && dx && wpart && in_scale && in_shift, MPN_ERR_BAD_ARG, "%s: null pointer", who);
+    MPN_REQUIRE(bn_part == nullptr || (mean && invstd), MPN_ERR_BAD_ARG, "%s: the reduction needs mean and invstd", who);
+    MPN_REQUIRE(dx != dy && dx != x && dx != addend, MPN_ERR_BAD_ARG, "%s: dx must not alias an input", who);
+    MPN_REQUIRE(!ap || (ap->y && ap->scale && ap->shift && ap->mean && ap->invstd && ap->k1 && ap->k2), MPN_ERR_BAD_ARG,
+                "%s: null pointer (y_raw or its batch-norm)", who);
+    MPN_REQUIRE(!ap || dx != ap->y, MPN_ERR_BAD_ARG, "%s: dx must not alias an input", who);
     DwParams p = {};
     if (int rc = fill_params(p, N, H, W, C, 2, dtype)) return rc;
     p.x = x; p.dy = dy; p.w = w; p.y = dx; p.wpart = wpart; p.part = bn_part; p.addend = addend;
     p.in_scale = in_scale; p.in_shift = in_shift; p.in_act = in_act; p.bnr.mean = mean; p.bnr.invstd = invstd;
+    if (ap) dw_set_apply(p, *ap);
     const DwWgSwGeom g = dw_wg_sw_geom(p);
     p.cblocks = g.cblocks;
     unsigned grid;
-    if (int rc = dw_grid((long long)g.units * g.cblocks, "dwconv_bwd_fused_s2", &grid)) return rc;
+    if (int rc = dw_grid((long long)g.units * g.cblocks, who, &grid)) return rc;
     hipStream_t st = (hipStream_t)stream;
     MPN_DISPATCH_DTYPE(dtype, dw_with_bnr_add(bn_part != nullptr, addend != nullptr, [&](auto B, auto A) {
-        dwconv_bwd_s2_kernel<T, decltype(B)::value, decltype(A)::value><<<grid, kThreads, 0, st>>>(p, g.ncg, g.cols, g.xblocks, g.yblocks, g.rows);
+        if (ap) {
+            if constexpr (kDwApply<T>)
+                dwconv_bwd_s2_kernel<T, decltype(B)::value, decltype(A)::value, true><<<grid, kThreads, 0, st>>>(p, g.ncg, g.cols, g.xblocks, g.yblocks, g.rows);
+        } else dwconv_bwd_s2_kernel<T, decltype(B)::value, decltype(A)::value><<<grid, kThreads, 0, st>>>(p, g.ncg, g.cols, g.xblocks, g.yblocks, g.rows);
     }));
     MPN_LAUNCH_CHECK();
     return MPN_OK;
 }
+
+extern "C" int mpn_dwconv_bwd_fused_apply_supported(int N, int H, int W, int C, int stride, int dtype) {
+    return dtype != MPN_F32 ? mpn_dwconv_bwd_fused_supported(N, H, W, C, stride, dtype) : 0;
+}
+
+extern "C" int mpn_dwconv_bwd_fused(const void* x, const void* dy, const float* w, void* dx, float* wpart, int N, int H, int W, int C,
+                                    int dtype, const float* in_scale, const float* in_shift, int in_act, const float* mean,
+                                    const float* invstd, float* bn_part, mpn_stream_t stream) {
+    return dw_bwd_fused_s1("dwconv_bwd_fused", x, dy, w, dx, wpart, N, H, W, C, dtype, in_scale, in_shift, in_act, mean, invstd, bn_part,
+                           nullptr, stream);
+}
+
+extern "C" int mpn_dwconv_bwd_fused_s2(const void* x, const void* dy, const float* w, void* dx, float* wpart, int N, int H, int W, int C,
+                                       int dtype, const float* in_scale, const float* in_shift, int in_act, const float* mean,
+                                       const float* invstd, float* bn_part, const void* addend, mpn_stream_t stream) {
+    return dw_bwd_fused_s2("dwconv_bwd_fused_s2", x, dy, w, dx, wpart, N, H, W, C, dtype, in_scale, in_shift, in_act, mean, invstd, bn_part,
+                           addend, nullptr, stream);
+}
+
+extern "C" int mpn_dwconv_bwd_fused_apply(const void* x, const void* g, const void* y_raw, const float* w, void* dx, float* wpart, int N,
+                                          int H, int W, int C, int dtype, const float* in_scale, const float* in_shift, int in_act,
+                                          const float* mean, const float* invstd, float* bn_part, const float* ap_scale,
+                                          const float* ap_shift, const float* ap_mean, const float* ap_invstd, const float* ap_k1,
+                                          const float* ap_k2, int ap_act, mpn_stream_t stream) {
+    const DwApplyArgs ap = {y_raw, ap_scale, ap_shift, ap_mean, ap_invstd, ap_k1, ap_k2, ap_act};
+    return dw_bwd_fused_s1("dwconv_bwd_fused_apply", x, g, w, dx, wpart, N, H, W, C, dtype, in_scale, in_shift, in_act, mean, invstd, bn_part,
+                           &ap, stream);
+}
+
+extern "C" int mpn_dwconv_bwd_fused_s2_apply(const void* x, const void* g, const void* y_raw, const float* w, void* dx, float* wpart, int N,
+                                             int H, int W, int C, int dtype, const float* in_scale, const float* in_shift, int in_act,
+                                             const float* mean, const float* invstd, float* bn_part, const void* addend,
+                                             const float* ap_scale, const float* ap_shift, const float* ap_mean, const float* ap_invstd,
+                                             const float* ap_k1, const float* ap_k2, int ap_act, mpn_stream_t stream) {
+    const DwApplyArgs ap = {y_raw, ap_scale, ap_shift, ap_mean, ap_invstd, ap_k1, ap_k2, ap_act};
+    return dw_bwd_fused_s2("dwconv_bwd_fused_s2_apply", x, g, w, dx, wpart, N, H, W, C, dtype, in_scale, in_shift, in_act, mean, invstd,
+                           bn_part, addend, &ap, stream);
+}
diff --git a/multiposenet_amd/csrc/dwconv_walk.h b/multiposenet_amd/csrc/dwconv_walk.h
--- a/multiposenet_amd/csrc/dwconv_walk.h
+++ b/multiposenet_amd/csrc/dwconv_walk.h
@@ -180,6 +180,44 @@
         q01 += g01 * (x01 * is01 + nm01); q23 += g23 * (x23 * is23 + nm23);
     }
 };
+template <typename T> struct DyApply {
+    f32x2_t sc01, sc23, cb01, cb23, cc01, cc23;
+    bool pair67;
+    __device__ __forceinline__ void load(const float* scale, const float* mean, const float* invstd, const float* k1, const float* k2, int cc) {
+        const float4 s4 = *reinterpret_cast<const float4*>(scale + cc), m4 = *reinterpret_cast<const float4*>(mean + cc);
+        const float4 i4 = *reinterpret_cast<const float4*>(invstd + cc);
+        const float4 a4 = *reinterpret_cast<const float4*>(k1 + cc), b4 = *reinterpret_cast<const float4*>(k2 + cc);
+        const float ss[4] = {s4.x, s4.y, s4.z, s4.w}, mm[4] = {m4.x, m4.y, m4.z, m4.w}, ii[4] = {i4.x, i4.y, i4.z, i4.w};
+        const float aa[4] = {a4.x, a4.y, a4.z, a4.w}, bb[4] = {b4.x, b4.y, b4.z, b4.w};
+        float cb[4], cc_[4];
+#pragma unroll
+        for (int j = 0; j < 4; ++j) {
+            cb[j] = -ss[j] * bb[j] * ii[j];
+            cc_[j] = -ss[j] * (aa[j] - mm[j] * ii[j] * bb[j]);
+        }
+        sc01 = (f32x2_t){ss[0], ss[1]}; sc23 = (f32x2_t){ss[2], ss[3]};
+        cb01 = (f32x2_t){cb[0], cb[1]}; cb23 = (f32x2_t){cb[2], cb[3]};
+        cc01 = (f32x2_t){cc_[0], cc_[1]}; cc23 = (f32x2_t){cc_[2], cc_[3]};
+        pair67 = (cc & 4) != 0;
+    }
+    static __device__ __forceinline__ f32x2_t unfused(f32x2_t sc, f32x2_t g, f32x2_t cb, f32x2_t y, f32x2_t cc) {
+#pragma clang fp contract(off)
+        const f32x2_t t = cb * y, u = sc * g;
+        return (cc + t) + u;
+    }
+    __device__ __forceinline__ void apply(float (&f)[4], const Raw4<T>& yr, unsigned elem) const {
+        f32x2_t y01, y23;
+        raw_unpack2(yr, y01, y23);
+        const f32x2_t g01 = {f[0], f[1]}, g23 = {f[2], f[3]};
+        const f32x2_t o01 = __builtin_elementwise_fma(sc01, g01, __builtin_elementwise_fma(cb01, y01, cc01));
+        f32x2_t o23 = __builtin_elementwise_fma(sc23, g23, __builtin_elementwise_fma(cb23, y23, cc23));
+        const f32x2_t v23 = unfused(sc23, g23, cb23, y23, cc23);
+        if (pair67 && ((elem >> 11) & 3u) != 2u) o23 = v23;
+        const f32x2_t r01 = round_storage<T>(o01), r23 = round_storage<T>(o23);
+        f[0] = r01.x; f[1] = r01.y; f[2] = r23.x; f[3] = r23.y;
+    }
+};
+
 __device__ __forceinline__ void write_sums_row(float* red, const SwLane& l, int ncg, int cols, int C, float* part, f32x2_t s01, f32x2_t s23,
                                                f32x2_t q01, f32x2_t q23) {
     float st[8] = {s01.x, s01.y, s23.x, s23.y, q01.x, q01.y, q23.x, q23.y};
diff --git a/multiposenet_amd/net.py b/multiposenet_amd/net.py
--- a/multiposenet_amd/net.py
+++ b/multiposenet_amd/net.py
@@ -169,6 +169,7 @@
         assert ob == ok + nk, "heatmaps/kernel and heatmaps/bias must be adjacent in the arena"
         self._head_grad = self.grad[ok:ob + nb]
         self.fuse_dw_bn = True
+        self.fuse_dw_apply = True
         self.fuse_conv_bn = True
         self._l2 = None
         self._wd = None
@@ -562,15 +563,28 @@
             feature = FEATURE_BLOCKS.get(self.blocks[i]["i"])
             if feature in ("c2", "c3", "c4") and not lateral_added:
                 ops.add_inplace(dA, g["c"][feature])
-            dY = self._backward_pointwise(b, g, sp, slab, i, dA, reduced, raw=i == last)
-            dA, reduced, lateral_added = self._backward_depthwise(b, g, sp, slab, i, dY)
+            dY, applied = self._backward_pointwise(b, g, sp, slab, i, dA, reduced, raw=i == last, fold=self._dw_folds_apply(b, g, i))
+            dA, reduced, lateral_added = self._backward_depthwise(b, g, sp, slab, i, dY, apply=not applied)
         if phase == 1:
             g["bb_chain"] = (dA, reduced, lateral_added)
             return
         ops.bn_backward(self.stem_bn, g["stem"], b["stem"], sp, reduced_parts=reduced)
         ops.stem_conv_bwd_weight(images, g["stem"], self.stem_dw, slab[id(self.stem_dw)], reduce=False)
 
-    def _backward_pointwise(self, b, g, sp, slab, i, dA, reduced, raw):
+    def _dw_lateral(self, g, i):
+        return g["c"][FEATURE_BLOCKS[self.blocks[i - 1]["i"]]] if i > 0 and self.blocks[i - 1]["i"] in FEATURE_BLOCKS else None
+
+    def _dw_walks_fused(self, b, g, i):
+        s, (N, _, _, C) = self.blocks[i]["stride"], b["dw"][i].shape
+        return (self.fuse_dw_bn and (s == 2 or self._dw_lateral(g, i) is None)
+                and ops.dwconv_bwd_fused_supported(N, *b["hw"][i], C, s, self.dtype))
+
+    def _dw_folds_apply(self, b, g, i):
+        s, (N, _, _, C) = self.blocks[i]["stride"], b["dw"][i].shape
+        return (self.fuse_dw_apply and self._dw_walks_fused(b, g, i)
+                and ops.dwconv_bwd_fused_apply_supported(N, *b["hw"][i], C, s, self.dtype))
+
+    def _backward_pointwise(self, b, g, sp, slab, i, dA, reduced, raw, fold=False):
         blk = self.blocks[i]
         pw, x, dY = blk["pw"], b["dw"][i], g["dw"][i]
         fused = self.fuse_conv_bn and ops.conv1x1_bwd_fused_supported(pw.cin, pw.cout, self.dtype) and pw.cin <= 64
@@ -587,18 +601,21 @@
                     rows = ops.conv_bwd_data_bn(dA, pw.packed.bwd, pw.cin, 1, blk["dw_bn"], x, dY, sp)
                 else:
                     ops.conv_fwd(dA, pw.packed.bwd, pw.cin, 1, None, out=dY)
-        ops.bn_backward(blk["dw_bn"], dY, x, sp, reduced_parts=rows, raw=True)
-        return dY
-
-    def _backward_depthwise(self, b, g, sp, slab, i, dY):
+        applied = not (fold and rows > 0)
+        ops.bn_backward(blk["dw_bn"], dY, x, sp, reduced_parts=rows, raw=True, apply=applied)
+        return dY, applied
+
+    def _backward_depthwise(self, b, g, sp, slab, i, dY, apply=False):
         blk = self.blocks[i]
         x, bn, dA = (b["pw"][i - 1], self.blocks[i - 1]["pw_bn"], g["pw"][i - 1]) if i > 0 else (b["stem"], self.stem_bn, g["stem"])
         N, hw, C, s = dA.shape[0], b["hw"][i], dA.shape[3], blk["stride"]
-        lateral = g["c"][FEATURE_BLOCKS[self.blocks[i - 1]["i"]]] if i > 0 and self.blocks[i - 1]["i"] in FEATURE_BLOCKS else None
-        if self.fuse_dw_bn and (s == 2 or lateral is None) and ops.dwconv_bwd_fused_supported(N, *hw, C, s, self.dtype):
+        lateral = self._dw_lateral(g, i)
+        if self._dw_walks_fused(b, g, i):
             _, reduced = ops.dwconv_bwd_fused(x, dY, blk["dw_w"], bn, None, out=dA, wpart=slab[id(blk["dw_dw"])], bn_part=sp,
-                                              reduce=False, stride=s, addend=lateral)
+                                              reduce=False, stride=s, addend=lateral, apply_bn=blk["dw_bn"] if apply else None,
+                                              y_raw=b["dw"][i] if apply else None)
             return dA, reduced, lateral is not None
+        assert not apply, "only the fused depthwise walk applies the batch-norm backward on load"
         ops.dwconv_bwd_weight(x, dY, s, bn.affine, blk["dw_dw"], slab[id(blk["dw_dw"])], reduce=False)
         late = lateral is not None and not ops.dwconv_bwd_data_add_supported(N, *hw, C, s, self.dtype)
         addend = None if late else lateral
diff --git a/multiposenet_amd/ops.py b/multiposenet_amd/ops.py
--- a/multiposenet_amd/ops.py
+++ b/multiposenet_amd/ops.py
@@ -514,11 +514,21 @@
     return _lib.lib().mpn_dwconv_bwd_fused_supported(N, H, W, C, stride, _lib.dtype_code(dtype)) == 1
 
 
-def dwconv_bwd_fused(x, dy, w, bn, dw_out, out=None, wpart=None, bn_part=None, reduce=True, reduce_bn=True, stride=1, addend=None):
+def dwconv_bwd_fused_apply_supported(N, H, W, C, stride, dtype):
+    return _lib.lib().mpn_dwconv_bwd_fused_apply_supported(N, H, W, C, stride, _lib.dtype_code(dtype)) == 1
+
+
+def dwconv_bwd_fused(x, dy, w, bn, dw_out, out=None, wpart=None, bn_part=None, reduce=True, reduce_bn=True, stride=1, addend=None,
+                     apply_bn=None, y_raw=None):
     N, H, W, C = x.shape
     dc = _lib.dtype_code(x.dtype)
     if not dwconv_bwd_fused_supported(N, H, W, C, stride, x.dtype):
         raise ValueError("dwconv_bwd_fused: shape not supported")
+    if apply_bn is not None:
+        if not dwconv_bwd_fused_apply_supported(N, H, W, C, stride, x.dtype):
+            raise ValueError("dwconv_bwd_fused: apply_bn not supported for this shape or dtype")
+        if y_raw is None or y_raw.shape != dy.shape or y_raw.dtype != dy.dtype or not y_raw.is_contiguous():
+            raise ValueError("dwconv_bwd_fused: apply_bn needs y_raw of dy's shape and dtype")
     if addend is not None and (stride != 2 or addend.shape != x.shape or addend.dtype != x.dtype or not addend.is_contiguous()):
         raise ValueError("dwconv_bwd_fused: addend needs stride 2 and the result's shape and dtype")
     if out is None:
@@ -530,7 +540,13 @@
         bn_part = _f32(rows * 2 * C, x.device)
     if wpart.numel() < rows * 9 * C or (reduce_bn and bn_part.numel() < rows * 2 * C):
         raise ValueError("dwconv_bwd_fused: partial slab too small")
-    if stride == 2:
+    ab = apply_bn
+    if ab is not None:
+        aps = (ptr(ab.scale), ptr(ab.shift), ptr(ab.mean), ptr(ab.invstd), ptr(ab.k1), ptr(ab.k2), int(ab.act))
+        name, add = ("mpn_dwconv_bwd_fused_s2_apply", (ptr(addend),)) if stride == 2 else ("mpn_dwconv_bwd_fused_apply", ())
+        call(name, ptr(x), ptr(dy), ptr(y_raw), ptr(w), ptr(out), ptr(wpart), N, H, W, C, dc, ptr(bn.scale), ptr(bn.shift), int(bn.act),
+             ptr(bn.mean), ptr(bn.invstd), ptr(bn_part) if reduce_bn else None, *add, *aps, stream_ptr())
+    elif stride == 2:
         call("mpn_dwconv_bwd_fused_s2", ptr(x), ptr(dy), ptr(w), ptr(out), ptr(wpart), N, H, W, C, dc, ptr(bn.scale), ptr(bn.shift),
              int(bn.act), ptr(bn.mean), ptr(bn.invstd), ptr(bn_part) if reduce_bn else None, ptr(addend), stream_ptr())
     else:
```

Measured after the change: 4367 images/s (median of 6 runs). 1.03x the previous value.
